# ori-drs/gpmp2

Hardware: AMD Instinct MI355X
Metric: trajectories/sec (higher is better)
Workload: dtype f64; 1 GPU; WAMFactorGraphExample: 7-DOF WAM, 100 steps x 5 GP-interp, 200^3 SDF (Synth200), 64 random-init restarts per GPU, GN to tolerance; restarts_per_gpu=64, total_restarts=64, total_step=100, obs_check_inter=5, optimizer=GN, parallelism=trajectory-sharded x1

## Files before the change

### gpmp2_amd/csrc/assembler.h

```cpp
#pragma once
#include "device_math.h"
#include "plan.h"
#include "tiles.h"

namespace g2 {

#ifdef G2_STAMPS
#define G2_BSTAMP(k) do { if (i == 4 && lane == 0 && row0 == 0 && col0 == 0 && pb.iters[b] == G2_STAMP_ITER) pb.stamps[(size_t)b * 64 + 24 + (k)] = __builtin_amdgcn_s_memtime(); } while (0)
#else
#define G2_BSTAMP(k) do {} while (0)
#endif

constexpr int GP_EXTRA_LIE = 18;

template <int D, bool LIE>
struct Assembler {
  static constexpr int n = 2 * D, NG = D * (D + 1) / 2, RECP = NG + D + 1;
  static constexpr int GPN = n + 1 + GP_EXTRA_LIE;
  static constexpr int CQ = 24;
  static constexpr int PT_EXTRA_LIE = 36;
  static constexpr int RECMAX = RECP + PT_EXTRA_LIE;

  struct Slot {
    double* base;
    int rec;
    int npts;
    int gps;
    __device__ __forceinline__ double* pt(int jj) const { return base + jj * rec; }
    __device__ __forceinline__ const double* gpr() const { return base + npts * rec; }
    __device__ __forceinline__ double* gpw() const { return base + npts * rec; }
    __device__ __forceinline__ const double* coef(int jj) const { return base + npts * rec + gps + CQ * jj; }
  };
  __host__ __device__ static int slot_doubles(int I, int RECS, int GPS) { return (I + 1) * RECS + GPS + CQ * I; }
  __device__ __forceinline__ Slot make_slot(double* smem, int which) const {
    return Slot{smem + which * slot_doubles(P.I, P.RECS, P.GPS), P.RECS, P.I + 1, P.GPS};
  }

  const PlanParams& P;
  const PlanBuffers& pb;
  const double* rec;
  const double* gpu;
  int b, lane, c, g;
  int rhscol;
  int row0, col0;
  int tri[4];
  bool valid[4];
  int a_row[4], k_row[4], a_col, k_col;

  __device__ Assembler(const PlanParams& P_, const PlanBuffers& pb_, const double* rec_, const double* gpu_,
                       int b_, int lane_, int row0_ = 0, int col0_ = 0, int rhscol_ = RHSCOL)
      : P(P_), pb(pb_), rec(rec_), gpu(gpu_), b(b_), lane(lane_), c(col0_ + (lane_ & 15)), g(row0_ + (lane_ >> 4)),
        rhscol(rhscol_), row0(row0_), col0(col0_) {
    a_col = c >= D;
    k_col = c - a_col * D;
#pragma unroll
    for (int k = 0; k < 4; k++) {
      const int rho = g + 4 * k;
      valid[k] = rho < n && c < n;
      a_row[k] = rho >= D;
      k_row[k] = rho - a_row[k] * D;
      const int lo = min(k_row[k], k_col), hi = max(k_row[k], k_col);
      tri[k] = valid[k] ? lo * D - (lo * (lo - 1)) / 2 + (hi - lo) : 0;
    }
  }

  static constexpr int NLD2 = (D <= 7) ? 6 : (D <= 11) ? 9 : 14;
  __device__ __forceinline__ void stage2(int iv, const Slot& s0, const Slot& s1, int count = 2) const {
    const int I = P.I, RECS = P.RECS, GPS = P.GPS;
    double2 val[2][NLD2];
#pragma unroll
    for (int w = 0; w < 2; w++) {
      if (w >= count) break;
      const int ivw = iv + w;
      const int npt = (ivw == 0) ? 1 : I + 1;
      const int nd2 = (npt * RECS) >> 1, ng2 = GPS >> 1, nc2 = (CQ / 2) * I;
      const int p0 = (ivw == 0) ? 0 : 1 + (ivw - 1) * (I + 1);
      const bool in_range = ivw <= P.N;
      const double2* src = reinterpret_cast<const double2*>(rec + ((size_t)b * P.Ppad + p0) * RECS);
      const double2* gsrc = reinterpret_cast<const double2*>(gpu + ((size_t)b * P.Npad + ivw) * GPS);
      const double2* csrc = reinterpret_cast<const double2*>(P.coefq);
#pragma unroll
      for (int m = 0; m < NLD2; m++) {
        const int v = lane + 64 * m;
        double2 x = {0.0, 0.0};
        if (v < nd2) {
          if (in_range) x = src[v];
        } else if (v < nd2 + ng2) {
          if (in_range && ivw > 0) x = gsrc[v - nd2];
        } else if (v < nd2 + ng2 + nc2) {
          x = csrc[v - nd2 - ng2];
        }
        val[w][m] = x;
      }
    }
#pragma unroll
    for (int w = 0; w < 2; w++) {
      if (w >= count) break;
      const Slot& s = w ? s1 : s0;
      const int ivw = iv + w;
      const int npt = (ivw == 0) ? 1 : I + 1;
      const int nd2 = (npt * RECS) >> 1, ng2 = GPS >> 1, nc2 = (CQ / 2) * I;
      double2* dpt = reinterpret_cast<double2*>(s.pt((ivw == 0) ? I : 0));
      double2* dgp = reinterpret_cast<double2*>(s.gpw());
#pragma unroll
      for (int m = 0; m < NLD2; m++) {
        const int v = lane + 64 * m;
        if (v < nd2) dpt[v] = val[w][m];
        else if (v < nd2 + ng2 + nc2) dgp[v - nd2] = val[w][m];
      }
    }
  }

  __device__ __forceinline__ static double hint_vec(const double* pt, const double* M, double s, int kr) {
    const double* gp_ = pt + NG;
    if (kr >= 3) return s * gp_[kr];
    return M[0 * 3 + kr] * gp_[0] + M[1 * 3 + kr] * gp_[1] + M[2 * 3 + kr] * gp_[2];
  }

  static constexpr int KT = (D + 15) / 16;
  __device__ __forceinline__ Tile hint_tile(const double* M, const double* cf, int role, int rt, int cbase) const {
    const int j = cbase + (lane & 15), av = j >= D, kk = j - av * D;
    const double* Mk = M + (role * 2 + av) * 9;
    const double sk = cf[role * 2 + av];
    Tile T;
#pragma unroll
    for (int k = 0; k < 4; k++) {
      const int a = 16 * rt + (lane >> 4) + 4 * k;
      const bool pose = a < 3 && kk < 3;
      const double m = Mk[pose ? a * 3 + kk : 0];
      const double v = pose ? m : ((a == kk && a >= 3) ? sk : 0.0);
      T.r[k] = (a < D && j < n) ? v : 0.0;
    }
    return T;
  }
  __device__ __forceinline__ Tile g_tile(const double* pt, int rt, int ct) const {
    const int a2 = 16 * ct + (lane & 15);
    Tile T;
#pragma unroll
    for (int k = 0; k < 4; k++) {
      const int a = 16 * rt + (lane >> 4) + 4 * k;
      const bool in = a < D && a2 < D;
      const int lo = in ? min(a, a2) : 0, hi = in ? max(a, a2) : 0;
      const double v = pt[lo * D - (lo * (lo - 1)) / 2 + (hi - lo)];
      T.r[k] = in ? v : 0.0;
    }
    return T;
  }
  __device__ __forceinline__ static void mfma_atb_acc(const Tile& A, const Tile& B, int rt, v4d& acc) {
#pragma unroll
    for (int k = 0; k < 4; k++) {
      if (16 * rt + 4 * k >= D) continue;
      acc = __builtin_amdgcn_mfma_f64_16x16x4f64(A.r[k], B.r[k], acc, 0, 0, 0);
    }
  }
  __device__ __forceinline__ Tile gp_tile(const double* J, double s, int rt, int cbase) const {
    const int j = cbase + (lane & 15), av = j >= D, kk = j - av * D;
    Tile T;
#pragma unroll
    for (int k = 0; k < 4; k++) {
      const int a = 16 * rt + (lane >> 4) + 4 * k;
      const bool pose = !av && a < 3 && kk < 3;
      const double m = J[pose ? a * 3 + kk : 0];
      const double v = pose ? m : ((a == kk && (av || a >= 3)) ? (av ? 1.0 : s) : 0.0);
      T.r[k] = (a < D && j < n) ? v : 0.0;
    }
    return T;
  }
  __device__ __forceinline__ Tile qc_tile(int rt, int ct) const {
    const int a2 = 16 * ct + (lane & 15);
    Tile T;
#pragma unroll
    for (int k = 0; k < 4; k++) {
      const int a = 16 * rt + (lane >> 4) + 4 * k;
      const bool in = a < D && a2 < D;
      const double v = P.Qc_inv[in ? a * D + a2 : 0];
      T.r[k] = in ? v : 0.0;
    }
    return T;
  }
  __device__ __forceinline__ static void congruence(const Tile (&G)[KT][KT], const Tile (&EL)[KT], const Tile (&ER)[KT],
                                                    v4d& acc) {
#pragma unroll
    for (int ra = 0; ra < KT; ra++) {
      v4d ge = {0.0, 0.0, 0.0, 0.0};
#pragma unroll
      for (int rb = 0; rb < KT; rb++) mfma_atb_acc(G[rb][ra], ER[rb], rb, ge);
      Tile GE;
#pragma unroll
      for (int k = 0; k < 4; k++) GE.r[k] = ge[k];
      mfma_atb_acc(EL[ra], GE, ra, acc);
    }
  }
  bool skip_interp = false;
  __device__ __forceinline__ void lie_interp(const Slot& si, const Slot& sn, bool has_prev, bool has_next, bool want_c,
                                             double (&dk)[4], double (&hrk)[4], double (&hlk)[4]) const {
    if (skip_interp) return;
    v4d ad = {dk[0], dk[1], dk[2], dk[3]}, ar_ = {hrk[0], hrk[1], hrk[2], hrk[3]}, al = {hlk[0], hlk[1], hlk[2], hlk[3]};
    auto point = [&](const double* pt, const double* cf, int role, v4d& acc_d, v4d& acc_c) {
      const double* M = pt + RECP;
      Tile G[KT][KT], EL[KT], ER[KT];
#pragma unroll
      for (int ra = 0; ra < KT; ra++) {
#pragma unroll
        for (int rb = 0; rb < KT; rb++) G[rb][ra] = g_tile(pt, rb, ra);
        EL[ra] = hint_tile(M, cf, role, ra, row0);
        ER[ra] = hint_tile(M, cf, role, ra, col0);
      }
      congruence(G, EL, ER, acc_d);
      if (want_c) {
#pragma unroll
        for (int ra = 0; ra < KT; ra++) ER[ra] = hint_tile(M, cf, 1 - role, ra, col0);
        congruence(G, EL, ER, acc_c);
      }
    };
#pragma unroll 1
    for (int jj = 0; jj < P.I; jj++) {
      const double* cf = si.coef(jj) + 16;
      if (has_prev) point(si.pt(jj), cf, 1, ad, al);
      if (has_next) point(sn.pt(jj), cf, 0, ad, ar_);
    }
#pragma unroll
    for (int k = 0; k < 4; k++) {
      dk[k] = ad[k];
      hrk[k] = ar_[k];
      hlk[k] = al[k];
    }
  }

  __device__ __forceinline__ double build_tiles(int i, const Slot& si, const Slot& sn, const double* z, Tile& S,
                                                Tile& Cl, Tile& Cr, bool want_c) const {
    const int I = P.I, N = P.N;
    const bool has_prev = i > 0, has_next = i < N;
    constexpr bool lie = LIE;
    const double dt = P.delta_t, w0 = P.Winv[0], w1 = P.Winv[1], w3 = P.Winv[3];
    const double* J3i = si.gpr() + n + 1 + 9;
    const double* J1n = sn.gpr() + n + 1;
    const double* J1i = si.gpr() + n + 1;
    const double* J3n = sn.gpr() + n + 1 + 9;

    G2_BSTAMP(0);
    const bool need_diag = (row0 == col0), need_rhs = (rhscol >= col0 && rhscol < col0 + 16);
    const int orow = row0 + lane;
    const bool owner = lane < 16 && orow < n && (need_diag || need_rhs);
    const int nxp = pb.xp_n[b];
    double o_dd = 0.0, o_gg = 0.0, o_ee = 0.0;
    if (owner) {
      const int rho = orow, ar = rho >= D, kr = rho - ar * D;
      const bool prior_here = (i == 0 || (i == N && pb.goal_on[b] && (ar || !P.end_conf_prior_off)));
      const double zz = z[rho];
      double z0 = 0.0, z1 = 0.0, z2 = 0.0;
      if (lie) { z0 = z[0]; z1 = z[1]; z2 = z[2]; }
      double dd = 0.0, gg = 0.0, ee = 0.0;
      if (prior_here) {
        const double* tg = (i == 0) ? (ar ? pb.start_vel : pb.start_conf) : (ar ? pb.end_vel : pb.end_conf);
        tg += (size_t)b * D;
        const double w = ar ? P.vel_prior_w : P.conf_prior_w;
        double dz = zz - tg[kr];
        if (lie && !ar && kr < 3) {
          const P2 bt = pose2_between(P2{z0, z1, z2}, P2{tg[0], tg[1], tg[2]});
          dz = -(kr == 0 ? bt.x : kr == 1 ? bt.y : bt.th);
        }
        dd += w;
        gg += w * dz;
        ee += w * dz * dz;
      }
      double Hh;
      if (!ar && P.flag_pos_limit && !(lie && kr < 3)) {
        const double e = hinge_limit(zz, P.pos_lo[kr], P.pos_hi[kr], P.pos_th[kr], Hh);
        dd += P.pos_w[kr] * Hh * Hh;
        gg += P.pos_w[kr] * Hh * e;
        ee += P.pos_w[kr] * e * e;
      }
      if (ar && P.flag_vel_limit) {
        const double e = hinge_limit(zz, -P.vel_lim[kr], P.vel_lim[kr], P.vel_th[kr], Hh);
        dd += P.vel_w[kr] * Hh * Hh;
        gg += P.vel_w[kr] * Hh * e;
        ee += P.vel_w[kr] * e * e;
      }
      if (ar && kr == 1 && P.vdyn_w > 0.0) {
        dd += P.vdyn_w;
        gg += P.vdyn_w * zz;
        ee += P.vdyn_w * zz * zz;
      }
      for (int e = 0; e < nxp; e++) {
        const size_t xe = (size_t)b * XP_MAX + e;
        if (pb.xp_state[xe] != i || (ar && !pb.xp_has_vel[xe])) continue;
        const double* Wm = pb.xp_info + (xe * 2 + ar) * D * D + (size_t)kr * D;
        const double* tg = pb.xp_target + xe * n + ar * D;
        double wr = 0.0, rk = 0.0;
        for (int cc = 0; cc < D; cc++) {
          double rc = z[ar * D + cc] - tg[cc];
          if (lie && !ar && cc < 3) {
            const P2 bt = pose2_between(P2{z0, z1, z2}, P2{tg[0], tg[1], tg[2]});
            rc = -(cc == 0 ? bt.x : cc == 1 ? bt.y : bt.th);
          }
          wr = fma(Wm[cc], rc, wr);
          if (cc == kr) rk = rc;
        }
        dd += Wm[kr];
        gg += wr;
        ee += wr * rk;
      }
      if (need_rhs) {
        if (!ar) gg += si.pt(I)[NG + kr];
        for (int jj = 0; jj < I; jj++) {
          const double* cf = si.coef(jj) + 16;
          const double cp = ar ? cf[3] : cf[2], cl = ar ? cf[1] : cf[0];
          if (lie) {
            if (has_prev) gg += hint_vec(si.pt(jj), si.pt(jj) + RECP + (ar ? 27 : 18), cp, kr);
            if (has_next) gg += hint_vec(sn.pt(jj), sn.pt(jj) + RECP + (ar ? 9 : 0), cl, kr);
            continue;
          }
          if (has_prev) gg = fma(cp, si.pt(jj)[NG + kr], gg);
          if (has_next) gg = fma(cl, sn.pt(jj)[NG + kr], gg);
        }
        if (!lie) {
          if (has_next) gg += ar ? (dt * sn.gpr()[kr] + sn.gpr()[D + kr]) : sn.gpr()[kr];
          if (has_prev) gg -= si.gpr()[rho];
        } else {
          if (has_next) {
            if (ar) gg += -dt * sn.gpr()[kr] - sn.gpr()[D + kr];
            else if (kr < 3) gg += J1n[0 * 3 + kr] * sn.gpr()[0] + J1n[1 * 3 + kr] * sn.gpr()[1] + J1n[2 * 3 + kr] * sn.gpr()[2];
            else gg -= sn.gpr()[kr];
          }
          if (has_prev) {
            if (ar) gg += si.gpr()[D + kr];
            else if (kr < 3) gg += J3i[0 * 3 + kr] * si.gpr()[0] + J3i[1 * 3 + kr] * si.gpr()[1] + J3i[2 * 3 + kr] * si.gpr()[2];
            else gg += si.gpr()[kr];
          }
        }
      }
      o_dd = dd;
      o_gg = gg;
      o_ee = need_diag ? ee : 0.0;
    }

    G2_BSTAMP(1);
    double dk[4] = {0, 0, 0, 0}, hrk[4] = {0, 0, 0, 0}, hlk[4] = {0, 0, 0, 0};
    const int ac = a_col, kc = k_col;
    if constexpr (!lie) {
      const int cc_ = min(c, n - 1);
      const double fp = has_prev ? 1.0 : 0.0, fn = has_next ? 1.0 : 0.0;
      int wq[4];
      const double* un = si.pt(I);
#pragma unroll
      for (int k = 0; k < 4; k++) {
        const int rr_ = min(g + 4 * k, n - 1);
        wq[k] = a_row[k] * 2 + ac;
        double d = fp * P.KB[rr_ * n + cc_] + fn * P.KA[rr_ * n + cc_];
        const double u = un[tri[k]];
        d += (wq[k] == 0) ? u : 0.0;
        dk[k] = d;
        if (want_c) {
          hrk[k] = fn * P.KO[rr_ * n + cc_];
          hlk[k] = fp * P.KO[cc_ * n + rr_];
        }
      }
      G2_BSTAMP(2);
      if (has_prev && has_next) {
#pragma unroll 1
        for (int jj = 0; jj < I; jj++) {
          const double* cq = si.coef(jj);
          const double* pp_ = si.pt(jj);
          const double* pn_ = sn.pt(jj);
#pragma unroll
          for (int k = 0; k < 4; k++) {
            const double Gp = pp_[tri[k]], Gn = pn_[tri[k]];
            dk[k] = fma(cq[wq[k]], Gp, dk[k]);
            dk[k] = fma(cq[4 + wq[k]], Gn, dk[k]);
            if (want_c) {
              hrk[k] = fma(cq[8 + wq[k]], Gn, hrk[k]);
              hlk[k] = fma(cq[12 + wq[k]], Gp, hlk[k]);
            }
          }
        }
      } else {
        for (int jj = 0; jj < I; jj++) {
          const double* cq = si.coef(jj);
          const double* pp_ = si.pt(jj);
          const double* pn_ = sn.pt(jj);
#pragma unroll
          for (int k = 0; k < 4; k++) {
            if (has_prev) {
              const double Gp = pp_[tri[k]];
              dk[k] = fma(cq[wq[k]], Gp, dk[k]);
              if (want_c) hlk[k] = fma(cq[12 + wq[k]], Gp, hlk[k]);
            }
            if (has_next) {
              const double Gn = pn_[tri[k]];
              dk[k] = fma(cq[4 + wq[k]], Gn, dk[k]);
              if (want_c) hrk[k] = fma(cq[8 + wq[k]], Gn, hrk[k]);
            }
          }
        }
      }
#pragma unroll
      for (int k = 0; k < 4; k++) {
        dk[k] = valid[k] ? dk[k] : 0.0;
        hrk[k] = valid[k] ? hrk[k] : 0.0;
        hlk[k] = valid[k] ? hlk[k] : 0.0;
      }
    } else {
    v4d xdp = {0.0, 0.0, 0.0, 0.0}, xl = xdp, xdn = xdp, xr = xdp;
    {
      Tile Qt[KT][KT], EL[KT], ER[KT];
#pragma unroll
      for (int ra = 0; ra < KT; ra++)
#pragma unroll
        for (int rb = 0; rb < KT; rb++) Qt[rb][ra] = qc_tile(rb, ra);
      if (has_prev) {
#pragma unroll
        for (int ra = 0; ra < KT; ra++) { EL[ra] = gp_tile(J3i, 1.0, ra, row0); ER[ra] = gp_tile(J3i, 1.0, ra, col0); }
        congruence(Qt, EL, ER, xdp);
// ... 63 lines not shown
```

### gpmp2_amd/csrc/cr_kernels.hip

```cpp
#include "assembler.h"
#include "cr_schedule.h"
#include "dispatch.h"
#include "plan_device.h"

namespace g2 {

#ifdef G2_STAMPS
#define G2_STAMP(k)                                                          \
  do {                                                                       \
    if (tid == 0 && (k) < 64 && g2_son) pb.stamps[(size_t)b * 64 + (k)] = __builtin_amdgcn_s_memtime(); \
  } while (0)
#define G2_STAMP_DECL const bool g2_son = pb.iters[b] == G2_STAMP_ITER
#else
#define G2_STAMP(k) do {} while (0)
#define G2_STAMP_DECL do {} while (0)
#endif
#ifdef G2_TSTAMPS
#define G2_TSTAMP(q)                                                                                     \
  do {                                                                                                   \
    if (w == 0 && lane == 0 && idx == 0 && g2_son && (h == 4 || h == 8 || h == 16)) \
      pb.stamps[((size_t)gridDim.x + b) * 64 + (h == 4 ? 0 : h == 8 ? 8 : 16) + (q)] = __builtin_amdgcn_s_memtime(); \
  } while (0)
#else
#define G2_TSTAMP(q) do {} while (0)
#endif
#ifdef G2_STAMPS
#define G2_ASTAMP(k) do { if (v == 5 && lane == 0 && pb.iters[b] == G2_STAMP_ITER) pb.stamps[(size_t)b * 64 + 32 + (k)] = __builtin_amdgcn_s_memtime(); \
                          if (v == 6 && lane == 0 && pb.iters[b] == G2_STAMP_ITER) pb.stamps[(size_t)b * 64 + 40 + (k)] = __builtin_amdgcn_s_memtime(); } while (0)
#else
#define G2_ASTAMP(k) do {} while (0)
#endif

template <int n>
__device__ __forceinline__ void schur_sub(Tile& S, const Tile& A, int lane) {
  const int c = lane & 15, g = lane >> 4;
  const Tile T = tile_atb(A, A);
#pragma unroll
  for (int k = 0; k < 4; k++)
    if ((g + 4 * k) < n && (c < n || c == RHSCOL)) S.r[k] -= T.r[k];
}
constexpr unsigned long long schur_mask(int n, int k) {
  unsigned long long m = 0;
  for (int g = 0; g < 4; g++)
    for (int c = 0; c < 16; c++)
      if (g + 4 * k < n && (c < n || c == RHSCOL)) m |= 1ull << (16 * g + c);
  return m;
}
template <unsigned long long M>
__device__ __forceinline__ double keep_lanes(double x) {
  int lo = __double2loint(x), hi = __double2hiint(x);
  const unsigned long long m = M;
  asm("v_cndmask_b32_e64 %0, 0, %0, %2\n\tv_cndmask_b32_e64 %1, 0, %1, %2" : "+v"(lo), "+v"(hi) : "s"(m));
  return __hiloint2double(hi, lo);
}
template <int n>
__device__ __forceinline__ void schur_keep(Tile& T) {
  T.r[0] = keep_lanes<schur_mask(n, 0)>(T.r[0]);
  T.r[1] = keep_lanes<schur_mask(n, 1)>(T.r[1]);
  T.r[2] = keep_lanes<schur_mask(n, 2)>(T.r[2]);
  T.r[3] = keep_lanes<schur_mask(n, 3)>(T.r[3]);
}
template <int n>
__device__ __forceinline__ Tile schur_prod(const Tile& A, int lane) {
  Tile T = tile_atb(A, A);
  schur_keep<n>(T);
  return T;
}
template <int n>
__device__ __forceinline__ Tile coupling(const Tile& A, const Tile& B, int lane) {
  const int c = lane & 15, g = lane >> 4;
  Tile T = tile_atb(A, B);
#pragma unroll
  for (int k = 0; k < 4; k++) T.r[k] = ((g + 4 * k) < n && c < n) ? -T.r[k] : 0.0;
  return T;
}

constexpr int ASM_WAVES = 4;
constexpr int ASM_WT_MAX_B = 256;
#ifndef G2_ASM_MINW
#define G2_ASM_MINW 5
#endif
template <int D, bool LIE, StorePolicy ASM_OUT>
__global__ __launch_bounds__(64 * ASM_WAVES, LIE ? 2 : G2_ASM_MINW) void k_assemble(const PlanParams* __restrict__ pp, PlanBuffers pb,
                                                              const double* __restrict__ traj, int bufsel,
                                                              double* __restrict__ tiles,
                                                              const int* __restrict__ active, int early_stop) {
  constexpr int n = 2 * D;
  using Asm = Assembler<D, LIE>;
  const PlanParams& P = *pp;
  const int N = P.N;
  const int groups = crr_groups(N, ASM_WAVES);
  const int b = blockIdx.x / groups, q = blockIdx.x - b * groups;
  if (active && !active[b]) return;
  if (early_stop) {
    int status;
    if (gn_decide(P.rules, pb.iters[b], pb.prev_err[b], error_from_shares(P, pb, b), status) != 0) return;
  }
  if (active && dogleg_retry(P, pb, b)) return;
  const int wv = threadIdx.x >> 6, lane = threadIdx.x & 63, c = lane & 15, g = lane >> 4;
  const int v = ASM_WAVES * q + wv, i = v - 1;
  const bool live = v >= 1 && i <= N;
  const int ic = min(max(i, 0), N);
  extern __shared__ __attribute__((aligned(16))) double asm_smem[];
  const int slotd = Asm::slot_doubles(P.I, P.RECS, P.GPS);
  double* xch = asm_smem + (size_t)(ASM_WAVES + 1) * slotd;
  double* xs0 = (slotd >= TILE_DBL) ? asm_smem : xch + 4 * TILE_DBL;
  const double* rec = rec_of(pb, pb.which[b], bufsel);
  const double* gpu = gpu_of(pb, pb.which[b], bufsel);
  Asm as(P, pb, rec, gpu, b, lane);
  G2_ASTAMP(0);
  const typename Asm::Slot slot0 = as.make_slot(asm_smem, wv), slot1 = as.make_slot(asm_smem, wv + 1);
  as.stage2(max(i, 0), slot0, slot1, wv == ASM_WAVES - 1 ? 2 : 1);
  __syncthreads();
  G2_ASTAMP(1);
  const bool odd = (v & 1) != 0;
  const bool fuse2 = N >= 3;
  const bool lvl2 = fuse2 && wv == 2 && live;
  Tile S, Cl, Cr;
  double err_acc = as.build_tiles(ic, slot0, slot1, traj + ((size_t)b * (N + 1) + ic) * n, S, Cl, Cr,
                                  odd || P.rules.opt_type == GPMP2MI_OPT_DOGLEG);
  G2_ASTAMP(2);
  if (live) {
    if (!early_stop) {
      err_acc = wave_sum(err_acc);
      if (lane == 0) pb.epart[(size_t)b * P.Npad + i] = 0.5 * err_acc;
      if (c == RHSCOL) {
#pragma unroll
        for (int k = 0; k < 4; k++) pb.gvec[((size_t)b * (N + 1) + i) * 16 + g + 4 * k] = -S.r[k];
      }
    }
    if (P.rules.opt_type == GPMP2MI_OPT_DOGLEG) {
      double* ht = pb.htiles + ((size_t)b * (N + 1) + i) * 2 * TILE_DBL;
      tile_store(ht, S, lane);
      tile_store(ht + TILE_DBL, Cr, lane);
    }
    if (P.rules.opt_type == GPMP2MI_OPT_LM) {
      const double lam = pb.lambda[b];
#pragma unroll
      for (int k = 0; k < 4; k++)
        if (g + 4 * k == c && c < n) S.r[k] += lam;
    }
    if (!odd) {
      if (!fuse2) tile_store_rows<n, ASM_OUT>(tiles + ((size_t)b * (N + 1) + i) * TILE_DBL, S, lane);
      else if (wv == 0) tile_store(xs0, S, lane);
    } else {
      Tile V;
      G2_ASTAMP(3);
      const bool ok = tile_eliminate_cv<n>(S, Cl, Cr, V, lane);
      G2_ASTAMP(4);
      double* f = pb.fac + ((size_t)b * (N + 1) + i) * 3 * TILE_DBL;
      tile_store_rows<n, ASM_OUT>(f, Cl, lane);
      tile_store_rows<n, ASM_OUT>(f + TILE_DBL, Cr, lane);
      tile_store_transposed<n, ASM_OUT>(f + 2 * TILE_DBL, V, lane);
      if (fuse2) {
        double* x = xch + (size_t)(wv >> 1) * 2 * TILE_DBL;
        tile_store(x, Cl, lane);
        tile_store(x + TILE_DBL, Cr, lane);
      }
      if (!ok && lane == 0) pb.notspd[b] = 1;
      G2_ASTAMP(5);
    }
  }
  if (!fuse2) return;
  __syncthreads();
  G2_ASTAMP(6);
  if (wv != 2) return;
  const int v0 = ASM_WAVES * q, M = N + 1;
  const bool has0 = q >= 1;
  const bool next = v0 + 4 <= M;
  Tile Sp = tile_zero();
  if (has0) Sp = tile_load(xs0, lane);
  Tile A1 = tile_zero(), R = tile_zero();
  if (has0 && v0 + 1 <= M) {
    const Tile Wl1 = tile_load(xch, lane);
    A1 = tile_atb(Wl1, Wl1);
  }
  if (next) {
    const Tile Wr3 = tile_load(xch + 3 * TILE_DBL, lane);
    R = tile_atb(Wr3, Wr3);
  }
  if (live) {
    const Tile Wr_m = tile_load(xch + TILE_DBL, lane);
    schur_sub<n>(S, Wr_m, lane);
    Tile C2l = tile_zero(), C2r = tile_zero();
    if (has0) {
      const Tile Wl_m = tile_load(xch, lane);
      C2l = coupling<n>(Wr_m, Wl_m, lane);
    }
    if (v + 1 <= M) {
      const Tile Wl_p = tile_load(xch + 2 * TILE_DBL, lane);
      schur_sub<n>(S, Wl_p, lane);
      if (v + 2 <= M) {
        const Tile Wr_p = tile_load(xch + 3 * TILE_DBL, lane);
        C2r = coupling<n>(Wl_p, Wr_p, lane);
      }
    }
    Tile V;
    const bool ok = tile_eliminate_cv<n>(S, C2l, C2r, V, lane);
    double* f = pb.fac + ((size_t)b * (N + 1) + i) * 3 * TILE_DBL;
    tile_store_rows<n, ASM_OUT>(f, C2l, lane);
    tile_store_rows<n, ASM_OUT>(f + TILE_DBL, C2r, lane);
    tile_store_transposed<n, ASM_OUT>(f + 2 * TILE_DBL, V, lane);
    if (!ok && lane == 0) pb.notspd[b] = 1;
    const Tile A2 = tile_atb(C2l, C2l);
#pragma unroll
    for (int k = 0; k < 4; k++) A1.r[k] += A2.r[k];
    if (next) {
      const Tile B2 = tile_atb(C2r, C2r);
#pragma unroll
      for (int k = 0; k < 4; k++) R.r[k] += B2.r[k];
      if (has0) {
        const Tile K = (q & 1) ? coupling<n>(C2l, C2r, lane) : coupling<n>(C2r, C2l, lane);
        tile_store_rows<n, ASM_OUT>(pb.coup + ((size_t)b * groups + q) * TILE_DBL, K, lane);
      }
    }
    G2_ASTAMP(7);
  }
  schur_keep<n>(A1);
  schur_keep<n>(R);
  if (has0) {
#pragma unroll
    for (int k = 0; k < 4; k++) Sp.r[k] -= A1.r[k];
    tile_store_rows<n, ASM_OUT>(tiles + ((size_t)b * (N + 1) + v0 - 1) * TILE_DBL, Sp, lane);
  }
  if (next) tile_store_rows<n, ASM_OUT>(pb.pend + ((size_t)b * groups + q) * TILE_DBL, R, lane);
}

int launch_assemble(const PlanParams& hp, const PlanBuffers& pb, const double* traj, int bufsel,
                    const int* active, hipStream_t st, bool early_stop) {
  const int es = early_stop ? 1 : 0;
  const dim3 grid(hp.B * crr_groups(hp.N, ASM_WAVES)), block(64 * ASM_WAVES);
  const size_t slotd = (size_t)(hp.I + 1) * hp.RECS + hp.GPS + 24 * hp.I;
  const size_t shmem = ((ASM_WAVES + 1) * slotd + (slotd >= TILE_DBL ? 4 : 5) * TILE_DBL) * sizeof(double);
  return launch_for_dof(TILE_DOFS, hp.D, [&](auto d) {
    constexpr int D = decltype(d)::value;
    constexpr StorePolicy WT = StorePolicy::WriteThrough, PL = StorePolicy::Plain;
    const bool wt = hp.B <= ASM_WT_MAX_B;
    if (hp.lie && wt) k_assemble<D, true, WT><<<grid, block, shmem, st>>>(pb.params, pb, traj, bufsel, pb.tiles, active, es);
    else if (hp.lie) k_assemble<D, true, PL><<<grid, block, shmem, st>>>(pb.params, pb, traj, bufsel, pb.tiles, active, es);
    else if (wt) k_assemble<D, false, WT><<<grid, block, shmem, st>>>(pb.params, pb, traj, bufsel, pb.tiles, active, es);
    else k_assemble<D, false, PL><<<grid, block, shmem, st>>>(pb.params, pb, traj, bufsel, pb.tiles, active, es);
  });
}

constexpr int FIN_BLOCKS = 8;
#ifndef G2_CR_WAVES
#define G2_CR_WAVES 16
#endif
constexpr int CR_WAVES = G2_CR_WAVES;



template <int n>
__device__ __forceinline__ bool cr_forward(const PlanBuffers& pb, int b, int N, int tid) {
  const int w = __builtin_amdgcn_readfirstlane(tid >> 6), lane = tid & 63, c = lane & 15, g = lane >> 4;
  double* tiles = pb.tiles + (size_t)b * (N + 1) * TILE_DBL;
  double* fac = pb.fac + (size_t)b * (N + 1) * 3 * TILE_DBL;
  bool ok = true;
  G2_STAMP_DECL;
  const int htop = crr_top(N), M = N + 1;
  const int h0 = (N >= 3) ? 4 : 2;
  const bool defer4 = (h0 == 4) && (htop >= 8);
  for (int h = h0; h <= htop; h <<= 1) {
    const CrrLevel level = crr_level(N, h, !(defer4 && h == 4));
    const int hh = h >> 1;
    for (int idx = w; idx < level.tasks(); idx += CR_WAVES) {
      const bool elim = level.elim(idx);
      const int v = level.block(idx), j = v - 1;
      const bool first = h0 == 4 && (h == 4 || (defer4 && h == 8));
      const bool ready = h0 == 4 && h == 4;
      const int jm = j - hh, jp = j + hh, qj = v >> 2;
      const bool ep = v + hh <= M;
      const bool cm = elim && v - h >= 1, cp = elim && v + h <= M;
      auto facp = [&](int blk, int which) { return fac + ((size_t)blk * 3 + which) * TILE_DBL; };
      const int groups = crr_groups(N, 4);
      const double* pend = pb.pend + (size_t)b * groups * TILE_DBL;
      const double* coup = pb.coup + (size_t)b * groups * TILE_DBL;
      G2_TSTAMP(0);
      Tile S = tile_load_rows<n>(tiles + (size_t)j * TILE_DBL, lane);
      Tile Pd = tile_zero();
      Tile Wr_m = tile_zero(), Wl_m = tile_zero(), Wl_p = tile_zero(), Wr_p = tile_zero();
      Tile Cl = tile_zero(), Cr = tile_zero();
      if (first) Pd = tile_load_rows<n>(pend + (size_t)(qj - 1) * TILE_DBL, lane);
      if (ready) {
        if (cm) Cl = tile_load_rows<n>(coup + (size_t)(qj - 1) * TILE_DBL, lane);
        if (cp) Cr = tile_load_rows<n>(coup + (size_t)qj * TILE_DBL, lane);
      } else {
        Wr_m = tile_load_rows<n>(facp(jm, 1), lane);
        if (cm) Wl_m = tile_load_rows<n>(facp(jm, 0), lane);
        if (ep) Wl_p = tile_load_rows<n>(facp(jp, 0), lane);
        if (cp) Wr_p = tile_load_rows<n>(facp(jp, 1), lane);
      }
#ifdef G2_TSTAMPS
      asm volatile("s_waitcnt vmcnt(0)" ::: "memory");
#endif
      G2_TSTAMP(1);
#pragma unroll
      for (int k = 0; k < 4; k++) S.r[k] -= Pd.r[k];
      if (!ready) {
        schur_sub<n>(S, Wr_m, lane);
        if (cm) Cl = coupling<n>(Wr_m, Wl_m, lane);
        if (ep) schur_sub<n>(S, Wl_p, lane);
        if (cp) Cr = coupling<n>(Wl_p, Wr_p, lane);
      }
      if (!elim) {
        tile_store_rows<n>(tiles + (size_t)j * TILE_DBL, S, lane);
        continue;
      }
#ifdef G2_TSTAMPS
      asm volatile("" : "+v"(S.r[0]), "+v"(Cl.r[0]), "+v"(Cr.r[0]));
#endif
      G2_TSTAMP(2);
      Tile V;
      ok = tile_eliminate_cv<n>(S, Cl, Cr, V, lane) && ok;
#ifdef G2_TSTAMPS
      asm volatile("" : "+v"(V.r[0]), "+v"(Cl.r[0]), "+v"(Cr.r[0]));
#endif
      G2_TSTAMP(3);
      double* f = fac + (size_t)j * 3 * TILE_DBL;
      tile_store_rows<n>(f, Cl, lane);
      tile_store_rows<n>(f + TILE_DBL, Cr, lane);
      tile_store_rows<n>(f + 2 * TILE_DBL, V, lane);
      G2_TSTAMP(4);
    }
    __syncthreads();
    { const int idx = 0; G2_TSTAMP(5); }
    G2_STAMP(5 + __builtin_ctz(h));
  }
  return ok;
}

template <int n>
__device__ __forceinline__ void cr_backward(const PlanBuffers& pb, int b, int N, int tid, double* xs, int hmin = 1) {
  const int w = __builtin_amdgcn_readfirstlane(tid >> 6), lane = tid & 63, c = lane & 15, g = lane >> 4;
  const double* fac = pb.fac + (size_t)b * (N + 1) * 3 * TILE_DBL;
  G2_STAMP_DECL;
  const int htop = crr_top(N), M = N + 1;
  Tile pWl = tile_zero(), pWr = tile_zero(), pV = tile_zero();
  auto prefetch = [&](int h) {
    if (h >= hmin && w < crr_back_count(N, h)) {
      const double* f = fac + (size_t)(crr_back_block(N, h, w) - 1) * 3 * TILE_DBL;
      pWl = tile_load_rows<n>(f, lane);
      pWr = tile_load_rows<n>(f + TILE_DBL, lane);
      pV = load_v<n>(f + 2 * TILE_DBL, h, N, lane);
    }
  };
  prefetch(htop);
  for (int h = htop; h >= hmin; h >>= 1) {
    const int count = crr_back_count(N, h);
    for (int idx = w; idx < count; idx += CR_WAVES) {
      const int v = crr_back_block(N, h, idx), j = v - 1;
      Tile Wl = pWl, Wr = pWr, V = pV;
      if (idx != w) {
        const double* f = fac + (size_t)j * 3 * TILE_DBL;
        Wl = tile_load_rows<n>(f, lane);
        Wr = tile_load_rows<n>(f + TILE_DBL, lane);
        V = load_v<n>(f + 2 * TILE_DBL, h, N, lane);
      }
      const int jl = j - h, jr = j + h;
      const double xl = (v - h >= 1) ? xs[jl * 16 + c] : 0.0;
      const double xr = (v + h <= M) ? xs[jr * 16 + c] : 0.0;
      const double x = cr_backsolve<n>(Wl, Wr, V, xl, xr, lane);
      if (g == 0) xs[j * 16 + c] = (c < n) ? x : 0.0;
    }
    prefetch(h >> 1);
    __syncthreads();
    G2_STAMP(16 + __builtin_ctz(h));
  }

}

template <int D>
__device__ __forceinline__ void gn_step_body(const PlanParams& P, const PlanBuffers& pb, int pass, int early_stop) {
  constexpr int n = 2 * D;
  const int b = blockIdx.x, tid = threadIdx.x, w = tid >> 6, lane = tid & 63, c = lane & 15, g = lane >> 4;
  if (!pb.active[b]) return;
  const int N = P.N;
  const size_t tsz = (size_t)(N + 1) * n;
  const bool odd = P.fuse_finish && (pass & 1);
  double* cur = (odd ? pb.last : pb.cur) + b * tsz;
  double* last = (odd ? pb.cur : pb.last) + b * tsz;
  double* result = pb.result + b * tsz;
  extern __shared__ __attribute__((aligned(16))) double smem[];
  double* xs = smem;
  double* red = smem + (size_t)(N + 1) * 16;
  int* flags = reinterpret_cast<int*>(red + CR_WAVES);
  G2_STAMP_DECL;

  G2_STAMP(0);
  const int it = pb.iters[b];
  const double prev = pb.prev_err[b];
  double new_err;
  if (early_stop) {
    new_err = error_from_shares(P, pb, b);
    if (tid == 0) flags[1] = 0;
  } else {
    if (w == 0) {
      double acc = 0.0;
      for (int i = lane; i <= N; i += 64) acc += pb.epart[(size_t)b * P.Npad + i];
      acc = wave_sum(acc);
      if (lane == 0) {
        red[0] = acc;
        flags[1] = 0;
      }
    }
    __syncthreads();
    new_err = red[0];
  }
  int status;
  const int decision = gn_decide(P.rules, it, prev, new_err, status);
  if (tid == 0) {
    if (it <= P.rules.max_iter) pb.trace[(size_t)b * (P.rules.max_iter + 1) + it] = new_err;
    pb.cur_err[b] = new_err;
    if (decision != 0) {
      pb.status[b] = status;
      pb.final_err[b] = (decision == 2) ? prev : new_err;
    }
  }
  const bool keep_err = it == 0 || (decision == 0 && P.rules.fixed_iters == 0);
  if (decision != 0) {
    const double* src = (decision == 2) ? last : cur;
    for (size_t k = tid; k < tsz; k += blockDim.x) result[k] = src[k];
    __syncthreads();
    if (tid == 0) {
      if (keep_err) pb.prev_err[b] = new_err;
      pb.active[b] = 0;
    }
    return;
  }

  G2_STAMP(1);
  const bool ok = cr_forward<n>(pb, b, N, tid);
  G2_STAMP(2);
  if ((!ok && lane == 0) || (tid == 0 && pb.notspd[b])) flags[1] = 1;
  __syncthreads();
  if (tid == 0 && keep_err) pb.prev_err[b] = new_err;
  if (flags[1]) {
    if (tid == 0) pb.notspd[b] = 0;
    for (size_t k = tid; k < tsz; k += blockDim.x) result[k] = cur[k];
    if (tid == 0) {
      pb.status[b] = GPMP2MI_TRAJ_NOT_SPD;
      pb.final_err[b] = pb.cur_err[b];
      pb.active[b] = 0;
    }
    return;
  }

  if (P.split_back) {
    cr_backward<n>(pb, b, N, tid, xs, FIN_BLOCKS);
    G2_STAMP(3);
    double* xg = pb.xg + (size_t)b * (N + 1) * 16;
    for (int k = tid; k < ((N + 1) / FIN_BLOCKS) * 16; k += blockDim.x) {
      const size_t o = ((size_t)((k >> 4) + 1) * FIN_BLOCKS - 1) * 16 + (k & 15);
      xg[o] = xs[o];
    }
    G2_STAMP(4);
    if (tid == 0) {
      pb.stepped[b] = pass + 1;
      pb.last_err[b] = pb.cur_err[b];
      pb.iters[b] += 1;
      atomicAdd(pb.n_active + pass, 1);
    }
    return;
  }
  cr_backward<n>(pb, b, N, tid, xs);
  G2_STAMP(3);
  for (size_t k = tid; k < tsz; k += blockDim.x) last[k] = cur[k];
  __syncthreads();
  for (size_t k = tid; k < tsz; k += blockDim.x) {
    const int i = (int)(k / n), rho = (int)(k - (size_t)i * n);
    const double* zs = last + (size_t)i * n;
    const double* dz = xs + i * 16;
    cur[k] = (rho < D) ? retract_coord(P.lie != 0, rho, zs, dz) : zs[rho] + dz[rho];
  }
  G2_STAMP(4);
  if (tid == 0) {
    pb.last_err[b] = pb.cur_err[b];
    pb.iters[b] += 1;
    atomicAdd(pb.n_active + pass, 1);
  }
}
template <int D>
__global__ __launch_bounds__(64 * CR_WAVES) void k_gn_step_cr(const PlanParams* __restrict__ pp,
                                                               PlanBuffers pb, int pass, int early_stop) {
  gn_step_body<D>(*pp, pb, pass, early_stop);
  if (threadIdx.x == 0) publish_pass_count(pb, pass);
}

template <int D>
struct FinishGroup {
  static constexpr int n = 2 * D;
  Tile Wl, Wr, V;
  int b, q, wv, lane, c, g, v, i, N;
  bool live;
  __device__ __forceinline__ FinishGroup(const PlanBuffers& pb, int N_, int b_, int q_, double (*xl_)[16])
      : b(b_), q(q_), N(N_) {
    wv = __builtin_amdgcn_readfirstlane(threadIdx.x >> 6);
    lane = threadIdx.x & 63;
    c = lane & 15;
    g = lane >> 4;
    v = FIN_BLOCKS * q + wv;
    i = v - 1;
    live = v >= 1 && i <= N;
    const double* xg = pb.xg + (size_t)b * (N + 1) * 16;
    const double* fac = pb.fac + (size_t)b * (N + 1) * 3 * TILE_DBL;
    Wl = Wr = V = tile_zero();
    if (live && wv != 0) {
      const double* f = fac + (size_t)i * 3 * TILE_DBL;
      Wl = tile_load_rows<n>(f, lane);
      Wr = tile_load_rows<n>(f + TILE_DBL, lane);
      V = load_v<n>(f + 2 * TILE_DBL, (v & 3) ? 1 : 4, N, lane);
    }
    if (wv == 0 && lane < 16) xl_[0][lane] = live ? xg[(size_t)i * 16 + lane] : 0.0;
    if (wv == 1 && lane < 16)
      xl_[FIN_BLOCKS][lane] = (FIN_BLOCKS * q + FIN_BLOCKS <= N + 1) ? xg[(size_t)(FIN_BLOCKS * q + FIN_BLOCKS - 1) * 16 + lane] : 0.0;
  }
  __device__ __forceinline__ void solve(int h, double (*xl_)[16]) const {
    const int vl = v - h, vr = v + h;
    const double xl = (vl >= 1) ? xl_[vl - FIN_BLOCKS * q][c] : 0.0;
    const double xr = (vr <= N + 1) ? xl_[vr - FIN_BLOCKS * q][c] : 0.0;
    const double x = cr_backsolve<n>(Wl, Wr, V, xl, xr, lane);
    if (g == 0) xl_[wv][c] = (c < n) ? x : 0.0;
  }
  __device__ __forceinline__ void solve_all(double (*xl_)[16]) const {
    __syncthreads();
    if (wv == 4 && live) solve(4, xl_);
    __syncthreads();
    if ((wv == 2 || wv == 6) && live) solve(2, xl_);
    __syncthreads();
    if ((wv & 1) && live) solve(1, xl_);
    __syncthreads();
  }
};

template <int D>
__global__ __launch_bounds__(64 * FIN_BLOCKS) void k_finish_step(const PlanParams* __restrict__ pp, PlanBuffers pb, int pass) {
  constexpr int n = 2 * D;
  const PlanParams& P = *pp;
  const int N = P.N;
  const int groups = crr_groups(N, FIN_BLOCKS);
  const int b = blockIdx.x / groups, q = blockIdx.x - b * groups;
  if (pb.stepped[b] != pass + 1) return;
  __shared__ double xl_[FIN_BLOCKS + 1][16];
  const FinishGroup<D> fg(pb, N, b, q, xl_);
  fg.solve_all(xl_);
  const int lane = fg.lane, i = fg.i;
  if (!fg.live || lane >= n) return;
  const size_t k = ((size_t)b * (N + 1) + i) * n + lane;
  const double* zs = pb.cur + ((size_t)b * (N + 1) + i) * n;
  const double zold = zs[lane];
  const double znew = (lane < D) ? retract_coord(P.lie != 0, lane, zs, xl_[fg.wv]) : zold + xl_[fg.wv][lane];
  pb.last[k] = zold;
  __builtin_amdgcn_wave_barrier();
  pb.cur[k] = znew;
}

int launch_finish_step(const PlanParams& hp, const PlanBuffers& pb, int pass, hipStream_t st) {
  const dim3 grid(hp.B * crr_groups(hp.N, FIN_BLOCKS)), block(64 * FIN_BLOCKS);
  return launch_for_dof(TILE_DOFS, hp.D, [&](auto d) {
    k_finish_step<decltype(d)::value><<<grid, block, 0, st>>>(pb.params, pb, pass);
  });
}

template <int D, int X>
__device__ __forceinline__ void finish_trial_group(const PlanParams& P, const PlanBuffers& pb, int b, int q, int i0,
                                                   const double* x) {
  constexpr int n = 2 * D;
  __shared__ double psum[FIN_BLOCKS][3];
  const int N = P.N, groups = P.spart_groups;
  const int wv = __builtin_amdgcn_readfirstlane(threadIdx.x >> 6), lane = threadIdx.x & 63;
  const int i = i0 + wv;
  double gd = 0.0, dd = 0.0, gg = 0.0;
  if (i >= 0 && i <= N && lane < n) {
    const size_t k = ((size_t)b * (N + 1) + i) * n + lane;
    const double* zs = pb.cur + ((size_t)b * (N + 1) + i) * n;
    const double xk = x[lane], gk = pb.gvec[((size_t)b * (N + 1) + i) * X + lane];
    pb.delta[k] = xk;
    pb.trial[k] = (lane < D) ? retract_coord(P.lie != 0, lane, zs, x) : zs[lane] + xk;
    gd = gk * xk;
    dd = xk * xk;
    gg = gk * gk;
  }
  gd = wave_sum(gd);
  dd = wave_sum(dd);
  gg = wave_sum(gg);
  if (lane == 0) {
    psum[wv][0] = gd;
    psum[wv][1] = dd;
    psum[wv][2] = gg;
  }
  __syncthreads();
  if (threadIdx.x < 3) {
    const int t = threadIdx.x;
    double a = 0.0;
    for (int w = 0; w < FIN_BLOCKS; w++) a += psum[w][t];
    pb.spart[((size_t)b * groups + q) * 3 + t] = a;
  }
}

template <int D>
__global__ __launch_bounds__(64 * FIN_BLOCKS) void k_finish_trial(const PlanParams* __restrict__ pp, PlanBuffers pb) {
  const PlanParams& P = *pp;
  const int N = P.N;
  const int groups = crr_groups(N, FIN_BLOCKS);
  const int b = blockIdx.x / groups, q = blockIdx.x - b * groups;
  if (!pb.active[b] || pb.stepped[b] != 1) return;
  __shared__ double xl_[FIN_BLOCKS + 1][16];
  const FinishGroup<D> fg(pb, N, b, q, xl_);
  fg.solve_all(xl_);
  finish_trial_group<D, 16>(P, pb, b, q, FIN_BLOCKS * q - 1, xl_[fg.wv]);
}

int launch_finish_trial(const PlanParams& hp, const PlanBuffers& pb, hipStream_t st) {
  const dim3 grid(hp.B * crr_groups(hp.N, FIN_BLOCKS)), block(64 * FIN_BLOCKS);
  return launch_for_dof(TILE_DOFS, hp.D, [&](auto d) {
    k_finish_trial<decltype(d)::value><<<grid, block, 0, st>>>(pb.params, pb);
  });
}

int launch_gn_step_cr(const PlanParams& hp, const PlanBuffers& pb, int pass, hipStream_t st, bool early_stop) {
  const dim3 grid(hp.B), block(64 * CR_WAVES);
  const size_t shmem = ((size_t)(hp.N + 1) * 16 + CR_WAVES + 2) * sizeof(double);
  if (shmem > 150 * 1024) {
    set_error("total_step too large for the LDS-resident solution buffer");
    return GPMP2MI_ERR_UNSUPPORTED;
  }
  return launch_for_dof(TILE_DOFS, hp.D, [&](auto d) {
    k_gn_step_cr<decltype(d)::value><<<grid, block, shmem, st>>>(pb.params, pb, pass, early_stop ? 1 : 0);
  });
}

#include "wide_cr.h"

template <int D_>
struct CrForm {
  static constexpr int D = D_, n = 2 * D, WAVES = CR_WAVES, X = 16;
  static __device__ __forceinline__ int handed(int N) { return (N + 1) / FIN_BLOCKS; }
  static __device__ __forceinline__ int handed_state(int k) { return (k + 1) * FIN_BLOCKS - 1; }
  static __device__ __forceinline__ bool forward(const PlanParams& P, const PlanBuffers& pb, int b, int tid) {
    return cr_forward<n>(pb, b, P.N, tid);
  }
  static __device__ __forceinline__ void backward(const PlanBuffers& pb, int b, int N, int tid, double* xs, int hmin = 1) {
    cr_backward<n>(pb, b, N, tid, xs, hmin);
  }
};
template <int D_>
struct WcrForm {
  static constexpr int D = D_, n = 2 * D, WAVES = WCR_WAVES, X = WX;
  static __device__ __forceinline__ int handed(int N) { return N / FIN_BLOCKS + 1; }
  static __device__ __forceinline__ int handed_state(int k) { return k * FIN_BLOCKS; }
  static __device__ __forceinline__ bool forward(const PlanParams& P, const PlanBuffers& pb, int b, int tid) {
    return wcr_forward<n>(pb, b, P.N, tid, P.wide_h0);
  }
  static __device__ __forceinline__ void backward(const PlanBuffers& pb, int b, int N, int tid, double* xs, int hmin = 1) {
    wcr_backward<n>(pb, b, N, tid, xs, hmin);
  }
};

template <class F>
__global__ __launch_bounds__(64 * F::WAVES) void k_solve_step(const PlanParams* __restrict__ pp, PlanBuffers pb) {
  constexpr int X = F::X;
  const PlanParams& P = *pp;
  const int b = blockIdx.x, tid = threadIdx.x;
  if (!pb.active[b]) return;
  const int N = P.N;
  double* sc = pb.scal + (size_t)b * SC_COUNT;
  extern __shared__ __attribute__((aligned(16))) double smem[];
  double* xs = smem;
  double* red = smem + (size_t)(N + 1) * X;
  int* flags = reinterpret_cast<int*>(red + F::WAVES);
  const bool dogleg = P.rules.opt_type == GPMP2MI_OPT_DOGLEG;
  const bool resolve = !dogleg_retry(P, pb, b);
  if (tid == 0) {
    flags[1] = 0;
    pb.stepped[b] = 0;
  }
  __syncthreads();
  if (resolve) {
    const bool ok = F::forward(P, pb, b, tid);
    if ((!ok && (tid & 63) == 0) || (tid == 0 && pb.notspd[b])) flags[1] = 1;
    __syncthreads();
    if (flags[1]) {
      if (tid == 0) pb.notspd[b] = 1;
      return;
    }
    if (P.split_back && !dogleg) {
      F::backward(pb, b, N, tid, xs, FIN_BLOCKS);
      double* xg = pb.xg + (size_t)b * (N + 1) * X;
      for (int k = tid; k < F::handed(N) * X; k += blockDim.x) {
        const size_t o = (size_t)F::handed_state(k / X) * X + (k % X);
        xg[o] = xs[o];
      }
      if (tid == 0) pb.stepped[b] = 1;
      return;
    }
    F::backward(pb, b, N, tid, xs);
    if (dogleg) {
      double acc = 0.0;
      for (int i = tid; i <= N; i += blockDim.x) acc += pb.hgpart[(size_t)b * P.Npad + i];
      acc = block_sum<F::WAVES>(acc, red, tid);
      if (tid == 0) sc[SC_GHG] = acc;
    }
  }
  trial_step_tail<F::WAVES, X>(P, pb, b, F::n, F::D, resolve, xs, xs, pb.gvec + (size_t)b * (N + 1) * X, red, tid,
                               blockDim.x);
}

int launch_solve_step(const PlanParams& hp, const PlanBuffers& pb, hipStream_t st) {
  const dim3 grid(hp.B), block(64 * CR_WAVES);
  const size_t shmem = ((size_t)(hp.N + 1) * 16 + CR_WAVES + 2) * sizeof(double);
  return launch_for_dof(TILE_DOFS, hp.D, [&](auto d) {
    k_solve_step<CrForm<decltype(d)::value>><<<grid, block, shmem, st>>>(pb.params, pb);
  });
}

int launch_solve_step_wide(const PlanParams& hp, const PlanBuffers& pb, hipStream_t st) {
  const dim3 grid(hp.B), block(64 * WCR_WAVES);
  const size_t shmem = ((size_t)(hp.N + 1) * WX + WCR_WAVES + 2) * sizeof(double);
  if (shmem > 150 * 1024) {
    set_error("total_step too large for the LDS-resident solution buffer");
    return GPMP2MI_ERR_UNSUPPORTED;
  }
  return launch_for_dof(WIDE_DOFS, hp.D, [&](auto d) {
    k_solve_step<WcrForm<decltype(d)::value>><<<grid, block, shmem, st>>>(pb.params, pb);
  });
}

template <int D>
__global__ __launch_bounds__(64) void k_ghg(const PlanParams* __restrict__ pp, PlanBuffers pb) {
  constexpr int n = 2 * D;
  const PlanParams& P = *pp;
  const int N = P.N;
  const int b = blockIdx.x / (N + 1), i = blockIdx.x - b * (N + 1);
  if (!pb.active[b] || dogleg_retry(P, pb, b)) return;
  const int lane = threadIdx.x, c = lane & 15, g = lane >> 4;
  const double* ht = pb.htiles + ((size_t)b * (N + 1) + i) * 2 * TILE_DBL;
  const Tile Dt = tile_load(ht, lane), Ht = tile_load(ht + TILE_DBL, lane);
  const double* gv = pb.gvec + ((size_t)b * (N + 1) + i) * 16;
  const double gi_c = (c < n) ? gv[c] : 0.0;
  const double gn_c = (c < n && i < N) ? gv[16 + c] : 0.0;
  double acc = 0.0;
#pragma unroll
  for (int k = 0; k < 4; k++) {
    const int rho = g + 4 * k;
    const double gi_r = (rho < n) ? gv[rho] : 0.0;
    if (c < n) acc += gi_r * (Dt.r[k] * gi_c + 2.0 * Ht.r[k] * gn_c);
  }
  acc = wave_sum(acc);
  if (lane == 0) pb.hgpart[(size_t)b * P.Npad + i] = acc;
}

int launch_ghg(const PlanParams& hp, const PlanBuffers& pb, hipStream_t st) {
  const dim3 grid(hp.B * (hp.N + 1)), block(64);
  return launch_for_dof(TILE_DOFS, hp.D, [&](auto d) { k_ghg<decltype(d)::value><<<grid, block, 0, st>>>(pb.params, pb); });
}

__global__ void k_debug_crosslane(const double* __restrict__ in, double* __restrict__ out) {
  const int l = threadIdx.x;
  const double v = in[l];
  out[0 * 64 + l] = bcast_row<0>(v);
  out[1 * 64 + l] = bcast_row<1>(v);
  out[2 * 64 + l] = bcast_row<2>(v);
  out[3 * 64 + l] = bcast_row<3>(v);
  out[4 * 64 + l] = bcast_in_row<5>(v);
  out[5 * 64 + l] = row_sum16_dpp(v);
  out[6 * 64 + l] = sum_rows(v);
  out[7 * 64 + l] = bcast_in_row<13>(v);
}
int launch_debug_crosslane(const double* in, double* out, hipStream_t st) {
  k_debug_crosslane<<<dim3(1), dim3(64), 0, st>>>(in, out);
  G2_HIP(hipGetLastError());
  return GPMP2MI_OK;
}

}
```

### gpmp2_amd/csrc/host/plan_create.hip

```cpp
#include <cmath>
#include <cstring>
#include <mutex>

#include "host.h"
#include "../cr_schedule.h"
#include "../dispatch.h"

namespace g2 {
static std::mutex g_flag_mu;
static std::vector<FlagBuf> g_flag_pool;
static std::atomic<long> g_live_chunks{0}, g_live_flagbufs{0}, g_leaked_plans{0};
int flags_acquire(int need, FlagBuf* out) {
  {
    std::lock_guard<std::mutex> lk(g_flag_mu);
    int cur = 0;
    (void)hipGetDevice(&cur);
    for (size_t k = 0; k < g_flag_pool.size(); k++)
      if (g_flag_pool[k].cap >= need && g_flag_pool[k].device == cur) {
        *out = g_flag_pool[k];
        g_flag_pool.erase(g_flag_pool.begin() + k);
        g_live_flagbufs.fetch_add(1);
        return GPMP2MI_OK;
      }
  }
// ... 85 lines not shown
  p->arena_left -= bytes;
  return GPMP2MI_OK;
}

static int choose_forms(const RobotDev& h, const gpmp2mi_settings& s, int B, const gpmp2mi_debug_forms* force,
                        PlanForms* out) {
  const gpmp2mi_debug_forms f = force ? *force : gpmp2mi_debug_forms{};
  const int D = h.dof, N = s.total_step, I = s.obs_check_inter;
  const bool fixed_arm = h.kind == GPMP2MI_ROBOT_ARM;
  G2_CHECK(f.lin_split == 0 || f.lin_split == 1 || (fixed_arm && (f.lin_split == 2 || f.lin_split == 4)), GPMP2MI_ERR_UNSUPPORTED,
           "forced lin_split: 1, or 2 / 4 on a fixed-base arm");
  static_assert(chunk_states(2) <= ZNS && chunk_states(1) > ZNS, "the I >= 2 below and at the default choice");
  G2_CHECK(f.lin_split != 4 || I >= 2, GPMP2MI_ERR_UNSUPPORTED, "forced lin_split 4: needs obs_check_inter >= 2");
  PlanForms F;
  F.wide = 2 * D > 15;
  G2_CHECK(!f.wide_dense || F.wide, GPMP2MI_ERR_UNSUPPORTED, "forced wide_dense: the plan has no wide blocks (dof < 8)");
  F.dense = D > 11 || f.wide_dense;
  F.split_back = !F.dense && N >= 16;
  while (F.wide && F.wide_h0 < 8 && 4 * F.wide_h0 <= N) F.wide_h0 *= 2;
  const bool four = B <= 256 || s.opt_type != GPMP2MI_OPT_DOGLEG;
  F.lin_split = (fixed_arm && h.nr_spheres >= 2) ? (four ? 4 : 2) : 1;
  if (F.lin_split == 4 && I < 2) F.lin_split = 2;
  if (f.lin_split) F.lin_split = f.lin_split;
  F.fuse_finish = F.lin_split == 4 && F.split_back && !F.wide && !f.no_fused_finish;
  F.spart_groups = F.fuse_finish ? (1 + N * (I + 1) + 63) / 64 : F.wide ? (N + 8) / 8 : crr_groups(N, 8);
  F.generic_gn = f.generic_gn != 0;
  F.no_early_stop = f.no_early_stop != 0;
  *out = F;
  return GPMP2MI_OK;
}

static int fill_params(const RobotDev& h, const gpmp2mi_settings* s, const gpmp2mi_graph_opts& o, const PlanForms& F,
                       int B, PlanParams& P) {
  const int D = h.dof;
  std::memset(&P, 0, sizeof(P));
  P.B = B;
  P.N = s->total_step;
  P.I = s->obs_check_inter;
  P.P = 1 + P.N * (P.I + 1);
  P.Ppad = (P.P + 63) / 64 * 64;
  P.D = D;
  P.n = 2 * D;
  P.NG = D * (D + 1) / 2;
  P.REC = P.NG + D + 1 + ((h.base_dof == 3 && P.I > 0) ? 36 : 0);
  P.Npad = (P.N + 1 + 63) / 64 * 64;
  P.lie = h.base_dof == 3 ? 1 : 0;
  P.wide = F.wide; P.split_back = F.split_back; P.spart_groups = F.spart_groups;
  P.wide_h0 = F.wide_h0; P.lin_split = F.lin_split; P.fuse_finish = F.fuse_finish;
  P.GPREC = P.n + 1 + (P.lie ? 18 : 0);
  P.RECS = (P.REC + 1) & ~1;
  P.GPS = (P.GPREC + 1) & ~1;
  P.obs_skip_first = o.obs_skip_first_state;
  P.flag_pos_limit = s->flag_pos_limit;
  P.flag_vel_limit = s->flag_vel_limit;
  P.rules.opt_type = s->opt_type;
  P.rules.max_iter = s->max_iter;
  P.rules.no_increase = s->final_iter_no_increase;
  P.rules.fixed_iters = o.fixed_iterations;
  P.end_conf_prior_off = o.end_conf_prior_off ? 1 : 0;
  P.eps = s->epsilon;
  P.obs_w = 1.0 / (s->cost_sigma * s->cost_sigma);
  P.delta_t = s->total_time / static_cast<double>(s->total_step);
  const double inter_dt = P.delta_t / static_cast<double>(s->obs_check_inter + 1);
  P.conf_prior_w = 1.0 / (s->conf_prior_sigma * s->conf_prior_sigma);
  P.vel_prior_w = 1.0 / (s->vel_prior_sigma * s->vel_prior_sigma);
  P.vdyn_w = o.vehicle_dynamics_sigma > 0 ? 1.0 / (o.vehicle_dynamics_sigma * o.vehicle_dynamics_sigma) : 0.0;
  P.rules.rel_thresh = s->rel_thresh;
  P.rules.abs_tol = o.abs_error_tol;
  P.rules.err_tol = o.error_tol;
  P.rules.lm_lambda0 = o.lm_lambda_initial;
  P.rules.lm_factor = o.lm_lambda_factor;
  P.rules.lm_upper = o.lm_lambda_upper;
  P.rules.lm_lower = o.lm_lambda_lower;
  P.rules.lm_min_fidelity = o.lm_min_model_fidelity;
  P.rules.dl_delta0 = o.dogleg_delta_initial;
  for (int j = 0; j < P.I; j++) {
    P.coef[j] = gp_coef(P.delta_t, inter_dt * static_cast<double>(j + 1));
    const double lam[2] = {P.coef[j].l11, P.coef[j].l12}, psi[2] = {P.coef[j].p11, P.coef[j].p12};
    double* q = P.coefq[j];
    for (int ar = 0; ar < 2; ar++)
      for (int ac = 0; ac < 2; ac++) {
        q[0 + ar * 2 + ac] = psi[ar] * psi[ac];
        q[4 + ar * 2 + ac] = lam[ar] * lam[ac];
        q[8 + ar * 2 + ac] = lam[ar] * psi[ac];
        q[12 + ar * 2 + ac] = psi[ar] * lam[ac];
      }
    q[16] = lam[0]; q[17] = lam[1]; q[18] = psi[0]; q[19] = psi[1];
  }
  gp_winv(P.delta_t, P.Winv);
  std::vector<double> Qc(D * D, 0.0), Qi(D * D, 0.0);
  for (int i = 0; i < D; i++) Qc[i * D + i] = 1.0;
  if (s->Qc) std::copy(s->Qc, s->Qc + D * D, Qc.begin());
  G2_CHECK(invert_small(D, Qc.data(), Qi.data()), GPMP2MI_ERR_INVALID, "Qc is singular");
  std::copy(Qi.begin(), Qi.end(), P.Qc_inv);
  for (int k = 0; k < D; k++) {
    P.pos_lo[k] = s->joint_pos_limits_down ? s->joint_pos_limits_down[k] : -1e6;
    P.pos_hi[k] = s->joint_pos_limits_up ? s->joint_pos_limits_up[k] : 1e6;
    P.pos_th[k] = s->pos_limit_thresh ? s->pos_limit_thresh[k] : 1e-3;
    const double ps = s->pos_limit_sigmas ? s->pos_limit_sigmas[k] : 1e-3;
    P.pos_w[k] = 1.0 / (ps * ps);
    P.vel_lim[k] = s->vel_limits ? s->vel_limits[k] : 1e6;
    P.vel_th[k] = s->vel_limit_thresh ? s->vel_limit_thresh[k] : 1e-3;
    const double vs = s->vel_limit_sigmas ? s->vel_limit_sigmas[k] : 1e-3;
    P.vel_w[k] = 1.0 / (vs * vs);
  }
  {
    const int n = P.n;
    const double dt = P.delta_t;
    auto W = [&](int r, int c) { return P.Winv[(r / D) * 2 + (c / D)] * Qi[(r % D) * D + (c % D)]; };
    auto PtW = [&](int r, int c) { return r < D ? W(r, c) : dt * W(r - D, c) + W(r, c); };
    for (int r = 0; r < n; r++)
      for (int c = 0; c < n; c++) {
        P.KB[r * n + c] = W(r, c);
        P.KO[r * n + c] = -PtW(r, c);
        P.KA[r * n + c] = c < D ? PtW(r, c) : dt * PtW(r, c - D) + PtW(r, c);
      }
  }
  const int cap = std::max(P.rules.fixed_iters, P.rules.max_iter);
  P.max_pass = cap * (P.rules.opt_type == GPMP2MI_OPT_LM ? 6 : P.rules.opt_type == GPMP2MI_OPT_DOGLEG ? 18 : 1) + 3;
  return GPMP2MI_OK;
}

struct ExtrasHost {
  std::vector<double> des, scd, radius;
};
static int check_extras(const RobotDev& h, const gpmp2mi_graph_opts& o, int N, PlanExtras& ex, ExtrasHost& hx) {
  std::memset(&ex, 0, sizeof(ex));
  G2_CHECK(o.n_workspace >= 0 && o.n_workspace <= GPMP2MI_MAX_WORKSPACE_FACTORS, GPMP2MI_ERR_INVALID, "too many workspace factors");
  G2_CHECK(o.n_self_collision >= 0 && o.n_self_collision <= GPMP2MI_MAX_SELF_COLLISION_PAIRS, GPMP2MI_ERR_INVALID,
           "too many self-collision pairs");
  ex.n_ws = o.n_workspace;
  ex.n_sc = o.n_self_collision;
  hx.des.assign(16 * std::max(ex.n_ws, 1), 0.0);
  hx.scd.assign(4 * std::max(ex.n_sc, 1), 0.0);
  hx.radius.assign(std::max(h.nr_spheres, 1), 0.0);
  for (int f = 0; f < ex.n_ws; f++) {
    const gpmp2mi_workspace_factor& w = o.workspace[f];
    G2_CHECK(w.mode >= GPMP2MI_WORKSPACE_POSITION && w.mode <= GPMP2MI_WORKSPACE_POSE, GPMP2MI_ERR_INVALID, "unknown workspace factor mode");
    G2_CHECK(w.link >= 0 && w.link < h.nr_links, GPMP2MI_ERR_INVALID, "workspace factor: link out of range");
    G2_CHECK(w.sigma > 0, GPMP2MI_ERR_INVALID, "workspace factor: sigma must be positive");
    G2_CHECK(w.first_state >= 0 && w.first_state <= w.last_state && w.last_state <= N, GPMP2MI_ERR_INVALID,
             "workspace factor: bad state range");
    ex.ws_mode[f] = w.mode;
    ex.ws_link[f] = w.link;
    ex.ws_first[f] = w.first_state;
    ex.ws_last[f] = w.last_state;
    ex.ws_w[f] = 1.0 / (w.sigma * w.sigma);
    std::copy(w.des_pose, w.des_pose + 16, hx.des.begin() + 16 * f);
  }
  if (ex.n_sc > 0) {
    G2_CHECK(o.self_collision_first >= 0 && o.self_collision_first <= o.self_collision_last && o.self_collision_last <= N,
             GPMP2MI_ERR_INVALID, "self collision: bad state range");
    ex.sc_first = o.self_collision_first;
    ex.sc_last = o.self_collision_last;
    for (int k = 0; k < ex.n_sc; k++) {
      const double a = o.self_collision[k][0], bb = o.self_collision[k][1], sg = o.self_collision[k][3];
      G2_CHECK(a >= 0 && a < h.nr_spheres && bb >= 0 && bb < h.nr_spheres, GPMP2MI_ERR_INVALID, "self collision: sphere id out of range");
      G2_CHECK(sg > 0, GPMP2MI_ERR_INVALID, "self collision: sigma must be positive");
      for (int t = 0; t < 4; t++) hx.scd[4 * k + t] = o.self_collision[k][t];
      ex.sc_w[k] = 1.0 / (sg * sg);
    }
  }
  G2_CHECK(o.max_moving_spheres >= 0 && o.max_moving_spheres <= GPMP2MI_MAX_MOVING_SPHERES, GPMP2MI_ERR_INVALID,
           "max_moving_spheres outside 0..GPMP2MI_MAX_MOVING_SPHERES");
  if (o.max_moving_spheres > 0) {
    G2_CHECK(o.moving_sigma > 0 && std::isfinite(o.moving_sigma), GPMP2MI_ERR_INVALID, "moving spheres: sigma must be positive");
    G2_CHECK(std::isfinite(o.moving_epsilon), GPMP2MI_ERR_INVALID, "moving spheres: epsilon must be finite");
    G2_CHECK(o.moving_first >= 0 && o.moving_first <= o.moving_last && o.moving_last <= N, GPMP2MI_ERR_INVALID,
             "moving spheres: bad state range");
    ex.mv_cap = o.max_moving_spheres;
    ex.mv_first = o.moving_first;
    ex.mv_last = o.moving_last;
    ex.mv_eps = o.moving_epsilon;
    ex.mv_w = 1.0 / (o.moving_sigma * o.moving_sigma);
  }
  G2_CHECK(o.max_self_pairs >= 0, GPMP2MI_ERR_INVALID, "max_self_pairs is negative");
  G2_CHECK(o.max_self_pairs <= GPMP2MI_MAX_PLAN_SELF_PAIRS, GPMP2MI_ERR_INVALID,
           "max_self_pairs above GPMP2MI_MAX_PLAN_SELF_PAIRS");
  if (o.max_self_pairs > 0) {
    G2_CHECK(o.self_pairs_first >= 0 && o.self_pairs_first <= o.self_pairs_last && o.self_pairs_last <= N,
             GPMP2MI_ERR_INVALID, "self-collision table: bad state range");
    ex.sp_cap = o.max_self_pairs;
    ex.sp_first = o.self_pairs_first;
    ex.sp_last = o.self_pairs_last;
  }
  G2_CHECK(o.max_carried_spheres >= 0 && o.max_carried_spheres <= GPMP2MI_MAX_CARRIED_SPHERES, GPMP2MI_ERR_INVALID,
           "max_carried_spheres outside 0..GPMP2MI_MAX_CARRIED_SPHERES");
  if (o.max_carried_spheres > 0) {
    G2_CHECK(o.carried_sigma > 0 && std::isfinite(o.carried_sigma), GPMP2MI_ERR_INVALID, "carried object: sigma must be positive");
    G2_CHECK(std::isfinite(o.carried_epsilon), GPMP2MI_ERR_INVALID, "carried object: epsilon must be finite");
    G2_CHECK(o.carried_first >= 0 && o.carried_first <= o.carried_last && o.carried_last <= N, GPMP2MI_ERR_INVALID,
             "carried object: bad state range");
    G2_DISPATCH_ROBOT_H(h, (void)0);
    ex.cr_cap = o.max_carried_spheres;
    ex.cr_first = o.carried_first;
    ex.cr_last = o.carried_last;
    ex.cr_eps = o.carried_epsilon;
    ex.cr_w = 1.0 / (o.carried_sigma * o.carried_sigma);
  }
  if (ex.n_sc > 0 || ex.mv_cap > 0)
    for (int sidx = 0; sidx < h.nr_spheres; sidx++) hx.radius[h.sph_orig[sidx]] = h.sph_r[sidx];
  G2_CHECK(o.workspace_path == 0 || o.workspace_path == 1, GPMP2MI_ERR_INVALID, "workspace_path must be 0 or 1");
  if (o.workspace_path) {
    G2_CHECK(o.workspace_path_mode >= GPMP2MI_WORKSPACE_POSITION && o.workspace_path_mode <= GPMP2MI_WORKSPACE_POSE,
             GPMP2MI_ERR_INVALID, "workspace path: unknown mode");
    G2_CHECK(o.workspace_path_link >= 0 && o.workspace_path_link < h.nr_links, GPMP2MI_ERR_INVALID,
             "workspace path: link out of range");
    G2_DISPATCH_ROBOT_H(h, (void)0);
    ex.wp_cap = 1;
    ex.wp_mode = o.workspace_path_mode;
    ex.wp_link = o.workspace_path_link;
  }
  return GPMP2MI_OK;
}

static int alloc_buffers(gpmp2mi_plan* p, const ExtrasHost& hx) {
  const PlanParams& P = p->hp;
  const PlanForms& F = p->forms;
  const RobotDev& h = p->robot->h;
  PlanBuffers& pb = p->pb;
  PlanExtras& ex = p->ex;
  const int B = P.B, D = P.D;
  const size_t tsz = p->tsz(), M = (size_t)B * (P.N + 1);
  std::memset(&pb, 0, sizeof(pb));
  G2_TRY(plan_alloc(p, &pb.params, 1));
  for (double** q : {&pb.start_conf, &pb.start_vel, &pb.end_conf, &pb.end_vel}) G2_TRY(plan_alloc(p, q, (size_t)B * D));
  for (double** q : {&pb.cur, &pb.last, &pb.trial, &pb.init, &pb.result, &pb.delta}) G2_TRY(plan_alloc(p, q, tsz));
  const size_t tq = F.wide ? 4 : 1;
  G2_TRY(plan_alloc(p, &pb.gvec, (size_t)B * (P.N + 1) * (F.wide ? 32 : 16)));
  G2_TRY(plan_alloc(p, &pb.htiles, P.rules.opt_type == GPMP2MI_OPT_DOGLEG ? (size_t)B * (P.N + 1) * 512 * tq : 1));
  G2_TRY(plan_alloc(p, &pb.hgpart, (size_t)B * P.Npad));
  G2_TRY(plan_alloc(p, &pb.scal, (size_t)B * SC_COUNT));
  for (int** q : {&pb.which, &pb.stepped}) G2_TRY(plan_alloc(p, q, B));
  G2_TRY(plan_alloc(p, &pb.spart, (size_t)B * std::max((P.N + 4) / 4, P.Ppad / 64) * 3));
  G2_TRY(plan_alloc(p, &pb.xg, (size_t)B * (P.N + 1) * (F.wide ? 32 : 16)));
  if (F.dense) {
    G2_TRY(plan_alloc(p, &pb.wHd, (size_t)B * (P.N + 1) * P.n * P.n));
    G2_TRY(plan_alloc(p, &pb.wHo, (size_t)B * P.N * P.n * P.n));
    G2_TRY(plan_alloc(p, &pb.wg, (size_t)B * (P.N + 1) * P.n));
    for (double** q : {&pb.wWl, &pb.wWr}) G2_TRY(plan_alloc(p, q, (size_t)B * (P.N + 1) * P.n * P.n));
    for (double** q : {&pb.wy, &pb.wrb, &pb.wx}) G2_TRY(plan_alloc(p, q, (size_t)B * (P.N + 1) * P.n));
  }
  G2_TRY(plan_alloc(p, &pb.xp_n, B));
  for (int** q : {&pb.xp_state, &pb.xp_has_vel}) G2_TRY(plan_alloc(p, q, (size_t)B * XP_MAX));
  G2_TRY(plan_alloc(p, &pb.xp_target, (size_t)B * XP_MAX * P.n));
  G2_TRY(plan_alloc(p, &pb.xp_info, (size_t)B * XP_MAX * 2 * D * D));
  G2_TRY(plan_alloc(p, &pb.goal_on, B));
  for (double** q : {&pb.rec, &pb.rec2}) G2_TRY(plan_alloc(p, q, (size_t)B * P.RECS * P.Ppad));
  for (double** q : {&pb.gpu, &pb.gpu2}) G2_TRY(plan_alloc(p, q, (size_t)B * P.GPS * P.Npad));
  G2_TRY(plan_alloc(p, &pb.tiles, (size_t)B * (P.N + 1) * 256 * tq));
  G2_TRY(plan_alloc(p, &pb.fac, (size_t)B * (P.N + 1) * 768 * tq));
  for (double** q : {&pb.pend, &pb.coup}) G2_TRY(plan_alloc(p, q, (size_t)B * crr_groups(P.N, 4) * 256));
  for (double** q : {&pb.cur_err, &pb.prev_err, &pb.last_err, &pb.final_err, &pb.lambda}) G2_TRY(plan_alloc(p, q, B));
  G2_TRY(plan_alloc(p, &pb.trace, (size_t)B * (P.rules.max_iter + 1)));
  for (int** q : {&pb.iters, &pb.status, &pb.active, &pb.phase, &pb.notspd}) G2_TRY(plan_alloc(p, q, B));
  G2_TRY(plan_alloc(p, &pb.epart, (size_t)B * P.Npad));
  G2_TRY(plan_alloc(p, &pb.cshare, (size_t)B * (P.Ppad / 64) * 3));
  if (ex.n_ws > 0) {
    G2_TRY(plan_alloc(p, &ex.des, hx.des.size()));
    G2_TRY(plan_alloc(p, &ex.poses, M * h.nr_links * 16));
    G2_TRY(plan_alloc(p, &ex.Jp, M * h.nr_links * 6 * D));
    G2_TRY(plan_alloc(p, &ex.ws_err, (size_t)ex.n_ws * M * 6));
    G2_TRY(plan_alloc(p, &ex.ws_H, (size_t)ex.n_ws * M * 6 * D));
  }
  if (ex.n_sc > 0) {
    G2_TRY(plan_alloc(p, &ex.sc_data, hx.scd.size()));
    G2_TRY(plan_alloc(p, &ex.radius, hx.radius.size()));
    G2_TRY(plan_alloc(p, &ex.cen, M * h.nr_spheres * 3));
    G2_TRY(plan_alloc(p, &ex.Jc, M * h.nr_spheres * 3 * D));
    G2_TRY(plan_alloc(p, &ex.sc_err, M * ex.n_sc));
    G2_TRY(plan_alloc(p, &ex.sc_H, M * ex.n_sc * D));
  }
  if (ex.mv_cap > 0) {
    if (ex.n_sc == 0) {
      G2_TRY(plan_alloc(p, &ex.radius, hx.radius.size()));
      G2_TRY(plan_alloc(p, &ex.cen, M * h.nr_spheres * 3));
      G2_TRY(plan_alloc(p, &ex.Jc, M * h.nr_spheres * 3 * D));
    }
    G2_TRY(plan_alloc(p, &ex.mv_radius, (size_t)ex.mv_cap));
    G2_TRY(plan_alloc(p, &ex.mv_centers, (size_t)ex.mv_cap * (P.N + 1) * 3));
  }
  if (ex.sp_cap > 0) {
    if (ex.n_sc == 0 && ex.mv_cap == 0) {
      G2_TRY(plan_alloc(p, &ex.cen, M * h.nr_spheres * 3));
      G2_TRY(plan_alloc(p, &ex.Jc, M * h.nr_spheres * 3 * D));
    }
    G2_TRY(plan_alloc(p, &ex.sp_rec, (size_t)ex.sp_cap));
  }
  if (ex.wp_cap > 0) {
    G2_TRY(plan_alloc(p, &ex.wp_des, (size_t)(P.N + 1) * 16));
    G2_TRY(plan_alloc(p, &ex.wp_sigma, (size_t)P.N + 1));
    G2_TRY(plan_alloc(p, &ex.wp_list, (size_t)P.N + 1));
    G2_TRY(plan_alloc(p, &ex.wp_count, 1));
  }
  if (ex.cr_cap > 0) {
    G2_TRY(plan_alloc(p, &ex.cr_radius, (size_t)ex.cr_cap));
    G2_TRY(plan_alloc(p, &ex.cr_centers, (size_t)ex.cr_cap * 3));
  }
  G2_TRY(plan_alloc(p, &pb.n_active, p->n_active_len));
  G2_TRY(plan_alloc(p, &pb.stamps, (size_t)B * 128));
  G2_TRY(flags_acquire(p->n_active_len, &p->flagbuf));
  p->h_flags = p->flagbuf.host;
  pb.host_flags = p->flagbuf.dev;
  G2_TRY(plan_alloc(p, &pb.done, p->n_active_len));
  return GPMP2MI_OK;
}

static int upload_constants(gpmp2mi_plan* p, const ExtrasHost& hx) {
  const std::vector<int> ones(p->hp.B, 1);
  G2_HIP(hipMemcpy(p->pb.goal_on, ones.data(), ones.size() * sizeof(int), hipMemcpyHostToDevice));
  const PlanExtras& ex = p->ex;
  if (ex.n_ws > 0) G2_HIP(hipMemcpy(ex.des, hx.des.data(), hx.des.size() * sizeof(double), hipMemcpyHostToDevice));
  if (ex.n_sc > 0) {
    G2_HIP(hipMemcpy(ex.sc_data, hx.scd.data(), hx.scd.size() * sizeof(double), hipMemcpyHostToDevice));
  }
  if (ex.n_sc > 0 || ex.mv_cap > 0)
    G2_HIP(hipMemcpy(ex.radius, hx.radius.data(), hx.radius.size() * sizeof(double), hipMemcpyHostToDevice));
  G2_HIP(hipMemcpy(p->pb.params, &p->hp, sizeof(p->hp), hipMemcpyHostToDevice));
  G2_HIP(hipStreamSynchronize(nullptr));
  p->null_stream_dirty = false;
  return GPMP2MI_OK;
}

extern "C" {

int gpmp2mi_plan_create(const gpmp2mi_robot* robot, const gpmp2mi_sdf* sdf, const gpmp2mi_settings* s,
                        const gpmp2mi_graph_opts* o, int B, gpmp2mi_plan** out) {
  return gpmp2mi_debug_plan_create(robot, sdf, s, o, B, nullptr, out);
}

int gpmp2mi_debug_plan_create(const gpmp2mi_robot* robot, const gpmp2mi_sdf* sdf, const gpmp2mi_settings* s,
                              const gpmp2mi_graph_opts* o_in, int B, const gpmp2mi_debug_forms* forms,
                              gpmp2mi_plan** out) {
  G2_CHECK(robot && sdf && s && out, GPMP2MI_ERR_INVALID, "null argument");
  *out = nullptr;
  gpmp2mi_graph_opts o;
  if (o_in) o = *o_in;
  else gpmp2mi_graph_opts_default(&o);
  const int D = robot->h.dof;
  G2_CHECK(B > 0, GPMP2MI_ERR_INVALID, "batch size must be positive");
  G2_CHECK(s->dof == D, GPMP2MI_ERR_INVALID, "[TrajOptimizerSetting] dof does not match the robot");
  G2_CHECK(s->total_step >= 1 && s->total_time > 0, GPMP2MI_ERR_INVALID, "bad total_step / total_time");
  G2_CHECK(s->obs_check_inter >= 0 && s->obs_check_inter <= MAXI, GPMP2MI_ERR_UNSUPPORTED, "obs_check_inter > 16");
  G2_CHECK(D <= MAXD, GPMP2MI_ERR_UNSUPPORTED, "plans are instantiated for dof <= 18");
  G2_CHECK(D <= 11 || D == 17 || D == 18, GPMP2MI_ERR_UNSUPPORTED,
           "plans are instantiated for dof <= 11 and for dof 17 / 18 (SE(2) base [+ lift] + two 7-joint arms)");
  PlanForms F;
  G2_TRY(choose_forms(robot->h, *s, B, forms, &F));
  {
    const int nd = D * (D + 1) / 2 + D + 1 + ((robot->h.base_dof == 3 && s->obs_check_inter > 0) ? 36 : 0);
    const int gpr = 2 * D + 1 + (robot->h.base_dof == 3 ? 18 : 0);
    const int nds = (nd + 1) & ~1, gps = (gpr + 1) & ~1;
    G2_CHECK((s->obs_check_inter + 1) * nds + gps + 24 * s->obs_check_inter <= 2 * 64 * (D > 11 ? 14 : F.wide ? 9 : 6), GPMP2MI_ERR_UNSUPPORTED,
             "obs_check_inter too large for the staged assembly");
  }
  G2_CHECK(s->opt_type >= GPMP2MI_OPT_GAUSS_NEWTON && s->opt_type <= GPMP2MI_OPT_DOGLEG, GPMP2MI_ERR_INVALID,
           "unknown opt_type");
  G2_CHECK(s->cost_sigma > 0 && s->conf_prior_sigma > 0 && s->vel_prior_sigma > 0, GPMP2MI_ERR_INVALID,
           "sigmas must be positive");
  if (s->flag_vel_limit && s->vel_limits)
    for (int k = 0; k < D; k++)
      G2_CHECK(s->vel_limits[k] > 0, GPMP2MI_ERR_INVALID, "[VelocityLimitFactorVector] velocity limit <= 0");
  G2_TRY(ensure_device());

  auto p = std::make_unique<gpmp2mi_plan>();
  p->robot = robot;
  p->sdf = sdf;
  p->forms = F;
  p->fail_alloc_at = forms ? forms->fail_alloc_at : 0;
  G2_HIP(hipGetDevice(&p->device));
  G2_TRY(fill_params(robot->h, s, o, F, B, p->hp));
  p->n_active_len = p->hp.max_pass;
  p->Qc.assign((size_t)D * D, 0.0);
  for (int i = 0; i < D; i++) p->Qc[(size_t)i * D + i] = 1.0;
  if (s->Qc) std::copy(s->Qc, s->Qc + (size_t)D * D, p->Qc.begin());
  ExtrasHost hx;
  G2_TRY(check_extras(robot->h, o, p->hp.N, p->ex, hx));
  p->has_extras = p->ex.n_ws > 0 || p->ex.n_sc > 0 || p->ex.mv_cap > 0 || p->ex.wp_cap > 0 || p->ex.sp_cap > 0 ||
                  p->ex.cr_cap > 0;
  p->h_xp_n.assign(B, 0);
  p->goal_removed.assign(B, 0);
  G2_TRY(alloc_buffers(p.get(), hx));
  G2_TRY(upload_constants(p.get(), hx));
  *out = p.release();
  return GPMP2MI_OK;
}

void gpmp2mi_plan_destroy(gpmp2mi_plan* p) { delete p; }

int gpmp2mi_debug_resource_counts(long* live_chunks, long* pooled_chunks, long* live_flagbufs, long* pooled_flagbufs,
                                  long* leaked_plans) {
  std::lock_guard<std::mutex> lk(g_flag_mu);
  if (live_chunks) *live_chunks = g_live_chunks.load();
  if (pooled_chunks) *pooled_chunks = (long)g_chunk_pool.size();
  if (live_flagbufs) *live_flagbufs = g_live_flagbufs.load();
  if (pooled_flagbufs) *pooled_flagbufs = (long)g_flag_pool.size();
  if (leaked_plans) *leaked_plans = g_leaked_plans.load();
  return GPMP2MI_OK;
}

}
```

### gpmp2_amd/csrc/host/plan_run.hip

```cpp
#include <chrono>
#include <cstdlib>

#include "host.h"

using namespace g2;

int g2::plan_linearize(gpmp2mi_plan* p, const double* traj, int bufsel, const int* active, hipStream_t st, double* dst,
                       int pass, bool trial) {
  const PlanParams& P = p->hp;
  G2_TRY(launch_linearize(p->robot->h, p->robot->d, p->sdf->h, P, p->pb, traj, bufsel, active, st, dst, pass, trial));
  if (!p->has_extras) return GPMP2MI_OK;
  if (dst) traj = dst;
  const PlanExtras& ex = p->ex;
  const RobotDev& h = p->robot->h;
  const int M = P.B * (P.N + 1), D = P.D, L = h.nr_links, S = h.nr_spheres;
  if (ex.n_ws > 0) {
    G2_TRY(launch_fk(h, p->robot->d, M, traj, ex.poses, ex.Jp, st, 2 * D));
    for (int f = 0; f < ex.n_ws; f++)
      G2_TRY(launch_workspace_prior(ex.ws_mode[f], ex.ws_link[f], L, D, M, ex.des + 16 * f, ex.poses, ex.Jp,
                                    ex.ws_err + (size_t)f * M * 6, ex.ws_H + (size_t)f * M * 6 * D, st));
  }
  if (ex.n_sc > 0 || ex.mv_K > 0 || ex.sp_P > 0)
    G2_TRY(launch_sphere_centers(h, p->robot->d, M, traj, ex.cen, ex.Jc, st, 2 * D));
  if (ex.n_sc > 0)
    G2_TRY(launch_self_collision(ex.n_sc, S, D, M, ex.sc_data, ex.radius, ex.cen, ex.Jc, ex.sc_err, ex.sc_H, st));
  if (ex.n_ws > 0 || ex.n_sc > 0) G2_TRY(launch_extra_accumulate(P, p->pb, ex, L, S, bufsel, active, st));
  G2_TRY(launch_moving_accumulate(P, p->pb, ex, S, bufsel, active, st));
  G2_TRY(launch_selfpair_accumulate(P, p->pb, ex, S, bufsel, active, st));
  G2_TRY(launch_path_accumulate(h, p->robot->d, P, p->pb, ex, traj, bufsel, active, st));
  return launch_carried_accumulate(h, p->robot->d, p->sdf->h, P, p->pb, ex, traj, bufsel, active, st);
}

static double wait_timeout_seconds() {
  const char* e = getenv("GPMP2MI_WAIT_TIMEOUT_MS");
  const double ms = e ? atof(e) : 5000.0;
  return (ms > 0 ? ms : 5000.0) * 1e-3;
}
int g2::spin_wait_flag(const volatile int* flag, bool st_valid, hipStream_t st, double timeout_s, int* count) {
  const auto t0 = std::chrono::steady_clock::now();
  double next_query = 2e-3;
  for (long spin = 0;; spin++) {
    const int v = __atomic_load_n(flag, __ATOMIC_ACQUIRE);
    if (v >= 0) {
      *count = v;
      return GPMP2MI_OK;
    }
    if ((spin & 0xfff) == 0xfff) {
      const double el0 = std::chrono::duration<double>(std::chrono::steady_clock::now() - t0).count();
      if (st_valid && el0 >= next_query) {
        next_query = el0 + 2e-3;
        const hipError_t e = hipStreamQuery(st);
        if (e == hipSuccess) {
          const int w = __atomic_load_n(flag, __ATOMIC_ACQUIRE);
          G2_CHECK(w >= 0, GPMP2MI_ERR_HIP, "pass count was never published");
          *count = w;
          return GPMP2MI_OK;
        }
        if (e != hipErrorNotReady) G2_HIP(e);
      }
      const double el = std::chrono::duration<double>(std::chrono::steady_clock::now() - t0).count();
      if (el > timeout_s) {
        set_error("timed out after " + std::to_string((int)(el * 1e3)) +
                  " ms waiting for a pass to finish (kernel hung?); GPMP2MI_WAIT_TIMEOUT_MS raises the limit");
        return GPMP2MI_ERR_TIMEOUT;
      }
    }
  }
}
static int wait_pass_count(const int* flags, int pass, hipStream_t st, int* count) {
  return spin_wait_flag(flags + pass, true, st, wait_timeout_seconds(), count);
}

static int enqueue_gn_pass(gpmp2mi_plan* p, const PlanBuffers& pb, int pass, double* states, hipStream_t st) {
  const PlanParams& P = p->hp;
  const PlanForms& F = p->forms;
  const bool early = F.early_stop(p->has_extras);
  if (P.rules.fixed_iters > 0 && pass % (P.rules.fixed_iters + 1) == P.rules.fixed_iters) {
    if (!early) {
      p->timer.begin("final_error", st);
      G2_TRY(launch_error_parts(P, pb, states, 0, pb.active, st));
    }
  } else {
    p->timer.begin("assemble", st);
    G2_TRY(launch_assemble(P, pb, states, 0, pb.active, st, early));
  }
  p->timer.begin("gn_step_cr", st);
  G2_TRY(launch_gn_step_cr(P, pb, pass, st, early));
  if (F.split_back && !F.fuse_finish) {
    p->timer.begin("finish_step", st);
    G2_TRY(launch_finish_step(P, pb, pass, st));
  }
  return GPMP2MI_OK;
}

static int enqueue_trial_pass(gpmp2mi_plan* p, const PlanBuffers& pb, hipStream_t st) {
  const PlanParams& P = p->hp;
  const PlanForms& F = p->forms;
  if (F.dense) {
    p->timer.begin("export_dense", st);
    G2_TRY(launch_export_normal_eq(P, pb, pb.cur, 0, pb.wHd, pb.wHo, pb.wg, st, pb.active));
    p->timer.begin("solve_dense", st);
    G2_TRY(launch_solve_dense(P, pb, st));
  } else if (F.wide) {
    p->timer.begin("assemble_wide", st);
    G2_TRY(launch_assemble_wide(P, pb, pb.cur, 0, pb.active, st));
    if (P.rules.opt_type == GPMP2MI_OPT_DOGLEG) {
      p->timer.begin("ghg_wide", st);
      G2_TRY(launch_ghg_wide(P, pb, st));
    }
    for (int h = 2; h < P.wide_h0; h *= 2) {
      p->timer.begin(h == 2 ? "cr_level2_wide" : "cr_level4_wide", st);
      G2_TRY(launch_cr_level_wide(P, pb, h, st));
    }
    p->timer.begin("solve_step_wide", st);
    G2_TRY(launch_solve_step_wide(P, pb, st));
    if (F.finish_trial(P.rules.opt_type)) {
      p->timer.begin("finish_trial_wide", st);
      G2_TRY(launch_finish_trial_wide(P, pb, st));
    }
  } else {
    p->timer.begin("assemble", st);
    G2_TRY(launch_assemble(P, pb, pb.cur, 0, pb.active, st));
    if (P.rules.opt_type == GPMP2MI_OPT_DOGLEG) {
      p->timer.begin("ghg", st);
      G2_TRY(launch_ghg(P, pb, st));
    }
    p->timer.begin("solve_step", st);
    G2_TRY(launch_solve_step(P, pb, st));
    if (F.finish_trial(P.rules.opt_type)) {
      p->timer.begin("finish_trial", st);
      G2_TRY(launch_finish_trial(P, pb, st));
    }
  }
  p->timer.begin("linearize", st);
  if (F.trial_lin_steps(P.rules.opt_type)) {
    return plan_linearize(p, pb.cur, 1, pb.active, st, pb.trial, 1, true);
  }
  return plan_linearize(p, pb.trial, 1, pb.active, st);
}

static double* states_of(const gpmp2mi_plan* p, int pass) {
  return (p->forms.fuse_finish && (pass & 1)) ? p->pb.last : p->pb.cur;
}
static int enqueue_gn_lin(gpmp2mi_plan* p, int pass, hipStream_t st) {
  p->timer.begin("linearize", st);
  if (p->forms.fuse_finish && pass > 0)
    return plan_linearize(p, states_of(p, pass - 1), 0, p->pb.active, st, states_of(p, pass), pass);
  return plan_linearize(p, p->pb.cur, 0, p->pb.active, st);
}

static int plan_run_impl(gpmp2mi_plan* p, hipStream_t st, const double* start, bool update) {
  const PlanParams& P = p->hp;
  const PlanForms& F = p->forms;
  PlanBuffers& pb = p->pb;
  p->timer.reset();
  for (int k = 0; k < p->n_active_len; k++) p->h_flags[k] = -1;
  G2_TRY(launch_plan_reset(P, pb, start, st));
  const int iter_cap = (P.rules.fixed_iters > 0 ? P.rules.fixed_iters : P.rules.max_iter);
  if (P.rules.opt_type == GPMP2MI_OPT_GAUSS_NEWTON && F.gn_fast(update)) {
    const int max_pass = iter_cap + 1;
    G2_TRY(enqueue_gn_lin(p, 0, st));
    for (int pass = 0; pass < max_pass; pass++) {
      G2_TRY(enqueue_gn_pass(p, pb, pass, states_of(p, pass), st));
      if (pass + 1 == max_pass) break;
      G2_TRY(enqueue_gn_lin(p, pass + 1, st));
      p->timer.close(st);
      int cnt = 0;
      G2_TRY(wait_pass_count(p->h_flags, pass, st, &cnt));
      if (cnt == 0) break;
    }
    p->timer.close(st);
  } else {
    const int max_pass = p->n_active_len - 1;
    p->timer.begin("linearize", st);
    G2_TRY(plan_linearize(p, pb.cur, 0, pb.active, st));
    p->timer.begin("decide", st);
    G2_TRY(launch_decide(P, pb, 0, true, st));
    p->timer.close(st);
    for (int pass = 1; pass < max_pass; pass++) {
      G2_TRY(enqueue_trial_pass(p, pb, st));
      p->timer.begin("decide", st);
      G2_TRY(launch_decide(P, pb, pass, false, st));
      p->timer.close(st);
      if (pass >= 2) {
        int cnt = 0;
        G2_TRY(wait_pass_count(p->h_flags, pass - 1, st, &cnt));
        if (cnt == 0) break;
      }
    }
    G2_TRY(launch_finalize_unfinished(P, pb, st));
  }
  G2_HIP(hipStreamSynchronize(st));
  if (p->timer.enabled) p->timer.collect();
  p->optimized = true;
  return GPMP2MI_OK;
}
template <class Driver>
static int guarded_run(gpmp2mi_plan* p, hipStream_t st, QueueStage* stage, Driver driver) {
  p->mark_dirty(st);
  const int rc = driver();
  if (rc == GPMP2MI_ERR_TIMEOUT) {
    p->poisoned = true;
    if (stage) stage->leak();
    return rc;
  }
  if (rc != GPMP2MI_OK) (void)hipStreamSynchronize(st);
  p->mark_clean(st);
  return rc;
}
static int plan_run(gpmp2mi_plan* p, hipStream_t st, const double* start, bool update) {
  G2_PLAN_LIVE(p);
  return guarded_run(p, st, nullptr, [&] { return plan_run_impl(p, st, start, update); });
}

static int plan_queue_impl(gpmp2mi_plan* p, hipStream_t st, QueueRun q, int* passes_out) {
  const PlanParams& P = p->hp;
  const PlanForms& F = p->forms;
  const int B = P.B;
  const bool gn = P.rules.opt_type == GPMP2MI_OPT_GAUSS_NEWTON && F.gn_fast(false);
  const int iter_cap = (P.rules.fixed_iters > 0 ? P.rules.fixed_iters : P.rules.max_iter);
  q.budget = gn ? 0 : p->n_active_len - 2;
  const long per = gn ? iter_cap + 1 : q.budget;
  const long cap_l = ((long)q.M * per + B - 1) / B + per + 2;
  G2_CHECK(cap_l <= (1L << 26), GPMP2MI_ERR_UNSUPPORTED, "too many problems for one queue run");
  const int cap = (int)cap_l;

  const size_t ints = 5 * (size_t)B + 1 + 3 * (size_t)cap;
  const size_t bytes = sizeof(long long) + ints * sizeof(int);
  G2_TRY(p->ws[p->WS_QUEUE].reserve(bytes));
  if (p->qflags.cap < cap) {
    flags_release(p->qflags);
    p->qflags = FlagBuf{};
    G2_TRY(flags_acquire(cap, &p->qflags));
  }
  q.busy = (long long*)p->ws[p->WS_QUEUE].p;
  int* w = (int*)(q.busy + 1);
  q.job = w;
  q.next = w + B;
  q.act = w + 2 * B;
  q.fresh = w + 3 * B;
  q.qpass = w + 4 * B;
  q.head = w + 5 * B;
  PlanBuffers qb = p->pb;
  qb.n_active = q.head + 1;
  qb.done = qb.n_active + cap;
  qb.host_flags = qb.done + cap;
  q.flags = p->qflags.dev;
  for (int k = 0; k < cap; k++) p->qflags.host[k] = -1;
  G2_HIP(hipMemsetAsync(qb.n_active, 0, 3 * (size_t)cap * sizeof(int), st));

  const PlanBuffers& pb = p->pb;
  p->timer.reset();
  G2_TRY(launch_queue_reset(P, qb, q, st));
  G2_TRY(launch_queue_refill(P, qb, q, pb.cur, st));
  auto refill = [&](int pass, bool load, double* states) -> int {
    p->timer.begin("queue_scan", st);
    G2_TRY(launch_queue_scan(P, qb, q, pass, load, st));
    p->timer.begin("queue_refill", st);
    return launch_queue_refill(P, qb, q, states, st);
  };
  int passes = 0;
  if (gn) {
    G2_TRY(enqueue_gn_lin(p, 0, st));
    for (int pass = 0;; pass++) {
      G2_CHECK(pass < cap, GPMP2MI_ERR_HIP, "queue run exceeded its pass bound");
      G2_TRY(enqueue_gn_pass(p, qb, pass, states_of(p, pass), st));
      const bool load = P.rules.fixed_iters == 0 || pass % (P.rules.fixed_iters + 1) == P.rules.fixed_iters;
      G2_TRY(refill(pass, load, states_of(p, pass)));
      G2_TRY(enqueue_gn_lin(p, pass + 1, st));
      p->timer.close(st);
      passes = pass + 1;
      int cnt = 0;
      G2_TRY(wait_pass_count(p->qflags.host, pass, st, &cnt));
      if (cnt == 0) break;
    }
  } else {
    for (int pass = 0;; pass++) {
      G2_CHECK(pass < cap, GPMP2MI_ERR_HIP, "queue run exceeded its pass bound");
      p->timer.begin("linearize_fresh", st);
      G2_TRY(plan_linearize(p, pb.cur, 0, q.fresh, st));
      p->timer.begin("decide_fresh", st);
      G2_TRY(launch_queue_first(P, qb, q, pass, st));
      G2_TRY(enqueue_trial_pass(p, qb, st));
      p->timer.begin("decide", st);
      G2_TRY(launch_decide(P, qb, pass, false, st));
      G2_TRY(refill(pass, true, pb.cur));
      p->timer.close(st);
      passes = pass + 1;
      if (pass >= 1) {
        int cnt = 0;
        G2_TRY(wait_pass_count(p->qflags.host, pass - 1, st, &cnt));
        if (cnt == 0) {
          passes = pass;
          break;
        }
      }
    }
  }
  G2_HIP(hipStreamSynchronize(st));
  if (p->timer.enabled) p->timer.collect();
  *passes_out = passes;
  return GPMP2MI_OK;
}

void KernelTimer::collect() {
  names.clear();
  ms.clear();
  launches.clear();
  for (size_t i = 0; i + 1 < recs.size(); i++) {
    if (!recs[i].name) continue;
    float t = 0;
    if (hipEventElapsedTime(&t, recs[i].ev, recs[i + 1].ev) != hipSuccess) continue;
    size_t k = 0;
    for (; k < names.size(); k++)
      if (names[k] == recs[i].name) break;
    if (k == names.size()) {
      names.push_back(recs[i].name);
      ms.push_back(0.0);
      launches.push_back(0);
    }
    ms[k] += t;
    launches[k] += 1;
  }
  cnames.clear();
  for (auto& s : names) cnames.push_back(s.c_str());
}

int QueueStage::alloc(int M, const QueueRun& io, int D_, size_t trow, int T_) {
  D = D_, tr = trow, T = T_;
  const size_t m = M, md = m * D, mt = m * tr;
  const size_t nd = 4 * md + mt + (io.traj ? mt : 0) + (io.final_err ? m : 0) + (io.trace ? m * T : 0);
  const size_t ni = (io.iters ? m : 0) + (io.status ? m : 0);
  G2_TRY(dev_malloc(&base, nd * sizeof(double) + ni * sizeof(int)));
  double* d = (double*)base;
  auto take = [&](size_t cnt) { double* r = d; d += cnt; return r; };
  q.M = M;
  q.start_conf = take(md); q.start_vel = take(md); q.end_conf = take(md); q.end_vel = take(md); q.init = take(mt);
  if (io.traj) q.traj = take(mt);
  if (io.final_err) q.final_err = take(m);
  if (io.trace) q.trace = take(m * T);
  int* i = (int*)d;
  if (io.iters) q.iters = i, i += m;
  if (io.status) q.status = i;
  return GPMP2MI_OK;
}
int QueueStage::upload(const QueueRun& io, size_t j, hipStream_t st, bool with_init) const {
  const size_t md = (size_t)q.M * D * sizeof(double);
  G2_HIP(hipMemcpyAsync((void*)q.start_conf, io.start_conf + j * D, md, hipMemcpyHostToDevice, st));
  G2_HIP(hipMemcpyAsync((void*)q.start_vel, io.start_vel + j * D, md, hipMemcpyHostToDevice, st));
  G2_HIP(hipMemcpyAsync((void*)q.end_conf, io.end_conf + j * D, md, hipMemcpyHostToDevice, st));
  G2_HIP(hipMemcpyAsync((void*)q.end_vel, io.end_vel + j * D, md, hipMemcpyHostToDevice, st));
  if (with_init) G2_HIP(hipMemcpyAsync((void*)q.init, io.init + j * tr, q.M * tr * sizeof(double), hipMemcpyHostToDevice, st));
  return GPMP2MI_OK;
}
int QueueStage::download(const QueueRun& io, size_t j, hipStream_t st) const {
  const size_t m = q.M;
  if (q.traj) G2_HIP(hipMemcpyAsync(io.traj + j * tr, q.traj, m * tr * sizeof(double), hipMemcpyDeviceToHost, st));
  if (q.iters) G2_HIP(hipMemcpyAsync(io.iters + j, q.iters, m * sizeof(int), hipMemcpyDeviceToHost, st));
  if (q.final_err) G2_HIP(hipMemcpyAsync(io.final_err + j, q.final_err, m * sizeof(double), hipMemcpyDeviceToHost, st));
  if (q.status) G2_HIP(hipMemcpyAsync(io.status + j, q.status, m * sizeof(int), hipMemcpyDeviceToHost, st));
  if (q.trace) G2_HIP(hipMemcpyAsync(io.trace + j * T, q.trace, m * T * sizeof(double), hipMemcpyDeviceToHost, st));
  return GPMP2MI_OK;
}

int g2::plan_set_problem(gpmp2mi_plan* p, const double* sc, const double* sv, const double* ec, const double* ev,
                         const double* init, hipMemcpyKind kind, hipStream_t st) {
  G2_CHECK(p && sc && sv && ec && ev && init, GPMP2MI_ERR_INVALID, "null argument");
  G2_PLAN_LIVE(p);
  const size_t bd = (size_t)p->hp.B * p->hp.D * sizeof(double);
  G2_HIP(hipMemcpyAsync(p->pb.start_conf, sc, bd, kind, st));
  G2_HIP(hipMemcpyAsync(p->pb.start_vel, sv, bd, kind, st));
  G2_HIP(hipMemcpyAsync(p->pb.end_conf, ec, bd, kind, st));
  G2_HIP(hipMemcpyAsync(p->pb.end_vel, ev, bd, kind, st));
  G2_HIP(hipMemcpyAsync(p->pb.init, init, p->tsz() * sizeof(double), kind, st));
  G2_TRY(p->close_copies(kind, st));
  p->problem_set = true;
  p->optimized = false;
  return GPMP2MI_OK;
}

int g2::plan_optimize_queue(gpmp2mi_plan* p, QueueRun io, bool host, hipStream_t st) {
  G2_CHECK(p, GPMP2MI_ERR_INVALID, "null plan");
  G2_CHECK(io.M >= 1, GPMP2MI_ERR_INVALID, "queue: M must be >= 1");
  G2_CHECK(io.start_conf && io.start_vel && io.end_conf && io.end_vel && io.init, GPMP2MI_ERR_INVALID, "queue: null input");
  G2_PLAN_LIVE(p);
  const PlanParams& P = p->hp;
  for (int b = 0; b < P.B; b++) {
    G2_CHECK(p->h_xp_n[b] == 0, GPMP2MI_ERR_INVALID,
             "queue: slot " + std::to_string(b) + " carries state priors (fix_state / add_state_estimate): clear them with "
             "gpmp2mi_plan_clear_state_priors first");
    G2_CHECK(!p->goal_removed[b], GPMP2MI_ERR_INVALID,
             "queue: the goal of slot " + std::to_string(b) + " was removed (remove_goal): restore it with "
             "gpmp2mi_plan_change_goal first");
  }
  QueueStage stage;
  if (host) {
    G2_TRY(stage.alloc(io.M, io, P.D, (size_t)(P.N + 1) * P.n, P.rules.max_iter + 1));
    G2_TRY(stage.upload(io, 0, st));
  }
  const QueueRun q = host ? stage.q : io;
  p->problem_set = false;
  p->optimized = false;
  p->queue_ran = false;
  int passes = 0;
  G2_TRY(guarded_run(p, st, host ? &stage : nullptr, [&] { return plan_queue_impl(p, st, q, &passes); }));
  p->qstats.passes = passes;
  p->qstats.slot_passes = (long)P.B * passes;
  G2_HIP(hipMemcpy(&p->qstats.busy_slot_passes, p->ws[p->WS_QUEUE].p, sizeof(long long), hipMemcpyDeviceToHost));
  p->queue_ran = true;
  if (host) {
    G2_TRY(stage.download(io, 0, st));
    G2_HIP(hipStreamSynchronize(st));
  }
  return GPMP2MI_OK;
}

int g2::plan_get_result(gpmp2mi_plan* p, double* traj, int* iters, double* ferr, int* status, double* trace,
                        hipMemcpyKind kind, hipStream_t st) {
  G2_CHECK(p, GPMP2MI_ERR_INVALID, "null plan");
  G2_PLAN_LIVE(p);
  G2_CHECK(p->optimized, GPMP2MI_ERR_INVALID, "plan has not been optimized");
  const int B = p->hp.B;
  if (traj) G2_HIP(hipMemcpyAsync(traj, p->pb.result, p->tsz() * sizeof(double), kind, st));
  if (iters) G2_HIP(hipMemcpyAsync(iters, p->pb.iters, B * sizeof(int), kind, st));
  if (ferr) G2_HIP(hipMemcpyAsync(ferr, p->pb.final_err, B * sizeof(double), kind, st));
  if (status) G2_HIP(hipMemcpyAsync(status, p->pb.status, B * sizeof(int), kind, st));
  if (trace)
    G2_HIP(hipMemcpyAsync(trace, p->pb.trace, (size_t)B * (p->hp.rules.max_iter + 1) * sizeof(double), kind, st));
  return p->close_copies(kind, st);
}

static int plan_add_prior(gpmp2mi_plan* p, int b, int state, const double* conf, const double* Wc, const double* vel,
                          const double* Wv) {
  G2_CHECK(p && conf && Wc, GPMP2MI_ERR_INVALID, "null argument");
  G2_CHECK(b >= 0 && b < p->hp.B && state >= 0 && state <= p->hp.N, GPMP2MI_ERR_INVALID, "index out of range");
  G2_CHECK(p->h_xp_n[b] < XP_MAX, GPMP2MI_ERR_UNSUPPORTED, "too many state priors on this trajectory");
  const int D = p->hp.D, n = p->hp.n, e = p->h_xp_n[b];
  const size_t xe = (size_t)b * XP_MAX + e;
  std::vector<double> tg(n, 0.0), info(2 * D * D, 0.0);
  std::copy(conf, conf + D, tg.begin());
  std::copy(Wc, Wc + D * D, info.begin());
  const int has_vel = (vel && Wv) ? 1 : 0;
  if (has_vel) {
    std::copy(vel, vel + D, tg.begin() + D);
    std::copy(Wv, Wv + D * D, info.begin() + D * D);
  }
  G2_HIP(hipMemcpy(p->pb.xp_target + xe * n, tg.data(), n * sizeof(double), hipMemcpyHostToDevice));
  G2_HIP(hipMemcpy(p->pb.xp_info + xe * 2 * D * D, info.data(), info.size() * sizeof(double), hipMemcpyHostToDevice));
  G2_HIP(hipMemcpy(p->pb.xp_state + xe, &state, sizeof(int), hipMemcpyHostToDevice));
  G2_HIP(hipMemcpy(p->pb.xp_has_vel + xe, &has_vel, sizeof(int), hipMemcpyHostToDevice));
  p->h_xp_n[b] = e + 1;
  G2_HIP(hipMemcpy(p->pb.xp_n + b, &p->h_xp_n[b], sizeof(int), hipMemcpyHostToDevice));
  return GPMP2MI_OK;
}

extern "C" {

int gpmp2mi_plan_set_problem(gpmp2mi_plan* p, const double* sc, const double* sv, const double* ec,
                             const double* ev, const double* init) {
  return plan_set_problem(p, sc, sv, ec, ev, init, hipMemcpyHostToDevice, nullptr);
}
int gpmp2mi_plan_set_problem_dev(gpmp2mi_plan* p, const double* sc, const double* sv, const double* ec,
                                 const double* ev, const double* init, void* stream) {
  return plan_set_problem(p, sc, sv, ec, ev, init, hipMemcpyDeviceToDevice, (hipStream_t)stream);
}

int gpmp2mi_plan_optimize(gpmp2mi_plan* p, void* stream) {
  G2_CHECK(p, GPMP2MI_ERR_INVALID, "null plan");
  G2_CHECK(p->problem_set, GPMP2MI_ERR_INVALID, "call gpmp2mi_plan_set_problem first");
  return plan_run(p, (hipStream_t)stream, p->pb.init, false);
}
int gpmp2mi_plan_get_result(gpmp2mi_plan* p, double* traj, int* iters, double* ferr, int* status, double* trace) {
  return plan_get_result(p, traj, iters, ferr, status, trace, hipMemcpyDeviceToHost, nullptr);
}
int gpmp2mi_plan_get_result_dev(gpmp2mi_plan* p, double* traj, int* iters, double* ferr, int* status, void* stream) {
  return plan_get_result(p, traj, iters, ferr, status, nullptr, hipMemcpyDeviceToDevice, (hipStream_t)stream);
}
const double* gpmp2mi_plan_traj_dev(const gpmp2mi_plan* p) { return p ? p->pb.result : nullptr; }

int gpmp2mi_plan_optimize_queue(gpmp2mi_plan* p, int M, const double* start_conf, const double* start_vel,
                                const double* end_conf, const double* end_vel, const double* init, double* traj,
                                int* iters, double* final_error, int* status, double* error_trace) {
  const QueueRun io{M, 0, start_conf, start_vel, end_conf, end_vel, init, traj, iters, final_error, status, error_trace};
  return plan_optimize_queue(p, io, true, nullptr);
}
int gpmp2mi_plan_optimize_queue_dev(gpmp2mi_plan* p, int M, const double* start_conf, const double* start_vel,
                                    const double* end_conf, const double* end_vel, const double* init, double* traj,
                                    int* iters, double* final_error, int* status, double* error_trace, void* stream) {
  const QueueRun io{M, 0, start_conf, start_vel, end_conf, end_vel, init, traj, iters, final_error, status, error_trace};
  return plan_optimize_queue(p, io, false, (hipStream_t)stream);
}
int gpmp2mi_plan_queue_stats(const gpmp2mi_plan* p, gpmp2mi_queue_stats* out) {
  G2_CHECK(p && out, GPMP2MI_ERR_INVALID, "null argument");
  G2_CHECK(p->queue_ran, GPMP2MI_ERR_INVALID, "no queue run on this plan yet");
  *out = p->qstats;
  return GPMP2MI_OK;
}

int gpmp2mi_plan_graph_error(gpmp2mi_plan* p, const double* traj, double* err) {
  G2_CHECK(p && traj && err, GPMP2MI_ERR_INVALID, "null argument");
  G2_CHECK(p->problem_set, GPMP2MI_ERR_INVALID, "call gpmp2mi_plan_set_problem first");
  DevBuf<double> dt, de;
  G2_TRY(dt.upload(traj, p->tsz()));
  G2_TRY(de.out(err, p->hp.B));
  G2_TRY(plan_linearize(p, dt.p, 1, nullptr, nullptr));
  G2_TRY(launch_error_reduce(p->hp, p->pb, dt.p, 1, de.p, nullptr));
  return fetch_all(de);
}

int gpmp2mi_plan_linearize(gpmp2mi_plan* p, const double* traj, double* Hdiag, double* Hoff, double* g, double* err) {
  G2_CHECK(p && traj, GPMP2MI_ERR_INVALID, "null argument");
  G2_CHECK(p->problem_set, GPMP2MI_ERR_INVALID, "call gpmp2mi_plan_set_problem first");
  const PlanParams& P = p->hp;
  const size_t nb = (size_t)P.B * (P.N + 1), n = P.n;
  DevBuf<double> dt, dd, dob, dg, de;
  G2_TRY(dt.upload(traj, p->tsz()));
  if (Hdiag) G2_TRY(dd.out(Hdiag, nb * n * n));
  if (Hoff) G2_TRY(dob.out(Hoff, (size_t)P.B * P.N * n * n));
  if (g) G2_TRY(dg.out(g, nb * n));
  if (err) G2_TRY(de.out(err, P.B));
  const PlanBuffers& pb = p->pb;
  G2_TRY(plan_linearize(p, dt.p, 1, nullptr, nullptr));
  G2_TRY(launch_export_normal_eq(P, pb, dt.p, 1, dd.p, dob.p, dg.p, nullptr));
  if (err) G2_TRY(launch_error_reduce(P, pb, dt.p, 1, de.p, nullptr));
  return fetch_all(dd, dob, dg, de);
}

int gpmp2mi_plan_fix_state(gpmp2mi_plan* p, int b, int state_idx, const double* conf, const double* vel) {
  G2_CHECK(p && conf && vel, GPMP2MI_ERR_INVALID, "null argument");
  const int D = p->hp.D;
  std::vector<double> Wc(D * D, 0.0), Wv(D * D, 0.0);
  for (int k = 0; k < D; k++) {
    Wc[k * D + k] = p->hp.conf_prior_w;
    Wv[k * D + k] = p->hp.vel_prior_w;
  }
  return plan_add_prior(p, b, state_idx, conf, Wc.data(), vel, Wv.data());
}

int gpmp2mi_plan_add_state_estimate(gpmp2mi_plan* p, int b, int state_idx, const double* conf, const double* conf_cov,
                                    const double* vel, const double* vel_cov) {
  G2_CHECK(p && conf && conf_cov, GPMP2MI_ERR_INVALID, "null argument");
  G2_CHECK((vel == nullptr) == (vel_cov == nullptr), GPMP2MI_ERR_INVALID, "pass vel and vel_cov together");
  const int D = p->hp.D;
  std::vector<double> Wc(D * D), Wv(D * D);
  G2_CHECK(invert_small(D, conf_cov, Wc.data()), GPMP2MI_ERR_INVALID, "pose covariance is singular");
  if (vel) G2_CHECK(invert_small(D, vel_cov, Wv.data()), GPMP2MI_ERR_INVALID, "velocity covariance is singular");
  return plan_add_prior(p, b, state_idx, conf, Wc.data(), vel, vel ? Wv.data() : nullptr);
}

int gpmp2mi_plan_change_goal(gpmp2mi_plan* p, int b, const double* goal_conf, const double* goal_vel) {
  G2_CHECK(p && goal_conf && goal_vel && b >= 0 && b < p->hp.B, GPMP2MI_ERR_INVALID, "bad argument");
  const int D = p->hp.D, one = 1;
// ... 77 lines not shown
```

### gpmp2_amd/csrc/linearize_kernels.hip

```cpp
#include "dispatch.h"
#include "device_math.h"
#include "plan.h"
#include "tiles.h"
#include "cr_schedule.h"
#include "rec_pieces.h"
#include "plan_device.h"

namespace g2 {

#ifdef G2_STAMPS
#define G2_LSTAMP(k) do { if (chunk == 1 && threadIdx.x == 0 && pb.iters[b] == G2_STAMP_ITER) pb.stamps[(size_t)b * 64 + 48 + (k)] = __builtin_amdgcn_s_memtime(); } while (0)
#else
#define G2_LSTAMP(k) do {} while (0)
#endif
template <int KIND, int AD, int AD2, int SDIM, int NSPLIT>
__global__ __launch_bounds__(64 * NSPLIT, KIND == GPMP2MI_ROBOT_ARM ? 2 : 1) void k_linearize(const RobotDev* __restrict__ Rg, SdfDev sdf,
                                                            const PlanParams* __restrict__ pp,
                                                            PlanBuffers pb, const double* __restrict__ traj,
                                                            int bufsel, const int* __restrict__ active) {
  using K = Kin<KIND, AD, AD2>;
  constexpr int D = K::DOF, n = 2 * D, NG = D * (D + 1) / 2;
  const PlanParams& P = *pp;
  const int nchunk = P.Ppad / 64;
  const int b = blockIdx.x / nchunk, chunk = blockIdx.x - b * nchunk;
  if (active && !active[b]) return;
  const int wv = __builtin_amdgcn_readfirstlane(threadIdx.x >> 6), lane = threadIdx.x & 63;
#ifdef G2_WGTIMES
  if (threadIdx.x == 0) pb.stamps[(size_t)blockIdx.x * 2] = wall_clock64();
#endif
  double* __restrict__ rec = rec_of(pb, pb.which[b], bufsel);
  double* __restrict__ gpu = gpu_of(pb, pb.which[b], bufsel);
  G2_LSTAMP(0);
  __shared__ RobotDev R;
  constexpr int NT = 64 * NSPLIT, RN = sizeof(RobotDev) / 4, RPT = (RN + NT - 1) / NT;
  int rtmp[RPT];
#pragma unroll
  for (int u = 0; u < RPT; u++) {
    const int idx = threadIdx.x + NT * u;
    rtmp[u] = idx < RN ? reinterpret_cast<const int*>(Rg)[idx] : 0;
  }
  const int p_raw = chunk * 64 + lane;
  const int p = min(p_raw, P.P - 1);
  const int N = P.N, I = P.I;
  int i = 0, j = I;
  if (p > 0) {
    const int t = p - 1;
    i = 1 + t / (I + 1);
    j = t - (i - 1) * (I + 1);
  }
  const bool unary = (j == I);
  const double* z1 = traj + ((size_t)b * (N + 1) + i) * n;
  const double* z0 = (i > 0) ? z1 - n : z1;
  double x0[D], v0[D], x1[D], v1[D], q[D];
#pragma unroll
  for (int k = 0; k < D; k++) {
    x1[k] = z1[k];
    v1[k] = z1[D + k];
    x0[k] = (i > 0) ? z0[k] : 0.0;
    v0[k] = (i > 0) ? z0[D + k] : 0.0;
  }
  if (unary) {
#pragma unroll
    for (int k = 0; k < D; k++) q[k] = x1[k];
  } else {
    const GpCoef c = P.coef[j];
    if constexpr (K::BASE == 3) {
      lie_interpolate<D>(c, x0, v0, x1, v1, q, nullptr);
    } else {
#pragma unroll
      for (int k = 0; k < D; k++) q[k] = c.l11 * x0[k] + c.l12 * v0[k] + c.p11 * x1[k] + c.p12 * v1[k];
    }
  }

#pragma unroll
  for (int u = 0; u < RPT; u++) {
    const int idx = threadIdx.x + NT * u;
    if (idx < RN) reinterpret_cast<int*>(&R)[idx] = rtmp[u];
  }
  __syncthreads();
  if (NSPLIT == 1 && p_raw >= P.P) return;
  G2_LSTAMP(1);
  double G[NG], gv[D], e = 0.0;
#pragma unroll
  for (int k = 0; k < NG; k++) G[k] = 0.0;
#pragma unroll
  for (int k = 0; k < D; k++) gv[k] = 0.0;

  if (!(P.obs_skip_first && p == 0)) {
    const double eps = P.eps;
    double hx, hy, hz, r;
    auto accumulate = [&](const double (&Jc)[D][3], auto nc) {
      constexpr int NC = decltype(nc)::value, FIRST = decltype(nc)::first, NB = K::NB;
      auto live = [](int k) { return !(k >= NB && k < FIRST); };
      double Jr[NC];
#pragma unroll
      for (int k = 0; k < NC; k++)
        Jr[k] = hx * Jc[k][0] + hy * Jc[k][1] + (SDIM == 3 ? hz * Jc[k][2] : 0.0);
      e += r * r;
#pragma unroll
      for (int k = 0; k < NC; k++) {
        if (!live(k)) continue;
        gv[k] += Jr[k] * r;
#pragma unroll
        for (int k2 = k; k2 < NC; k2++)
          if (live(k2)) G[k * D - (k * (k - 1)) / 2 + (k2 - k)] += Jr[k] * Jr[k2];
      }
    };
    K::visit_spheres(
        R, q,
        [&](int s, const double (&pt)[3]) {
          if (s < 11) G2_LSTAMP(2 + s);
          r = hinge_obstacle<SDIM>(sdf, pt[0], pt[1], pt[2], R.sph_r[s] + eps, hx, hy, hz);
          return !(hx == 0.0 && hy == 0.0 && hz == 0.0 && r == 0.0);
        },
        [&](int, const double (&)[3], const double (&Jc)[D][3], auto nc) { accumulate(Jc, nc); }, wv, NSPLIT);
  }
  if constexpr (NSPLIT > 1) {
    static_assert(NSPLIT == 2, "two wavefronts per point set");
    constexpr int RV = NG + D + 1;
    __shared__ double part[RV][64];
    if (wv == 1) {
#pragma unroll
      for (int k = 0; k < NG; k++) part[k][lane] = G[k];
#pragma unroll
      for (int k = 0; k < D; k++) part[NG + k][lane] = gv[k];
      part[NG + D][lane] = e;
    }
    __syncthreads();
    if (wv == 0) {
#pragma unroll
      for (int k = 0; k < NG; k++) G[k] += part[k][lane];
#pragma unroll
      for (int k = 0; k < D; k++) gv[k] += part[NG + k][lane];
      e += part[NG + D][lane];
    }
  }
  const bool store_ok = (NSPLIT == 1) || (p_raw < P.P);
  G2_LSTAMP(13);
  const double w = P.obs_w;
  if (NSPLIT == 1 || wv == 0) {
    constexpr int RECL = NG + D + 1 + (K::BASE == 3 ? 36 : 0);
    double rv[RECL + 1];
#pragma unroll
    for (int k = 0; k < NG; k++) rv[k] = G[k] * w;
#pragma unroll
    for (int k = 0; k < D; k++) rv[NG + k] = gv[k] * w;
    rv[NG + D] = e * w;
    if constexpr (K::BASE == 3) {
      double Mlie[4][9];
#pragma unroll
      for (int m = 0; m < 4; m++)
#pragma unroll
        for (int t = 0; t < 9; t++) Mlie[m][t] = 0.0;
      if (!unary) {
        double a0[D], b0[D], a1[D], b1[D], qq[D];
#pragma unroll
        for (int k = 0; k < D; k++) {
          a1[k] = z1[k];
          b1[k] = z1[D + k];
          a0[k] = z0[k];
          b0[k] = z0[D + k];
        }
        lie_interpolate<D>(P.coef[j], a0, b0, a1, b1, qq, Mlie);
      }
#pragma unroll
      for (int m = 0; m < 4; m++)
#pragma unroll
        for (int t = 0; t < 9; t++) rv[NG + D + 1 + m * 9 + t] = Mlie[m][t];
    }
    rv[RECL] = 0.0;
    double2* rb = reinterpret_cast<double2*>(rec + ((size_t)b * P.Ppad + p) * P.RECS);
    const int nst = P.RECS >> 1;
#pragma unroll
    for (int k = 0; k < (RECL + 1) / 2; k++)
      if (k < nst && store_ok) rb[k] = double2{rv[2 * k], rv[2 * k + 1]};
  }

  G2_LSTAMP(14);
  if (unary && i > 0 && store_ok && (NSPLIT == 1 || wv == NSPLIT - 1)) {
    double rx[D], rv[D], sx[D], sv[D];
    double* gb = gpu + ((size_t)b * P.Npad + i) * P.GPS;
    if constexpr (NSPLIT > 1) {
#pragma unroll
      for (int k = 0; k < D; k++) {
        x1[k] = z1[k];
        v1[k] = z1[D + k];
        x0[k] = z0[k];
        v0[k] = z0[D + k];
      }
    }
    if constexpr (K::BASE == 3) {
      const P2 p1{x0[0], x0[1], x0[2]}, p2{x1[0], x1[1], x1[2]};
      const P2 bt = pose2_between(p1, p2);
      double lg[3], Hinv[9], Hc1[9], Hlog[9], T[9], J1[9];
      pose2_logmap(bt, lg);
      pose2_adjoint(p1, Hinv);
      pose2_adjoint(pose2_inverse(p2), Hc1);
      pose2_logmap_derivative(bt, Hlog);
      mat3_mul(Hlog, Hc1, T);
      mat3_mul(T, Hinv, J1);
#pragma unroll
      for (int k = 0; k < 9; k++) {
        gb[n + 1 + k] = -J1[k];
        gb[n + 1 + 9 + k] = Hlog[k];
      }
#pragma unroll
      for (int k = 0; k < D; k++) {
        const double r = (k < 3) ? lg[k] : (x1[k] - x0[k]);
        rx[k] = r - v0[k] * P.delta_t;
        rv[k] = v1[k] - v0[k];
      }
    } else {
#pragma unroll
      for (int k = 0; k < D; k++) {
        rx[k] = x0[k] + P.delta_t * v0[k] - x1[k];
        rv[k] = v0[k] - v1[k];
      }
    }
#pragma unroll
    for (int k = 0; k < D; k++) {
      double ax = 0, av = 0;
#pragma unroll
      for (int m = 0; m < D; m++) {
        ax += P.Qc_inv[k * D + m] * rx[m];
        av += P.Qc_inv[k * D + m] * rv[m];
      }
      sx[k] = ax;
      sv[k] = av;
    }
    double en = 0.0;
#pragma unroll
    for (int k = 0; k < D; k++) {
      const double ux = P.Winv[0] * sx[k] + P.Winv[1] * sv[k];
      const double uv = P.Winv[2] * sx[k] + P.Winv[3] * sv[k];
      gb[k] = ux;
      gb[D + k] = uv;
      en += rx[k] * ux + rv[k] * uv;
    }
    gb[n] = en;
  }
  G2_LSTAMP(15);
#ifdef G2_WGTIMES
  if (threadIdx.x == 0) pb.stamps[(size_t)blockIdx.x * 2 + 1] = wall_clock64();
#endif
}

template <int AD, int SDIM, int NW>
__global__ __launch_bounds__(64 * NW, 3) void k_linearize_arm(const RobotDev* __restrict__ Rg, SdfDev sdf,
                                                               const PlanParams* __restrict__ pp, PlanBuffers pb,
                                                               const double* __restrict__ traj, int bufsel,
                                                               const int* __restrict__ active, double* __restrict__ dst,
                                                               int pass, int trial) {
  static_assert(NW == 4, "tree reduction below");
  constexpr int D = AD, n = 2 * D, NG = D * (D + 1) / 2, RV = NG + D + 1;
  constexpr int FR = 9;
  constexpr int ROWS_F = FR * AD, ROWS_SC = 2 * AD;
  constexpr int ROWS_P = (NW / 2) * rec_lds_stride(RV);
  constexpr int ROWS = (ROWS_F + ROWS_SC > ROWS_P) ? ROWS_F + ROWS_SC : ROWS_P;
  const PlanParams& P = *pp;
  const int nchunk = P.Ppad / 64;
  const int b = blockIdx.x / nchunk, chunk = blockIdx.x - b * nchunk;
  if (active && !active[b]) return;
  const int wv = __builtin_amdgcn_readfirstlane(threadIdx.x >> 6), lane = threadIdx.x & 63;
  double* __restrict__ rec = rec_of(pb, pb.which[b], bufsel);
  double* __restrict__ gpu = gpu_of(pb, pb.which[b], bufsel);
  G2_LSTAMP(0);
  __shared__ RobotDev R;
  __shared__ double buf[ROWS][64];
  constexpr int NT = 64 * NW, RN = sizeof(RobotDev) / 4, RPT = (RN + NT - 1) / NT;
  int rtmp[RPT];
#pragma unroll
  for (int u = 0; u < RPT; u++) {
    const int idx = threadIdx.x + NT * u;
    rtmp[u] = idx < RN ? reinterpret_cast<const int*>(Rg)[idx] : 0;
  }
  const int p_raw = chunk * 64 + lane;
  const int p = min(p_raw, P.P - 1);
  const int N = P.N, I = P.I;
  int i = 0, j = I;
  if (p > 0) {
    const int t = p - 1;
    i = 1 + t / (I + 1);
    j = t - (i - 1) * (I + 1);
  }
  const bool unary = (j == I);
  const bool store_ok = p_raw < P.P;
  double (*fx)[16] = reinterpret_cast<double (*)[16]>(&buf[0][0]);
  static_assert(FXS * 16 <= ROWS * 64, "the step window lives in the frame buffer");
  __shared__ double zn[ZNS][n];
  const int p_lo = chunk * 64, p_hi = min(p_lo + 63, P.P - 1);
  auto state_of = [&](int pt) { return pt == 0 ? 0 : 1 + (pt - 1) / (I + 1); };
  const int s1 = state_of(p_hi), s0 = max(0, state_of(p_lo) - 1), ns = s1 - s0 + 1;
  const bool apply = dst != nullptr && pb.stepped[b] == pass;
  const bool shares = bufsel == 0 && !trial;
  double* __restrict__ cshare = pb.cshare + ((size_t)b * nchunk + chunk) * 3;
  if (apply) {
    const double* fac = pb.fac + (size_t)b * (N + 1) * 3 * TILE_DBL;
    const double* xg = pb.xg + (size_t)b * (N + 1) * 16;
    const int w0 = (s0 + 1) & ~7, M = N + 1, c = lane & 15, g = lane >> 4;
    using u64 = unsigned long long;
    const CrrWindow win = crr_window(N, s0, s1, FXS);
    const u64 need1 = win.need1, need2 = win.need2, need4 = win.need4, need8 = win.need8;
    for (u64 m = need8; m; m &= m - 1) {
      const int k = __builtin_ctzll(m);
      if (wv == ((k >> 3) & (NW - 1)) && lane < 16) fx[k][lane] = xg[(size_t)(w0 + k - 1) * 16 + lane];
    }
    __syncthreads();
    auto level = [&](u64 need, int h) {
      int t = 0;
      for (u64 m = need; m; m &= m - 1, t++) {
        if ((t & (NW - 1)) != wv) continue;
        const int k = __builtin_ctzll(m), vb = w0 + k;
        const double* f = fac + (size_t)(vb - 1) * 3 * TILE_DBL;
        const Tile Wl = tile_load_rows<n>(f, lane), Wr = tile_load_rows<n>(f + TILE_DBL, lane);
        const Tile V = load_v<n>(f + 2 * TILE_DBL, h, N, lane);
        const double xl = (vb - h >= 1) ? fx[k - h][c] : 0.0;
        const double xr = (vb + h <= M) ? fx[k + h][c] : 0.0;
        const double x = cr_backsolve<n>(Wl, Wr, V, xl, xr, lane);
        if (g == 0) fx[k][c] = (c < n) ? x : 0.0;
      }
      __syncthreads();
    };
    level(need4, 4);
    level(need2, 2);
    level(need1, 1);
  }
  double s_gd = 0.0, s_dd = 0.0, s_gg = 0.0;
  for (int e = threadIdx.x; e < ns * n; e += 64 * NW) {
    const int t = e / n, rho = e - t * n, st = s0 + t;
    const size_t k = ((size_t)b * (N + 1) + st) * n + rho;
    double z = traj[k];
    const double x = apply ? fx[st + 1 - ((s0 + 1) & ~7)][rho] : 0.0;
    z += x;
    zn[t][rho] = z;
    const int pu = st * (I + 1);
    if (dst != nullptr && pu >= p_lo && pu <= p_lo + 63) {
      dst[k] = z;
      if (trial && apply) {
        const double gk = pb.gvec[((size_t)b * (N + 1) + st) * 16 + rho];
        pb.delta[k] = x;
        s_gd = fma(gk, x, s_gd);
        s_dd = fma(x, x, s_dd);
        s_gg = fma(gk, gk, s_gg);
      }
    }
  }
  if (trial && apply) {
    __shared__ double psum[NW][3];
    s_gd = wave_sum(s_gd);
    s_dd = wave_sum(s_dd);
    s_gg = wave_sum(s_gg);
    if (lane == 0) {
      psum[wv][0] = s_gd;
      psum[wv][1] = s_dd;
      psum[wv][2] = s_gg;
    }
    __syncthreads();
    if (threadIdx.x < 3) {
      double a = 0.0;
#pragma unroll
      for (int w = 0; w < NW; w++) a += psum[w][threadIdx.x];
      pb.spart[((size_t)b * nchunk + chunk) * 3 + threadIdx.x] = a;
    }
  }
  __syncthreads();
  const double* z1 = &zn[i - s0][0];
  const double* z0 = (i > 0) ? z1 - n : z1;
  {
    double q[D];
    if (unary) {
#pragma unroll
      for (int k = 0; k < D; k++) q[k] = z1[k];
    } else {
      const GpCoef c = P.coef[j];
#pragma unroll
      for (int k = 0; k < D; k++) q[k] = c.l11 * z0[k] + c.l12 * z0[D + k] + c.p11 * z1[k] + c.p12 * z1[D + k];
    }
#pragma unroll
    for (int k = 0; k < AD; k++) {
      if (k % NW != wv) continue;
      double sn, cs;
      sincos(q[k] + Rg->bias[k], &sn, &cs);
      buf[ROWS_F + 2 * k][lane] = sn;
      buf[ROWS_F + 2 * k + 1][lane] = cs;
    }
  }
#pragma unroll
  for (int u = 0; u < RPT; u++) {
    const int idx = threadIdx.x + NT * u;
    if (idx < RN) reinterpret_cast<int*>(&R)[idx] = rtmp[u];
  }
  __syncthreads();
  G2_LSTAMP(1);
  if (wv == 0) {
    Frame F;
    frame_from_3x4(R.base, F);
    static_for<0, AD>([&](auto jc) {
      constexpr int k = decltype(jc)::value;
      const double sn = buf[ROWS_F + 2 * k][lane], cs = buf[ROWS_F + 2 * k + 1][lane];
      dh_advance_sc(F, sn, cs, R.a[k], R.d[k], R.ca[k], R.sa[k]);
#pragma unroll
      for (int t = 0; t < 3; t++) {
        buf[FR * k + t][lane] = F.c0[t];
        buf[FR * k + 3 + t][lane] = F.c2[t];
        buf[FR * k + 6 + t][lane] = F.t[t];
      }
    });
  } else if (wv == 1 && shares) {
    const int nxp = pb.xp_n[b];
    const bool every_state = misc_every_state(P, nxp);
    double acc = 0.0;
    for (int e = lane; e < ns * n; e += 64) {
      const int t = e / n, rho = e - t * n, st = s0 + t;
      const int pu = st * (I + 1);
      if (pu < p_lo || pu > p_lo + 63 || !(every_state || st == 0 || st == N)) continue;
      acc = misc_entry_add<false>(acc, P, pb, b, nxp, st, rho, &zn[t][0]);
    }
    acc = wave_sum(acc);
    if (lane == 0) cshare[2] = acc;
  } else if (wv == 2) {
    double en = 0.0;
    if (unary && i > 0 && store_ok) {
      double rx[D], rv[D], sx[D], sv[D];
      double* gb = gpu + ((size_t)b * P.Npad + i) * P.GPS;
#pragma unroll
      for (int k = 0; k < D; k++) {
        rx[k] = z0[k] + P.delta_t * z0[D + k] - z1[k];
        rv[k] = z0[D + k] - z1[D + k];
      }
#pragma unroll
      for (int k = 0; k < D; k++) {
        double ax = 0, av = 0;
#pragma unroll
        for (int m = 0; m < D; m++) {
          ax += P.Qc_inv[k * D + m] * rx[m];
          av += P.Qc_inv[k * D + m] * rv[m];
        }
        sx[k] = ax;
        sv[k] = av;
      }
#pragma unroll
      for (int k = 0; k < D; k++) {
        const double ux = P.Winv[0] * sx[k] + P.Winv[1] * sv[k];
        const double uv = P.Winv[2] * sx[k] + P.Winv[3] * sv[k];
        gb[k] = ux;
        gb[D + k] = uv;
        en += rx[k] * ux + rv[k] * uv;
      }
      gb[n] = en;
    }
    if (shares) {
      const double gs = wave_sum(en);
      if (lane == 0) cshare[1] = gs;
    }
  }
  __syncthreads();
  G2_LSTAMP(2);
  double G[NG], gv[D], e = 0.0;
#pragma unroll
  for (int k = 0; k < NG; k++) G[k] = 0.0;
#pragma unroll
  for (int k = 0; k < D; k++) gv[k] = 0.0;
  if (!(P.obs_skip_first && p == 0)) {
    const double eps = P.eps;
    static_for<0, AD>([&](auto jc) {
      constexpr int L = decltype(jc)::value, NC = L + 1;
      for (int s = R.link_first[L]; s < R.link_first[L + 1]; s++) {
        if (s % NW != wv) continue;
        double c0[3], c2[3], o[3], pt[3];
#pragma unroll
        for (int t = 0; t < 3; t++) {
          c0[t] = buf[FR * L + t][lane];
          c2[t] = buf[FR * L + 3 + t][lane];
          o[t] = buf[FR * L + 6 + t][lane];
        }
        const double c1[3] = {c2[1] * c0[2] - c2[2] * c0[1], c2[2] * c0[0] - c2[0] * c0[2], c2[0] * c0[1] - c2[1] * c0[0]};
        const double cx = R.sph_c[3 * s], cy = R.sph_c[3 * s + 1], cz = R.sph_c[3 * s + 2];
#pragma unroll
        for (int t = 0; t < 3; t++) pt[t] = o[t] + c0[t] * cx + c1[t] * cy + c2[t] * cz;
        double hx, hy, hz;
        const double r = hinge_obstacle<SDIM>(sdf, pt[0], pt[1], pt[2], R.sph_r[s] + eps, hx, hy, hz);
        if (hx == 0.0 && hy == 0.0 && hz == 0.0 && r == 0.0) continue;
        double Jr[NC];
#pragma unroll
        for (int k = 0; k < NC; k++) {
          double zx, zy, zz, ox, oy, oz;
          if (k == 0) {
            zx = R.base[2]; zy = R.base[6]; zz = R.base[10];
            ox = R.base[3]; oy = R.base[7]; oz = R.base[11];
          } else {
            zx = buf[FR * (k - 1) + 3][lane]; zy = buf[FR * (k - 1) + 4][lane]; zz = buf[FR * (k - 1) + 5][lane];
            ox = buf[FR * (k - 1) + 6][lane]; oy = buf[FR * (k - 1) + 7][lane]; oz = buf[FR * (k - 1) + 8][lane];
          }
          const double rx = pt[0] - ox, ry = pt[1] - oy, rz = pt[2] - oz;
          const double Jx = zy * rz - zz * ry, Jy = zz * rx - zx * rz, Jz = zx * ry - zy * rx;
          Jr[k] = hx * Jx + hy * Jy + (SDIM == 3 ? hz * Jz : 0.0);
        }
        e += r * r;
#pragma unroll
        for (int k = 0; k < NC; k++) {
          gv[k] += Jr[k] * r;
#pragma unroll
          for (int k2 = k; k2 < NC; k2++) G[k * D - (k * (k - 1)) / 2 + (k2 - k)] += Jr[k] * Jr[k2];
        }
      }
    });
  }
  G2_LSTAMP(3);
  __syncthreads();
  constexpr int RECL = RV, RVP = rec_lds_stride(RECL), SLOT = 64 * RVP;
  static_assert(2 * SLOT <= ROWS * 64, "two partial records fit in the frame buffer");
  double* const part = &buf[0][0];
  auto put = [&](int slot) {
    double* q = part + slot * SLOT + lane * RVP;
#pragma unroll
    for (int k = 0; k < NG; k++) q[k] = G[k];
#pragma unroll
    for (int k = 0; k < D; k++) q[NG + k] = gv[k];
    q[NG + D] = e;
  };
  auto add = [&](int slot) {
    const double* q = part + slot * SLOT + lane * RVP;
#pragma unroll
    for (int k = 0; k < NG; k++) G[k] += q[k];
#pragma unroll
    for (int k = 0; k < D; k++) gv[k] += q[NG + k];
    e += q[NG + D];
  };
  if (wv >= 2) put(wv - 2);
  __syncthreads();
  if (wv < 2) {
    add(wv);
    put(wv);
  }
  __syncthreads();
  G2_LSTAMP(13);
  const double w = P.obs_w;
  {
    const int npc = rec_piece_count(rec_live_points(P.P, p_lo), RECL);
    double* rchunk = rec + ((size_t)b * P.Ppad + p_lo) * P.RECS;
    constexpr int NIT = (64 * rec_npieces(RECL) + 64 * NW - 1) / (64 * NW);
#pragma unroll
    for (int it = 0; it < NIT; it++) {
      const int pe = threadIdx.x + 64 * NW * it;
      if (pe < npc) {
        const RecPiece pc = rec_piece(pe, RECL, P.RECS);
        const double* a = part + pc.src;
        const double v0 = (a[0] + a[SLOT]) * w;
        const double v1 = pc.padded ? 0.0 : (a[1] + a[SLOT + 1]) * w;
        *reinterpret_cast<double2*>(rchunk + pc.dst) = double2{v0, v1};
      }
    }
  }
  if (wv == 0 && shares) {
    const double es = wave_sum(store_ok ? (e + part[SLOT + lane * RVP + NG + D]) * w : 0.0);
    if (lane == 0) cshare[0] = es;
  }
  G2_LSTAMP(14);
  G2_LSTAMP(15);
}

int launch_linearize(const RobotDev& h, const RobotDev* robot, const SdfDev& sdf, const PlanParams& hp,
                     const PlanBuffers& pb, const double* traj, int bufsel, const int* active,
                     hipStream_t st, double* dst, int pass, bool trial) {
  if (dst != nullptr && !(hp.fuse_finish && hp.lin_split == 4)) {
    set_error("fused finish asked of a plan that was not set up for it");
    return GPMP2MI_ERR_INVALID;
  }
  if (hp.lin_split == 4 && chunk_states(hp.I) > ZNS) {
    set_error("the four-wavefront linearization needs obs_check_inter >= 2");
    return GPMP2MI_ERR_INVALID;
  }
  const dim3 grid(hp.B * (hp.Ppad / 64));
  if (hp.lin_split == 4) {
    const dim3 block(256);
    if (sdf.dim == 3) {
      G2_DISPATCH_ROBOT_ARM_ONLY(h.arm_dof, (k_linearize_arm<AD_, 3, 4><<<grid, block, 0, st>>>(robot, sdf, pb.params, pb, traj, bufsel, active, dst, pass, trial ? 1 : 0)));
    } else {
      G2_DISPATCH_ROBOT_ARM_ONLY(h.arm_dof, (k_linearize_arm<AD_, 2, 4><<<grid, block, 0, st>>>(robot, sdf, pb.params, pb, traj, bufsel, active, dst, pass, trial ? 1 : 0)));
    }
  } else if (hp.lin_split == 2) {
    const dim3 block(128);
    if (sdf.dim == 3) {
      G2_DISPATCH_ROBOT_ARM_ONLY(h.arm_dof, (k_linearize<GPMP2MI_ROBOT_ARM, AD_, 0, 3, 2><<<grid, block, 0, st>>>(robot, sdf, pb.params, pb, traj, bufsel, active)));
    } else {
      G2_DISPATCH_ROBOT_ARM_ONLY(h.arm_dof, (k_linearize<GPMP2MI_ROBOT_ARM, AD_, 0, 2, 2><<<grid, block, 0, st>>>(robot, sdf, pb.params, pb, traj, bufsel, active)));
    }
  } else {
    const dim3 block(64);
    if (sdf.dim == 3) {
      G2_DISPATCH_ROBOT_H(h, (k_linearize<KIND_, AD_, AD2_, 3, 1><<<grid, block, 0, st>>>(robot, sdf, pb.params, pb, traj, bufsel, active)));
    } else {
      G2_DISPATCH_ROBOT_H(h, (k_linearize<KIND_, AD_, AD2_, 2, 1><<<grid, block, 0, st>>>(robot, sdf, pb.params, pb, traj, bufsel, active)));
    }
  }
  G2_HIP(hipGetLastError());
  return GPMP2MI_OK;
}

}
```

### gpmp2_amd/csrc/plan.h

```cpp
#pragma once
#include <cstdint>

#include "common.h"
#include "step_control.h"

namespace g2 {

constexpr int MAXI = 16;
constexpr int TILE = 16;
constexpr int XP_MAX = GPMP2MI_MAX_STATE_PRIORS;

struct PlanParams {
  int B, N, I, P, Ppad, D, n, NG, REC, Npad, GPREC;
  int RECS, GPS;
  int max_pass;
  int obs_skip_first, flag_pos_limit, flag_vel_limit, lie;
  int lin_split;
  int end_conf_prior_off;
  int wide;
  int split_back;
  int spart_groups;
  int wide_h0;
  int fuse_finish;
  double eps, obs_w, delta_t;
  double conf_prior_w, vel_prior_w;
  double vdyn_w;
  StepRules rules;
  alignas(16) GpCoef coef[MAXI];
  alignas(16) double coefq[MAXI][24];
  double Winv[4];
  double Qc_inv[MAXD * MAXD];
  double pos_lo[MAXD], pos_hi[MAXD], pos_th[MAXD], pos_w[MAXD];
  double vel_lim[MAXD], vel_th[MAXD], vel_w[MAXD];
  double KA[4 * MAXD * MAXD], KB[4 * MAXD * MAXD], KO[4 * MAXD * MAXD];
};

struct SelfPairRec {
  double total_eps, w;
  int a, b;
};

struct PlanExtras {
  int n_ws, n_sc, sc_first, sc_last;
  int ws_mode[GPMP2MI_MAX_WORKSPACE_FACTORS], ws_link[GPMP2MI_MAX_WORKSPACE_FACTORS];
  int ws_first[GPMP2MI_MAX_WORKSPACE_FACTORS], ws_last[GPMP2MI_MAX_WORKSPACE_FACTORS];
  double ws_w[GPMP2MI_MAX_WORKSPACE_FACTORS];
  double sc_w[GPMP2MI_MAX_SELF_COLLISION_PAIRS];
  double* des;
  double* sc_data;
  double* radius;
  double* poses;
  double* Jp;
  double* ws_err;
  double* ws_H;
  double* cen;
  double* Jc;
  double* sc_err;
  double* sc_H;
  int mv_cap, mv_K, mv_first, mv_last;
  double mv_eps, mv_w;
  double* mv_radius;
  double* mv_centers;
  int wp_cap, wp_mode, wp_link, wp_n;
  double* wp_des;
  double* wp_sigma;
  int* wp_list;
  int* wp_count;
  int sp_cap, sp_P, sp_first, sp_last;
  SelfPairRec* sp_rec;
  int cr_cap, cr_A, cr_link, cr_first, cr_last;
  double cr_eps, cr_w;
  double* cr_radius;
  double* cr_centers;
};

struct PlanBuffers {
  PlanParams* params;
  double* start_conf;
  double* start_vel;
  double* end_conf;
  double* end_vel;
  double* cur;
  double* last;
  double* trial;
  double* init;
  double* result;
  double* rec;
  double* rec2;
  double* gpu;
  double* gpu2;
  double* tiles;
  double* fac;
  double* pend;
  double* coup;
  double* delta;
  double* gvec;
  double* htiles;
  double* hgpart;
  double* scal;
  int* xp_n;
  int* xp_state;
  int* xp_has_vel;
  double* xp_target;
  double* xp_info;
  int* goal_on;
  double* wHd;
  double* wHo;
  double* wg;
  double* wWl;
  double* wWr;
  double* wy;
  double* wrb;
  double* wx;
  double* xg;
  int* stepped;
  double* spart;
  int* which;
  double* cur_err;
  double* prev_err;
  double* last_err;
  double* final_err;
  double* lambda;
  double* trace;
  int* iters;
  int* status;
  int* active;
  int* phase;
  int* notspd;
  double* epart;
  double* cshare;
  int* n_active;
  int* done;
  int* host_flags;
  unsigned long long* stamps;
};

struct QueueRun {
  int M;
  int budget;
  const double* start_conf;
  const double* start_vel;
  const double* end_conf;
  const double* end_vel;
  const double* init;
  double* traj;
  int* iters;
  double* final_err;
  int* status;
  double* trace;
  int* job;
  int* next;
  int* act;
  int* fresh;
  int* qpass;
  int* head;
  long long* busy;
  int* flags;
};

enum { SC_GD = 0, SC_DD, SC_GG, SC_GHG, SC_GN, SC_NN, SC_Q, SC_XNORM, SC_ZERO_STEP, SC_COUNT = 16 };

__host__ __device__ inline double* rec_of(const PlanBuffers& pb, int which_b, int sel) {
  return (which_b ^ sel) ? pb.rec2 : pb.rec;
}
__host__ __device__ inline double* gpu_of(const PlanBuffers& pb, int which_b, int sel) {
  return (which_b ^ sel) ? pb.gpu2 : pb.gpu;
}

int launch_linearize(const RobotDev& hrobot, const RobotDev* robot, const SdfDev& sdf,
                     const PlanParams& hp, const PlanBuffers& pb, const double* traj, int bufsel,
                     const int* active, hipStream_t st, double* dst = nullptr, int pass = 0, bool trial = false);
int launch_extra_accumulate(const PlanParams& hp, const PlanBuffers& pb, const PlanExtras& ex, int L, int S, int bufsel,
                            const int* active, hipStream_t st);
int launch_moving_accumulate(const PlanParams& hp, const PlanBuffers& pb, const PlanExtras& ex, int S, int bufsel,
                             const int* active, hipStream_t st);
int launch_selfpair_accumulate(const PlanParams& hp, const PlanBuffers& pb, const PlanExtras& ex, int S, int bufsel,
                               const int* active, hipStream_t st);
int launch_path_accumulate(const RobotDev& h, const RobotDev* R, const PlanParams& hp, const PlanBuffers& pb,
                           const PlanExtras& ex, const double* traj, int bufsel, const int* active, hipStream_t st);
int launch_carried_accumulate(const RobotDev& h, const RobotDev* R, const SdfDev& s, const PlanParams& hp,
                              const PlanBuffers& pb, const PlanExtras& ex, const double* traj, int bufsel,
                              const int* active, hipStream_t st);
int launch_set_mode(const PlanBuffers& pb, int opt_type, int fixed_iters, hipStream_t st);
int launch_error_parts(const PlanParams& hp, const PlanBuffers& pb, const double* traj, int bufsel, const int* active,
                       hipStream_t st);
int launch_plan_reset(const PlanParams& hp, const PlanBuffers& pb, const double* start, hipStream_t st);
int launch_assemble(const PlanParams& hp, const PlanBuffers& pb, const double* traj, int bufsel,
                    const int* active, hipStream_t st, bool early_stop = false);
int launch_solve_step(const PlanParams& hp, const PlanBuffers& pb, hipStream_t st);
int launch_ghg(const PlanParams& hp, const PlanBuffers& pb, hipStream_t st);
int launch_decide(const PlanParams& hp, const PlanBuffers& pb, int pass, bool init, hipStream_t st);
int launch_finalize_unfinished(const PlanParams& hp, const PlanBuffers& pb, hipStream_t st);
int launch_queue_reset(const PlanParams& hp, const PlanBuffers& pb, const QueueRun& q, hipStream_t st);
int launch_queue_first(const PlanParams& hp, const PlanBuffers& pb, const QueueRun& q, int pass, hipStream_t st);
int launch_queue_scan(const PlanParams& hp, const PlanBuffers& pb, const QueueRun& q, int pass, bool load, hipStream_t st);
int launch_queue_refill(const PlanParams& hp, const PlanBuffers& pb, const QueueRun& q, double* states, hipStream_t st);
int launch_debug_crosslane(const double* in, double* out, hipStream_t st);
int launch_gn_step_cr(const PlanParams& hp, const PlanBuffers& pb, int pass, hipStream_t st, bool early_stop = false);
int launch_finish_step(const PlanParams& hp, const PlanBuffers& pb, int pass, hipStream_t st);
int launch_finish_trial(const PlanParams& hp, const PlanBuffers& pb, hipStream_t st);
int launch_solve_dense(const PlanParams& hp, const PlanBuffers& pb, hipStream_t st);
int launch_assemble_wide(const PlanParams& hp, const PlanBuffers& pb, const double* traj, int bufsel,
                         const int* active, hipStream_t st);
int launch_ghg_wide(const PlanParams& hp, const PlanBuffers& pb, hipStream_t st);
int launch_solve_step_wide(const PlanParams& hp, const PlanBuffers& pb, hipStream_t st);
int launch_finish_trial_wide(const PlanParams& hp, const PlanBuffers& pb, hipStream_t st);
int launch_cr_level_wide(const PlanParams& hp, const PlanBuffers& pb, int h, hipStream_t st);
int launch_error_reduce(const PlanParams& hp, const PlanBuffers& pb, const double* traj, int bufsel,
                        double* err, hipStream_t st);
int launch_export_normal_eq(const PlanParams& hp, const PlanBuffers& pb, const double* traj, int bufsel,
                            double* Hdiag, double* Hoff, double* g, hipStream_t st, const int* active = nullptr);
int launch_block_tridiag_solve(int B, int nblk, int n, const double* Hd, const double* Ho,
                               const double* b, double* x, int* ok, double* scratch, hipStream_t st);
struct PosteriorArgs {
  int nblk, K;
  const double *Hd, *Ho;
  const double* z;
  double *Sd, *So;
  double* delta;
  int* ok;
  double* fac;
};
int launch_posterior(int B, int n, const PosteriorArgs& a, hipStream_t st);
struct NormalFillArgs {
  uint64_t seed;
  uint32_t stream;
  int a_first, a_count, b_first, b_count, nblk, n;
  double* out;
};
int launch_normal_fill(const NormalFillArgs& a, hipStream_t st);
struct SeedSampleArgs {
  uint64_t seed;
  uint32_t stream;
  int nblk, count;
  int a_first, b_first;
  const double* fac;
  double* out;
  double scale;
  int keep_first, D;
  const double* mean;
  const double *start_conf, *end_conf;
};
int launch_sample_seeded(int systems, int n, bool shared, const SeedSampleArgs& a, hipStream_t st);

}
```

### gpmp2_amd/csrc/plan_device.h

```cpp
#pragma once
#include "device_math.h"
#include "plan.h"
#include "tiles.h"

namespace g2 {

template <bool MAYBE_LIE = true>
__device__ __forceinline__ double misc_entry_add(double acc, const PlanParams& P, const PlanBuffers& pb, int b, int nxp,
                                                 int i, int rho, const double* __restrict__ zs) {
  const int D = P.D, n = P.n, N = P.N;
  const bool lie = MAYBE_LIE && P.lie;
  const int a = rho >= D, k = rho - a * D;
  const double z = zs[rho];
  if (i == 0 || (i == N && pb.goal_on[b] && (a || !P.end_conf_prior_off))) {
    const double* tg = (i == 0) ? (a ? pb.start_vel : pb.start_conf) : (a ? pb.end_vel : pb.end_conf);
    tg += (size_t)b * D;
    double d = z - tg[k];
    if (lie && !a && k < 3) {
      const P2 bt = pose2_between(P2{zs[0], zs[1], zs[2]}, P2{tg[0], tg[1], tg[2]});
      d = -(k == 0 ? bt.x : k == 1 ? bt.y : bt.th);
    }
    acc += (a ? P.vel_prior_w : P.conf_prior_w) * d * d;
  }
  for (int e = 0; e < nxp; e++) {
    const size_t xe = (size_t)b * XP_MAX + e;
    if (pb.xp_state[xe] != i || (a && !pb.xp_has_vel[xe])) continue;
    const double* Wm = pb.xp_info + (xe * 2 + a) * D * D + (size_t)k * D;
    const double* tg = pb.xp_target + xe * n + a * D;
    double wr = 0.0, rk = 0.0;
    for (int cc = 0; cc < D; cc++) {
      double rc = zs[a * D + cc] - tg[cc];
      if (lie && !a && cc < 3) {
        const P2 bt = pose2_between(P2{zs[0], zs[1], zs[2]}, P2{tg[0], tg[1], tg[2]});
        rc = -(cc == 0 ? bt.x : cc == 1 ? bt.y : bt.th);
      }
      wr = fma(Wm[cc], rc, wr);
      if (cc == k) rk = rc;
    }
    acc += wr * rk;
  }
  double H;
  if (!a && P.flag_pos_limit && !(lie && k < 3)) {
    const double e = hinge_limit(z, P.pos_lo[k], P.pos_hi[k], P.pos_th[k], H);
    acc += P.pos_w[k] * e * e;
  }
  if (a && P.flag_vel_limit) {
    const double e = hinge_limit(z, -P.vel_lim[k], P.vel_lim[k], P.vel_th[k], H);
    acc += P.vel_w[k] * e * e;
  }
  if (a && k == 1 && P.vdyn_w > 0.0) acc += P.vdyn_w * z * z;
  return acc;
}
__device__ __forceinline__ bool misc_every_state(const PlanParams& P, int nxp) {
  return P.flag_pos_limit || P.flag_vel_limit || P.vdyn_w > 0.0 || nxp > 0;
}
__device__ __forceinline__ double misc_error_partial(const PlanParams& P, const PlanBuffers& pb, int b,
                                                     const double* __restrict__ tr, int tid, int nthr) {
  const int n = P.n, N = P.N;
  double acc = 0.0;
  const int nxp = pb.xp_n[b];
  const bool every_state = misc_every_state(P, nxp);
  const int count = every_state ? (N + 1) * n : (N > 0 ? 2 * n : n);
  for (int q = tid; q < count; q += nthr) {
    const int idx = (every_state || q < n) ? q : N * n + (q - n);
    const int i = idx / n, rho = idx - i * n;
    acc = misc_entry_add(acc, P, pb, b, nxp, i, rho, tr + (size_t)i * n);
  }
  return acc;
}
__device__ __forceinline__ double misc_error(const PlanParams& P, const PlanBuffers& pb, int b,
                                             const double* __restrict__ tr, int lane) {
  return wave_sum(misc_error_partial(P, pb, b, tr, lane, 64));
}

__device__ __forceinline__ double total_error(const PlanParams& P, const PlanBuffers& pb, int b,
                                              const double* __restrict__ tr,
                                              const double* __restrict__ rec,
                                              const double* __restrict__ gpu, int lane) {
  const double* eb = rec + (size_t)b * P.Ppad * P.RECS + (P.NG + P.D);
  double acc = 0.0;
  for (int p = lane; p < P.P; p += 64) acc += eb[(size_t)p * P.RECS];
  const double* gb = gpu + (size_t)b * P.Npad * P.GPS + P.n;
  for (int i = 1 + lane; i <= P.N; i += 64) acc += gb[(size_t)i * P.GPS];
  return 0.5 * (wave_sum(acc) + misc_error(P, pb, b, tr, lane));
}

__device__ __forceinline__ double total_error_partial(const PlanParams& P, const PlanBuffers& pb, int b,
                                                      const double* __restrict__ tr, const double* __restrict__ rec,
                                                      const double* __restrict__ gpu, int tid, int nthr) {
  const double* eb = rec + (size_t)b * P.Ppad * P.RECS + (P.NG + P.D);
  double acc = 0.0;
  for (int p = tid; p < P.P; p += nthr) acc += eb[(size_t)p * P.RECS];
  const double* gb = gpu + (size_t)b * P.Npad * P.GPS + P.n;
  for (int i = 1 + tid; i <= P.N; i += nthr) acc += gb[(size_t)i * P.GPS];
  return acc + misc_error_partial(P, pb, b, tr, tid, nthr);
}

__device__ __forceinline__ bool dogleg_retry(const PlanParams& P, const PlanBuffers& pb, int b) {
  return P.rules.opt_type == GPMP2MI_OPT_DOGLEG && pb.phase[b] != 0;
}

__device__ __forceinline__ double error_from_shares(const PlanParams& P, const PlanBuffers& pb, int b) {
  const int nchunk = P.Ppad / 64;
  const double* __restrict__ cs = pb.cshare + (size_t)b * nchunk * 3;
  double acc = 0.0;
  for (int q = 0; q < nchunk; q++) acc += (cs[3 * q] + cs[3 * q + 1]) + cs[3 * q + 2];
  return 0.5 * acc;
}


template <int WAVES>
__device__ __forceinline__ double block_sum(double v, double* red, int tid) {
  v = wave_sum(v);
  __syncthreads();
  if ((tid & 63) == 0) red[tid >> 6] = v;
  __syncthreads();
  double t = 0.0;
  for (int k = 0; k < WAVES; k++) t += red[k];
  return t;
}

template <int WAVES, int X>
__device__ __forceinline__ void trial_step_tail(const PlanParams& P, const PlanBuffers& pb, int b, int n, int D,
                                                bool resolve, const double* xsrc, double* xs, const double* gv,
                                                double* red, int tid, int nthr) {
  const size_t tsz = (size_t)(P.N + 1) * n;
  const double* cur = pb.cur + b * tsz;
  double* trial = pb.trial + b * tsz;
  double* delta = pb.delta + b * tsz;
  double* sc = pb.scal + (size_t)b * SC_COUNT;
  const int xstride = X ? X : n;
  auto off = [&](size_t k) -> size_t {
    if constexpr (X == 0) {
      return k;
    } else {
      const int i = (int)(k / n), rho = (int)(k - (size_t)i * n);
      return i * X + rho;
    }
  };
  if (resolve) {
    double gd = 0.0, dd = 0.0, gg = 0.0;
    for (size_t k = tid; k < tsz; k += nthr) {
      const size_t o = off(k);
      const double x = xsrc[o], gk = gv[o];
      if constexpr (X == 0) xs[o] = x;
      delta[k] = x;
      gd = fma(gk, x, gd);
      dd = fma(x, x, dd);
      gg = fma(gk, gk, gg);
    }
    gd = block_sum<WAVES>(gd, red, tid);
    dd = block_sum<WAVES>(dd, red, tid);
    gg = block_sum<WAVES>(gg, red, tid);
    if (tid == 0) {
      sc[SC_GD] = gd;
      sc[SC_DD] = dd;
      sc[SC_GG] = gg;
      sc[SC_GN] = gd;
      sc[SC_NN] = dd;
    }
    __syncthreads();
  }
  const bool dogleg = P.rules.opt_type == GPMP2MI_OPT_DOGLEG;
  double q = 0.0, xn = 0.0;
  if (dogleg) {
    double cu, cn;
    dogleg_blend(sc[SC_GG], sc[SC_GHG], sc[SC_GN], sc[SC_NN], pb.lambda[b], cu, cn, q);
    __syncthreads();
    for (size_t k = tid; k < tsz; k += nthr) {
      const size_t o = off(k);
      const double x = cu * gv[o] + cn * delta[k];
      xs[o] = x;
      xn = fma(x, x, xn);
    }
    __syncthreads();
  }
  for (size_t k = tid; k < tsz; k += nthr) {
    const int i = (int)(k / n), rho = (int)(k - (size_t)i * n);
    const double* zs = cur + (size_t)i * n;
    const double* dz = xs + i * xstride;
    trial[k] = (rho < D) ? retract_coord(P.lie != 0, rho, zs, dz) : zs[rho] + dz[rho];
  }
  if (!dogleg) return;
  xn = block_sum<WAVES>(xn, red, tid);
  if (tid == 0) {
    sc[SC_Q] = q;
    sc[SC_XNORM] = sqrt(xn);
  }
}

__device__ __forceinline__ void publish_pass_count(const PlanBuffers& pb, int pass) {
  __threadfence();
  if (atomicAdd(pb.done + pass, 1) == (int)gridDim.x - 1) {
    const int v = atomicAdd(pb.n_active + pass, 0);
    __hip_atomic_store(pb.host_flags + pass, v, __ATOMIC_RELEASE, __HIP_MEMORY_SCOPE_SYSTEM);
  }
}

}
```

### gpmp2_amd/csrc/plan_kernels.hip

```cpp
#include "device_math.h"
#include "dispatch.h"
#include "plan.h"
#include "tiles.h"
#include "assembler.h"
#include "cr_schedule.h"
#include "plan_device.h"

namespace g2 {

__global__ __launch_bounds__(64) void k_extra_accumulate(const PlanParams* __restrict__ pp, PlanBuffers pb, PlanExtras ex,
                                                          int bufsel, const int* __restrict__ active) {
  const PlanParams& P = *pp;
  const int N = P.N, D = P.D, M = P.B * (N + 1);
  const int m = blockIdx.x * blockDim.x + threadIdx.x;
  if (m >= M) return;
  const int b = m / (N + 1), i = m - b * (N + 1);
  if (active && !active[b]) return;
  double* rec = rec_of(pb, pb.which[b], bufsel) + ((size_t)b * P.Ppad + (size_t)i * (P.I + 1)) * P.RECS;
  auto add_rows = [&](const double* err, const double* H, int rows, const double* w, double wu) {
    double e = 0.0;
    for (int r = 0; r < rows; r++) e += (w ? w[r] : wu) * err[r] * err[r];
    rec[P.NG + D] += e;
    for (int k = 0; k < D; k++) {
      double g = 0.0;
      for (int r = 0; r < rows; r++) g += (w ? w[r] : wu) * H[r * D + k] * err[r];
      rec[P.NG + k] += g;
      for (int k2 = k; k2 < D; k2++) {
        double a = 0.0;
        for (int r = 0; r < rows; r++) a += (w ? w[r] : wu) * H[r * D + k] * H[r * D + k2];
        rec[k * D - (k * (k - 1)) / 2 + (k2 - k)] += a;
      }
    }
  };
  for (int f = 0; f < ex.n_ws; f++) {
    if (i < ex.ws_first[f] || i > ex.ws_last[f]) continue;
    const int rows = ex.ws_mode[f] == GPMP2MI_WORKSPACE_POSE ? 6 : 3;
    add_rows(ex.ws_err + (size_t)f * M * 6 + (size_t)m * rows, ex.ws_H + ((size_t)f * M * 6 + (size_t)m * rows) * D, rows,
             nullptr, ex.ws_w[f]);
  }
  if (ex.n_sc > 0 && i >= ex.sc_first && i <= ex.sc_last)
    add_rows(ex.sc_err + (size_t)m * ex.n_sc, ex.sc_H + (size_t)m * ex.n_sc * D, ex.n_sc, ex.sc_w, 0.0);
}

int launch_extra_accumulate(const PlanParams& hp, const PlanBuffers& pb, const PlanExtras& ex, int L, int S, int bufsel,
                            const int* active, hipStream_t st) {
  const int M = hp.B * (hp.N + 1);
  k_extra_accumulate<<<dim3((M + 63) / 64), dim3(64), 0, st>>>(pb.params, pb, ex, bufsel, active);
  G2_HIP(hipGetLastError());
  return GPMP2MI_OK;
}

__global__ __launch_bounds__(64) void k_error_reduce(const PlanParams* __restrict__ pp, PlanBuffers pb,
                                                      const double* __restrict__ traj, int bufsel,
                                                      double* __restrict__ err) {
  const PlanParams& P = *pp;
  const int b = blockIdx.x, lane = threadIdx.x;
  const double e = total_error(P, pb, b, traj + (size_t)b * (P.N + 1) * P.n, rec_of(pb, pb.which[b], bufsel),
                               gpu_of(pb, pb.which[b], bufsel), lane);
  if (lane == 0) err[b] = e;
}

int launch_error_reduce(const PlanParams& hp, const PlanBuffers& pb, const double* traj, int bufsel,
                        double* err, hipStream_t st) {
  k_error_reduce<<<dim3(hp.B), dim3(64), 0, st>>>(pb.params, pb, traj, bufsel, err);
  G2_HIP(hipGetLastError());
  return GPMP2MI_OK;
}


__global__ __launch_bounds__(256) void k_error_parts(const PlanParams* __restrict__ pp, PlanBuffers pb,
                                                      const double* __restrict__ traj, int bufsel,
                                                      const int* __restrict__ active) {
  const PlanParams& P = *pp;
  const int b = blockIdx.x, tid = threadIdx.x;
  if (active && !active[b]) return;
  __shared__ double red[4];
  const double part = total_error_partial(P, pb, b, traj + (size_t)b * (P.N + 1) * P.n, rec_of(pb, pb.which[b], bufsel),
                                          gpu_of(pb, pb.which[b], bufsel), tid, 256);
  const double ws = wave_sum(part);
  if ((tid & 63) == 0) red[tid >> 6] = ws;
  __syncthreads();
  const double e = 0.5 * (((red[0] + red[1]) + red[2]) + red[3]);
  for (int i = tid; i <= P.N; i += 256) pb.epart[(size_t)b * P.Npad + i] = (i == 0) ? e : 0.0;
}

int launch_error_parts(const PlanParams& hp, const PlanBuffers& pb, const double* traj, int bufsel, const int* active,
                       hipStream_t st) {
  k_error_parts<<<dim3(hp.B), dim3(256), 0, st>>>(pb.params, pb, traj, bufsel, active);
  G2_HIP(hipGetLastError());
  return GPMP2MI_OK;
}

__global__ void k_set_mode(PlanParams* pp, int opt_type, int fixed_iters) {
  pp->rules.opt_type = opt_type;
  pp->rules.fixed_iters = fixed_iters;
}
int launch_set_mode(const PlanBuffers& pb, int opt_type, int fixed_iters, hipStream_t st) {
  k_set_mode<<<dim3(1), dim3(1), 0, st>>>(pb.params, opt_type, fixed_iters);
  G2_HIP(hipGetLastError());
  return GPMP2MI_OK;
}

__device__ __forceinline__ void reset_slot(const PlanParams& P, const PlanBuffers& pb, size_t b) {
  pb.iters[b] = 0;
  pb.status[b] = GPMP2MI_TRAJ_MAX_ITER;
  pb.active[b] = 1;
  pb.phase[b] = 0;
  pb.which[b] = 0;
  pb.stepped[b] = 0;
  pb.notspd[b] = 0;
  pb.cur_err[b] = pb.prev_err[b] = pb.last_err[b] = pb.final_err[b] = 0.0;
  pb.lambda[b] = (P.rules.opt_type == GPMP2MI_OPT_DOGLEG) ? P.rules.dl_delta0 : P.rules.lm_lambda0;
}

__global__ __launch_bounds__(256) void k_plan_reset(const PlanParams* __restrict__ pp, PlanBuffers pb,
                                                    const double* __restrict__ start) {
  const PlanParams& P = *pp;
  const size_t tid = (size_t)blockIdx.x * blockDim.x + threadIdx.x, nth = (size_t)gridDim.x * blockDim.x;
  const size_t B = P.B;
  if (start) {
    const size_t tot = B * (size_t)(P.N + 1) * P.n;
    for (size_t k = tid; k < tot; k += nth) pb.cur[k] = start[k];
  }
  for (size_t k = tid; k < (size_t)P.max_pass; k += nth) pb.n_active[k] = pb.done[k] = 0;
  for (size_t k = tid; k < B * SC_COUNT; k += nth) pb.scal[k] = 0.0;
  for (size_t k = tid; k < B * (size_t)(P.rules.max_iter + 1); k += nth) pb.trace[k] = __longlong_as_double(0x7ff8000000000000LL);
  for (size_t b = tid; b < B; b += nth) reset_slot(P, pb, b);
}

int launch_plan_reset(const PlanParams& hp, const PlanBuffers& pb, const double* start, hipStream_t st) {
  const size_t tot = (size_t)hp.B * (hp.N + 1) * hp.n;
  const int blocks = (int)std::min<size_t>(1024, std::max<size_t>(1, (tot + 1023) / 1024));
  k_plan_reset<<<dim3(blocks), dim3(256), 0, st>>>(pb.params, pb, start);
  G2_HIP(hipGetLastError());
  return GPMP2MI_OK;
}

__device__ __forceinline__ void decide_body(const PlanParams& P, const PlanBuffers& pb, int pass, int init) {
  const int b = blockIdx.x, tid = threadIdx.x, lane = tid & 63;
  const bool w0 = tid < 64;
  __shared__ int dec[2];
  __shared__ double red[4];
  if (!pb.active[b]) return;
  const int N = P.N, n = P.n;
  const size_t tsz = (size_t)(N + 1) * n;
  double* cur = pb.cur + b * tsz;
  double* last = pb.last + b * tsz;
  double* trial = pb.trial + b * tsz;
  double* result = pb.result + b * tsz;
  double* sc = pb.scal + (size_t)b * SC_COUNT;
  double* tr = pb.trace + (size_t)b * (P.rules.max_iter + 1);
  const int wh = pb.which[b];
  int action = 0, accept = 0;

  constexpr int PF = 10;
  double pf_cur[PF], pf_trial[PF];
#pragma unroll
  for (int m = 0; m < PF; m++) {
    const size_t k = tid + (size_t)m * 256;
    pf_cur[m] = (k < tsz) ? cur[k] : 0.0;
    pf_trial[m] = (!init && k < tsz) ? trial[k] : 0.0;
  }

  const bool failed = !init && pb.notspd[b] != 0;
  double err_sum = 0.0;
  if (!failed) {
    const double part = init ? total_error_partial(P, pb, b, cur, rec_of(pb, wh, 0), gpu_of(pb, wh, 0), tid, blockDim.x)
                             : total_error_partial(P, pb, b, trial, rec_of(pb, wh, 1), gpu_of(pb, wh, 1), tid, blockDim.x);
    const double ws = wave_sum(part);
    if (lane == 0) red[tid >> 6] = ws;
  }
  __syncthreads();
  if (!failed) err_sum = 0.5 * (((red[0] + red[1]) + red[2]) + red[3]);
  if (w0 && init) {
    const double err = err_sum;
    if (lane == 0) {
      pb.cur_err[b] = pb.prev_err[b] = err;
      tr[0] = err;
      int status;
      action = first_decide(P.rules, err, status);
      if (action) {
        pb.status[b] = status;
        pb.final_err[b] = err;
      }
    }
  } else if (w0) {
    const double new_err = err_sum;
    const int opt = P.rules.opt_type;
    double sp_gd = 0.0, sp_dd = 0.0, sp_gg = 0.0;
    if (P.split_back && opt == GPMP2MI_OPT_LM && !failed) {
      const int groups = P.spart_groups;
      const double* sp = pb.spart + (size_t)b * groups * 3;
      for (int qq = lane; qq < groups; qq += 64) {
        sp_gd += sp[3 * qq];
        sp_dd += sp[3 * qq + 1];
        sp_gg += sp[3 * qq + 2];
      }
      sp_gd = wave_sum(sp_gd);
      sp_dd = wave_sum(sp_dd);
      sp_gg = wave_sum(sp_gg);
    }
    if (lane == 0) {
      pb.notspd[b] = 0;
      const double cur_err = pb.cur_err[b];
      TrialOutcome o;
      if (opt == GPMP2MI_OPT_GAUSS_NEWTON) {
        o = gn_iterate(failed);
      } else if (opt == GPMP2MI_OPT_LM) {
        if (P.split_back && !failed) {
          sc[SC_GD] = sp_gd;
          sc[SC_DD] = sp_dd;
          sc[SC_GG] = sp_gg;
        }
        o = lm_try_lambda(P.rules, pb.lambda[b], cur_err, new_err, sc[SC_GD], sc[SC_DD], failed);
        pb.lambda[b] = o.param;
      } else {
        o = dogleg_iterate(pb.lambda[b], cur_err, new_err, sc[SC_Q], sc[SC_XNORM], failed);
        if (!failed) {
          pb.lambda[b] = o.param;
          pb.phase[b] = o.retry ? 1 : 0;
        }
      }
      if (o.not_spd) {
        action = 1;
        pb.status[b] = GPMP2MI_TRAJ_NOT_SPD;
        pb.final_err[b] = cur_err;
      }
      if (o.returned) {
        const double err_after = o.moved ? new_err : cur_err;
        const bool counted = o.moved || opt == GPMP2MI_OPT_DOGLEG;
        const int it = pb.iters[b] + (counted ? 1 : 0);
        pb.iters[b] = it;
        if (o.moved) accept = 1;
        const int call = (opt == GPMP2MI_OPT_LM) ? ++pb.phase[b] : it;
        if (call <= P.rules.max_iter) tr[call] = err_after;
        const double prev = pb.prev_err[b];
        int status;
        action = loop_decide(P.rules, it, counted, prev, err_after, status);
        if (action) {
          pb.status[b] = status;
          pb.final_err[b] = (action == 2) ? prev : err_after;
        } else if (P.rules.fixed_iters == 0) {
          pb.prev_err[b] = err_after;
        }
        pb.cur_err[b] = err_after;
      }
    }
  }
  if (tid == 0) {
    dec[0] = action;
    dec[1] = accept;
  }
  __syncthreads();
  action = dec[0];
  accept = dec[1];
  if (accept) {
    if (action == 2) {
#pragma unroll
      for (int m = 0; m < PF; m++) {
        const size_t k = tid + (size_t)m * 256;
        if (k < tsz) result[k] = pf_cur[m];
      }
      for (size_t k = tid + (size_t)PF * 256; k < tsz; k += 256) result[k] = cur[k];
    } else {
#pragma unroll
      for (int m = 0; m < PF; m++) {
        const size_t k = tid + (size_t)m * 256;
        if (k < tsz) {
          last[k] = pf_cur[m];
          cur[k] = pf_trial[m];
          if (action == 1) result[k] = pf_trial[m];
        }
      }
      for (size_t k = tid + (size_t)PF * 256; k < tsz; k += 256) {
        const double t = trial[k];
        last[k] = cur[k];
        cur[k] = t;
        if (action == 1) result[k] = t;
      }
      if (tid == 0) pb.which[b] = wh ^ 1;
    }
  } else if (action == 1) {
#pragma unroll
    for (int m = 0; m < PF; m++) {
      const size_t k = tid + (size_t)m * 256;
      if (k < tsz) result[k] = pf_cur[m];
    }
    for (size_t k = tid + (size_t)PF * 256; k < tsz; k += 256) result[k] = cur[k];
  } else if (action == 2) {
    for (size_t k = tid; k < tsz; k += blockDim.x) result[k] = last[k];
  }
  if (tid == 0) {
    if (action != 0) pb.active[b] = 0;
    else atomicAdd(pb.n_active + pass, 1);
  }
}
__global__ __launch_bounds__(256) void k_decide(const PlanParams* __restrict__ pp, PlanBuffers pb, int pass, int init) {
  decide_body(*pp, pb, pass, init);
  if (threadIdx.x == 0) publish_pass_count(pb, pass);
}

int launch_decide(const PlanParams& hp, const PlanBuffers& pb, int pass, bool init, hipStream_t st) {
  k_decide<<<dim3(hp.B), dim3(256), 0, st>>>(pb.params, pb, pass, init ? 1 : 0);
  G2_HIP(hipGetLastError());
  return GPMP2MI_OK;
}

__global__ __launch_bounds__(256) void k_finalize_unfinished(const PlanParams* __restrict__ pp, PlanBuffers pb) {
  const PlanParams& P = *pp;
  const int b = blockIdx.x;
  if (!pb.active[b]) return;
  const size_t tsz = (size_t)(P.N + 1) * P.n;
  for (size_t k = threadIdx.x; k < tsz; k += blockDim.x) pb.result[b * tsz + k] = pb.cur[b * tsz + k];
  if (threadIdx.x == 0) {
    pb.status[b] = GPMP2MI_TRAJ_MAX_ITER;
    pb.final_err[b] = pb.cur_err[b];
    pb.active[b] = 0;
  }
}
int launch_finalize_unfinished(const PlanParams& hp, const PlanBuffers& pb, hipStream_t st) {
  k_finalize_unfinished<<<dim3(hp.B), dim3(256), 0, st>>>(pb.params, pb);
  G2_HIP(hipGetLastError());
  return GPMP2MI_OK;
}

__global__ __launch_bounds__(256) void k_queue_reset(const PlanParams* __restrict__ pp, PlanBuffers pb, QueueRun q) {
  const int B = pp->B;
  for (int b = threadIdx.x; b < B; b += blockDim.x) {
    q.job[b] = -1;
    q.act[b] = 0;
    q.next[b] = b < q.M ? b : -1;
    q.fresh[b] = 0;
    q.qpass[b] = 0;
    pb.active[b] = 0;
  }
  if (threadIdx.x == 0) {
    *q.head = min(q.M, B);
    *q.busy = 0;
  }
}
int launch_queue_reset(const PlanParams& hp, const PlanBuffers& pb, const QueueRun& q, hipStream_t st) {
  k_queue_reset<<<dim3(1), dim3(256), 0, st>>>(pb.params, pb, q);
  G2_HIP(hipGetLastError());
  return GPMP2MI_OK;
}

__global__ __launch_bounds__(256) void k_queue_first(const PlanParams* __restrict__ pp, PlanBuffers pb,
                                                     const int* __restrict__ fresh, int pass) {
  if (!fresh[blockIdx.x]) return;
  decide_body(*pp, pb, pass, 1);
}
int launch_queue_first(const PlanParams& hp, const PlanBuffers& pb, const QueueRun& q, int pass, hipStream_t st) {
  k_queue_first<<<dim3(hp.B), dim3(256), 0, st>>>(pb.params, pb, q.fresh, pass);
  G2_HIP(hipGetLastError());
  return GPMP2MI_OK;
}

__global__ __launch_bounds__(256) void k_queue_scan(const PlanParams* __restrict__ pp, PlanBuffers pb, QueueRun q, int pass,
                                                    int load) {
  constexpr int NT = 256;
  const int B = pp->B, tid = threadIdx.x;
  const int per = (B + NT - 1) / NT, b0 = min(B, tid * per), b1 = min(B, b0 + per);
  const int head = *q.head;
  int elig = 0, still = 0, busy = 0;
  for (int b = b0; b < b1; b++) {
    const int j = q.job[b];
    int a = 0;
    if (j >= 0) {
      busy++;
      if (!pb.active[b]) {
        a = 1;
      } else if (q.budget > 0) {
        const int qp = q.qpass[b] + 1;
        q.qpass[b] = qp;
        if (qp >= q.budget) a = 2;
      }
      if (!a) still++;
    }
    q.act[b] = a;
    if (a || j < 0) elig++;
  }
  __shared__ int scan[NT];
  __shared__ int sums[2];
  if (tid == 0) sums[0] = sums[1] = 0;
  scan[tid] = elig;
  __syncthreads();
  if (still) atomicAdd(&sums[0], still);
  if (busy) atomicAdd(&sums[1], busy);
  for (int d = 1; d < NT; d *= 2) {
    const int v = (tid >= d) ? scan[tid - d] : 0;
    __syncthreads();
    scan[tid] += v;
    __syncthreads();
  }
  int r = scan[tid] - elig;
  for (int b = b0; b < b1; b++) {
    int nj = -1;
    if (q.act[b] || q.job[b] < 0) {
      if (load && head + r < q.M) nj = head + r;
      r++;
    }
    q.next[b] = nj;
  }
  if (tid == 0) {
    const int loaded = load ? min(scan[NT - 1], q.M - head) : 0;
    *q.head = head + loaded;
    *q.busy += sums[1];
    __hip_atomic_store(q.flags + pass, sums[0] + loaded + (q.M - head - loaded), __ATOMIC_RELEASE, __HIP_MEMORY_SCOPE_SYSTEM);
  }
}
int launch_queue_scan(const PlanParams& hp, const PlanBuffers& pb, const QueueRun& q, int pass, bool load, hipStream_t st) {
  k_queue_scan<<<dim3(1), dim3(256), 0, st>>>(pb.params, pb, q, pass, load ? 1 : 0);
  G2_HIP(hipGetLastError());
  return GPMP2MI_OK;
}

__global__ __launch_bounds__(256) void k_queue_refill(const PlanParams* __restrict__ pp, PlanBuffers pb, QueueRun q,
                                                      double* __restrict__ states) {
  const PlanParams& P = *pp;
  const int b = blockIdx.x, tid = threadIdx.x;
  const int a = q.act[b], nj = q.next[b];
  if (!a && nj < 0) {
    if (tid == 0) q.fresh[b] = 0;
    return;
  }
  const int D = P.D, T = P.rules.max_iter + 1;
  const size_t tsz = (size_t)(P.N + 1) * P.n;
  if (a) {
    const size_t j = q.job[b];
    const double* src = (a == 2 ? pb.cur : pb.result) + b * tsz;
    if (q.traj)
      for (size_t k = tid; k < tsz; k += blockDim.x) q.traj[j * tsz + k] = src[k];
    if (q.trace)
      for (int k = tid; k < T; k += blockDim.x) q.trace[j * T + k] = pb.trace[(size_t)b * T + k];
    if (tid == 0) {
      if (q.iters) q.iters[j] = pb.iters[b];
      if (q.status) q.status[j] = (a == 2) ? GPMP2MI_TRAJ_MAX_ITER : pb.status[b];
      if (q.final_err) q.final_err[j] = (a == 2) ? pb.cur_err[b] : pb.final_err[b];
      pb.active[b] = 0;
    }
    __syncthreads();
  }
  if (nj < 0) {
    if (tid == 0) {
      q.job[b] = -1;
      q.fresh[b] = 0;
    }
    return;
  }
  const size_t jn = nj;
  if (tid < D) {
    pb.start_conf[(size_t)b * D + tid] = q.start_conf[jn * D + tid];
    pb.start_vel[(size_t)b * D + tid] = q.start_vel[jn * D + tid];
    pb.end_conf[(size_t)b * D + tid] = q.end_conf[jn * D + tid];
    pb.end_vel[(size_t)b * D + tid] = q.end_vel[jn * D + tid];
  }
  for (size_t k = tid; k < tsz; k += blockDim.x) states[b * tsz + k] = q.init[jn * tsz + k];
  for (int k = tid; k < SC_COUNT; k += blockDim.x) pb.scal[(size_t)b * SC_COUNT + k] = 0.0;
  for (int k = tid; k < T; k += blockDim.x) pb.trace[(size_t)b * T + k] = __longlong_as_double(0x7ff8000000000000LL);
  if (tid == 0) {
    reset_slot(P, pb, b);
    q.job[b] = nj;
    q.fresh[b] = 1;
    q.qpass[b] = 0;
  }
}
int launch_queue_refill(const PlanParams& hp, const PlanBuffers& pb, const QueueRun& q, double* states, hipStream_t st) {
  k_queue_refill<<<dim3(hp.B), dim3(256), 0, st>>>(pb.params, pb, q, states);
  G2_HIP(hipGetLastError());
  return GPMP2MI_OK;
}

template <int D, bool LIE>
__global__ __launch_bounds__(64) void k_export_normal_eq(const PlanParams* __restrict__ pp, PlanBuffers pb,
                                                          const double* __restrict__ traj, int bufsel,
                                                          double* __restrict__ Hd, double* __restrict__ Ho,
                                                          double* __restrict__ gout, const int* __restrict__ active) {
  constexpr int n = 2 * D;
  using Asm = Assembler<D, LIE>;
  const PlanParams& P = *pp;
  const int N = P.N;
  const int b = blockIdx.x / (N + 1), i = blockIdx.x - b * (N + 1);
  if (active && (!active[b] || dogleg_retry(P, pb, b))) return;
  const int lane = threadIdx.x, c = lane & 15, g = lane >> 4;
  extern __shared__ __attribute__((aligned(16))) double asm_smem[];
  Asm as(P, pb, rec_of(pb, pb.which[b], bufsel), gpu_of(pb, pb.which[b], bufsel), b, lane);
  const typename Asm::Slot slot0 = as.make_slot(asm_smem, 0), slot1 = as.make_slot(asm_smem, 1);
  as.stage2(i, slot0, slot1);
  __syncthreads();
  constexpr int T = (n <= 15) ? 1 : (n <= 31) ? 2 : 3, RC = 16 * T - 1;
  const double* zi = traj + ((size_t)b * (N + 1) + i) * n;
  for (int ti = 0; ti < T; ti++)
    for (int tj = 0; tj < T; tj++) {
      Asm at(P, pb, rec_of(pb, pb.which[b], bufsel), gpu_of(pb, pb.which[b], bufsel), b, lane, 16 * ti, 16 * tj, RC);
      Tile S, Cl, Cr;
      at.build_tiles(i, slot0, slot1, zi, S, Cl, Cr, true);
      const int cc = 16 * tj + c;
#pragma unroll
      for (int k = 0; k < 4; k++) {
        const int rho = 16 * ti + g + 4 * k;
        if (rho < n && cc < n) {
          if (Hd) Hd[(((size_t)b * (N + 1) + i) * n + rho) * n + cc] = S.r[k];
          if (Ho && i < N) Ho[(((size_t)b * N + i) * n + cc) * n + rho] = Cr.r[k];
        }
        if (rho < n && cc == RC && gout) gout[((size_t)b * (N + 1) + i) * n + rho] = -S.r[k];
      }
    }
}

int launch_export_normal_eq(const PlanParams& hp, const PlanBuffers& pb, const double* traj, int bufsel,
                            double* Hd, double* Ho, double* g, hipStream_t st, const int* active) {
  const dim3 grid(hp.B * (hp.N + 1)), block(64);
  const size_t shmem = 2 * (size_t)((hp.I + 1) * hp.RECS + hp.GPS + 24 * hp.I) * sizeof(double);
  switch (hp.D) {
#define G2_EXP_CASE(DD) \
  case DD:                                                                                          \
    if (hp.lie) k_export_normal_eq<DD, true><<<grid, block, shmem, st>>>(pb.params, pb, traj, bufsel, Hd, Ho, g, active); \
    else k_export_normal_eq<DD, false><<<grid, block, shmem, st>>>(pb.params, pb, traj, bufsel, Hd, Ho, g, active);       \
    break;
    G2_EXP_CASE(1) G2_EXP_CASE(2) G2_EXP_CASE(3) G2_EXP_CASE(4) G2_EXP_CASE(5) G2_EXP_CASE(6) G2_EXP_CASE(7)
    G2_EXP_CASE(8) G2_EXP_CASE(9) G2_EXP_CASE(10) G2_EXP_CASE(11) G2_EXP_CASE(17) G2_EXP_CASE(18)
#undef G2_EXP_CASE
    default:
      set_error("normal equations are instantiated for dof <= 11 and 17, 18");
      return GPMP2MI_ERR_UNSUPPORTED;
  }
  G2_HIP(hipGetLastError());
  return GPMP2MI_OK;
}

template <int n>
__global__ __launch_bounds__(64) void k_block_tridiag_solve(int nblk, const double* __restrict__ Hd,
                                                             const double* __restrict__ Ho,
                                                             const double* __restrict__ rhs,
                                                             double* __restrict__ x, int* __restrict__ okf,
                                                             double* __restrict__ scratch) {
  const int b = blockIdx.x, lane = threadIdx.x, c = lane & 15, g = lane >> 4;
  const double* D_ = Hd + (size_t)b * nblk * n * n;
  const double* O_ = Ho + (size_t)b * (nblk - 1) * n * n;
  const double* r_ = rhs + (size_t)b * nblk * n;
  const bool ok = chain_solve<n>(
      nblk,
      [&](int i, Tile& Dt, Tile& Wt) {
#pragma unroll
        for (int k = 0; k < 4; k++) {
          const int rho = g + 4 * k;
          double d = 0.0, h = 0.0;
          if (rho < n && c < n) {
            d = D_[((size_t)i * n + rho) * n + c];
            if (i + 1 < nblk) h = O_[((size_t)i * n + c) * n + rho];
          }
          if (rho < n && c == RHSCOL) h = r_[(size_t)i * n + rho];
          Dt.r[k] = d;
          Wt.r[k] = h;
        }
      },
      scratch + (size_t)b * nblk * 512, x + (size_t)b * nblk * n, lane);
  if (lane == 0 && okf) okf[b] = ok ? 1 : 0;
}

int launch_block_tridiag_solve(int B, int nblk, int n, const double* Hd, const double* Ho, const double* b,
                               double* x, int* ok, double* scratch, hipStream_t st) {
  const dim3 grid(B), block(64);
  switch (n) {
#define G2_SOLVE_CASE(NN) \
  case NN: k_block_tridiag_solve<NN><<<grid, block, 0, st>>>(nblk, Hd, Ho, b, x, ok, scratch); break;
    G2_SOLVE_CASE(1) G2_SOLVE_CASE(2) G2_SOLVE_CASE(3) G2_SOLVE_CASE(4) G2_SOLVE_CASE(5) G2_SOLVE_CASE(6)
    G2_SOLVE_CASE(7) G2_SOLVE_CASE(8) G2_SOLVE_CASE(9) G2_SOLVE_CASE(10) G2_SOLVE_CASE(11) G2_SOLVE_CASE(12)
    G2_SOLVE_CASE(13) G2_SOLVE_CASE(14) G2_SOLVE_CASE(15)
#undef G2_SOLVE_CASE
    default:
      set_error("block size must be 1..15");
      return GPMP2MI_ERR_UNSUPPORTED;
  }
  G2_HIP(hipGetLastError());
  return GPMP2MI_OK;
}

}
```

Before: 104,100 trajectories/sec.

## Pass scalar constants by value, batch head loads, and fuse pass counter atomics

Kernel launches now receive a by-value PassConsts struct, so the kernels no longer dereference the PlanParams pointer for sizes and rules. Per-problem head loads (active, which, phase, iters, prev_err, share sums) are issued together up front, and the early-stop error reduction now reads the chunk shares lane-parallel and broadcasts them with readlane instead of a serial loop. The done and n_active atomics plus the threadfence are replaced by one packed 64-bit relaxed fetch-add, and the last arriving block publishes the count. The early-stop check is moved between the global loads and the LDS stores so its latency overlaps the staging loads. The risk is the relaxed ordering on the host-visible flag and the extra plumbing across kernels and queue buffers.

```diff
diff --git a/gpmp2_amd/csrc/assembler.h b/gpmp2_amd/csrc/assembler.h
--- a/gpmp2_amd/csrc/assembler.h
+++ b/gpmp2_amd/csrc/assembler.h
@@ -35,6 +35,13 @@
   __device__ __forceinline__ Slot make_slot(double* smem, int which) const {
     return Slot{smem + which * slot_doubles(P.I, P.RECS, P.GPS), P.RECS, P.I + 1, P.GPS};
   }
+  struct StageDims {
+    int I, RECS, GPS, N, Ppad, Npad;
+  };
+  __device__ __forceinline__ StageDims stage_dims() const { return StageDims{P.I, P.RECS, P.GPS, P.N, P.Ppad, P.Npad}; }
+  __device__ __forceinline__ static Slot make_slot(double* smem, int which, const StageDims& d) {
+    return Slot{smem + which * slot_doubles(d.I, d.RECS, d.GPS), d.RECS, d.I + 1, d.GPS};
+  }
 
   const PlanParams& P;
   const PlanBuffers& pb;
@@ -66,7 +73,12 @@
 
   static constexpr int NLD2 = (D <= 7) ? 6 : (D <= 11) ? 9 : 14;
   __device__ __forceinline__ void stage2(int iv, const Slot& s0, const Slot& s1, int count = 2) const {
-    const int I = P.I, RECS = P.RECS, GPS = P.GPS;
+    stage2(stage_dims(), iv, s0, s1, count, [] { return false; });
+  }
+  template <class Between>
+  __device__ __forceinline__ bool stage2(const StageDims& dm, int iv, const Slot& s0, const Slot& s1, int count,
+                                         Between between) const {
+    const int I = dm.I, RECS = dm.RECS, GPS = dm.GPS;
     double2 val[2][NLD2];
 #pragma unroll
     for (int w = 0; w < 2; w++) {
@@ -75,9 +87,9 @@
       const int npt = (ivw == 0) ? 1 : I + 1;
       const int nd2 = (npt * RECS) >> 1, ng2 = GPS >> 1, nc2 = (CQ / 2) * I;
       const int p0 = (ivw == 0) ? 0 : 1 + (ivw - 1) * (I + 1);
-      const bool in_range = ivw <= P.N;
-      const double2* src = reinterpret_cast<const double2*>(rec + ((size_t)b * P.Ppad + p0) * RECS);
-      const double2* gsrc = reinterpret_cast<const double2*>(gpu + ((size_t)b * P.Npad + ivw) * GPS);
+      const bool in_range = ivw <= dm.N;
+      const double2* src = reinterpret_cast<const double2*>(rec + ((size_t)b * dm.Ppad + p0) * RECS);
+      const double2* gsrc = reinterpret_cast<const double2*>(gpu + ((size_t)b * dm.Npad + ivw) * GPS);
       const double2* csrc = reinterpret_cast<const double2*>(P.coefq);
 #pragma unroll
       for (int m = 0; m < NLD2; m++) {
@@ -93,6 +105,7 @@
         val[w][m] = x;
       }
     }
+    if (between()) return true;
 #pragma unroll
     for (int w = 0; w < 2; w++) {
       if (w >= count) break;
@@ -109,6 +122,7 @@
         else if (v < nd2 + ng2 + nc2) dgp[v - nd2] = val[w][m];
       }
     }
+    return false;
   }
 
   __device__ __forceinline__ static double hint_vec(const double* pt, const double* M, double s, int kr) {
diff --git a/gpmp2_amd/csrc/cr_kernels.hip b/gpmp2_amd/csrc/cr_kernels.hip
--- a/gpmp2_amd/csrc/cr_kernels.hip
+++ b/gpmp2_amd/csrc/cr_kernels.hip
@@ -81,36 +81,46 @@
 #define G2_ASM_MINW 5
 #endif
 template <int D, bool LIE, StorePolicy ASM_OUT>
-__global__ __launch_bounds__(64 * ASM_WAVES, LIE ? 2 : G2_ASM_MINW) void k_assemble(const PlanParams* __restrict__ pp, PlanBuffers pb,
+__global__ __launch_bounds__(64 * ASM_WAVES, LIE ? 2 : G2_ASM_MINW) void k_assemble(PassConsts pc, const PlanParams* __restrict__ pp, PlanBuffers pb,
                                                               const double* __restrict__ traj, int bufsel,
                                                               double* __restrict__ tiles,
                                                               const int* __restrict__ active, int early_stop) {
   constexpr int n = 2 * D;
   using Asm = Assembler<D, LIE>;
   const PlanParams& P = *pp;
-  const int N = P.N;
+  const int N = pc.N;
   const int groups = crr_groups(N, ASM_WAVES);
   const int b = blockIdx.x / groups, q = blockIdx.x - b * groups;
-  if (active && !active[b]) return;
-  if (early_stop) {
-    int status;
-    if (gn_decide(P.rules, pb.iters[b], pb.prev_err[b], error_from_shares(P, pb, b), status) != 0) return;
-  }
-  if (active && dogleg_retry(P, pb, b)) return;
+  const int nchunk = pc.Ppad / 64;
+  int act = (active ? active : pb.active)[b];
+  int wh = pb.which[b];
+  int ph = pb.phase[b];
+  int it = pb.iters[b];
+  const double prev = pb.prev_err[b];
+  const ShareHead sh = shares_request(pb, b, nchunk, threadIdx.x & 63);
+  head_batch_end(act, wh, ph, it);
+  if (active && !act) return;
+  if (active && pc.rules.opt_type == GPMP2MI_OPT_DOGLEG && ph != 0) return;
   const int wv = threadIdx.x >> 6, lane = threadIdx.x & 63, c = lane & 15, g = lane >> 4;
   const int v = ASM_WAVES * q + wv, i = v - 1;
   const bool live = v >= 1 && i <= N;
   const int ic = min(max(i, 0), N);
   extern __shared__ __attribute__((aligned(16))) double asm_smem[];
-  const int slotd = Asm::slot_doubles(P.I, P.RECS, P.GPS);
+  const typename Asm::StageDims dm{pc.I, pc.RECS, pc.GPS, pc.N, pc.Ppad, pc.Npad};
+  const int slotd = Asm::slot_doubles(dm.I, dm.RECS, dm.GPS);
   double* xch = asm_smem + (size_t)(ASM_WAVES + 1) * slotd;
   double* xs0 = (slotd >= TILE_DBL) ? asm_smem : xch + 4 * TILE_DBL;
-  const double* rec = rec_of(pb, pb.which[b], bufsel);
-  const double* gpu = gpu_of(pb, pb.which[b], bufsel);
+  const double* rec = rec_of(pb, wh, bufsel);
+  const double* gpu = gpu_of(pb, wh, bufsel);
   Asm as(P, pb, rec, gpu, b, lane);
   G2_ASTAMP(0);
-  const typename Asm::Slot slot0 = as.make_slot(asm_smem, wv), slot1 = as.make_slot(asm_smem, wv + 1);
-  as.stage2(max(i, 0), slot0, slot1, wv == ASM_WAVES - 1 ? 2 : 1);
+  const typename Asm::Slot slot0 = Asm::make_slot(asm_smem, wv, dm), slot1 = Asm::make_slot(asm_smem, wv + 1, dm);
+  const bool stops = as.stage2(dm, max(i, 0), slot0, slot1, wv == ASM_WAVES - 1 ? 2 : 1, [&] {
+    if (!early_stop) return false;
+    int status;
+    return gn_decide(pc.rules, it, prev, error_from_shares(sh, pb, b, nchunk), status) != 0;
+  });
+  if (stops) return;
   __syncthreads();
   G2_ASTAMP(1);
   const bool odd = (v & 1) != 0;
@@ -236,10 +246,11 @@
     constexpr int D = decltype(d)::value;
     constexpr StorePolicy WT = StorePolicy::WriteThrough, PL = StorePolicy::Plain;
     const bool wt = hp.B <= ASM_WT_MAX_B;
-    if (hp.lie && wt) k_assemble<D, true, WT><<<grid, block, shmem, st>>>(pb.params, pb, traj, bufsel, pb.tiles, active, es);
-    else if (hp.lie) k_assemble<D, true, PL><<<grid, block, shmem, st>>>(pb.params, pb, traj, bufsel, pb.tiles, active, es);
-    else if (wt) k_assemble<D, false, WT><<<grid, block, shmem, st>>>(pb.params, pb, traj, bufsel, pb.tiles, active, es);
-    else k_assemble<D, false, PL><<<grid, block, shmem, st>>>(pb.params, pb, traj, bufsel, pb.tiles, active, es);
+    const PassConsts pc = pass_consts(hp);
+    if (hp.lie && wt) k_assemble<D, true, WT><<<grid, block, shmem, st>>>(pc, pb.params, pb, traj, bufsel, pb.tiles, active, es);
+    else if (hp.lie) k_assemble<D, true, PL><<<grid, block, shmem, st>>>(pc, pb.params, pb, traj, bufsel, pb.tiles, active, es);
+    else if (wt) k_assemble<D, false, WT><<<grid, block, shmem, st>>>(pc, pb.params, pb, traj, bufsel, pb.tiles, active, es);
+    else k_assemble<D, false, PL><<<grid, block, shmem, st>>>(pc, pb.params, pb, traj, bufsel, pb.tiles, active, es);
   });
 }
 
@@ -371,13 +382,20 @@
 }
 
 template <int D>
-__device__ __forceinline__ void gn_step_body(const PlanParams& P, const PlanBuffers& pb, int pass, int early_stop) {
+__device__ __forceinline__ int gn_step_body(const PassConsts& pc, const PlanParams& P, const PlanBuffers& pb, int pass,
+                                            int early_stop) {
   constexpr int n = 2 * D;
   const int b = blockIdx.x, tid = threadIdx.x, w = tid >> 6, lane = tid & 63, c = lane & 15, g = lane >> 4;
-  if (!pb.active[b]) return;
-  const int N = P.N;
+  const int N = pc.N, nchunk = pc.Ppad / 64;
+  int act = pb.active[b];
+  int it = pb.iters[b];
+  const double prev = pb.prev_err[b];
+  const ShareHead sh = shares_request(pb, b, nchunk, lane);
+  int prev_hi = __double2hiint(prev);
+  head_batch_end(act, it, prev_hi);
+  if (!act) return 0;
   const size_t tsz = (size_t)(N + 1) * n;
-  const bool odd = P.fuse_finish && (pass & 1);
+  const bool odd = pc.fuse_finish && (pass & 1);
   double* cur = (odd ? pb.last : pb.cur) + b * tsz;
   double* last = (odd ? pb.cur : pb.last) + b * tsz;
   double* result = pb.result + b * tsz;
@@ -388,11 +406,9 @@
   G2_STAMP_DECL;
 
   G2_STAMP(0);
-  const int it = pb.iters[b];
-  const double prev = pb.prev_err[b];
   double new_err;
   if (early_stop) {
-    new_err = error_from_shares(P, pb, b);
+    new_err = error_from_shares(sh, pb, b, nchunk);
     if (tid == 0) flags[1] = 0;
   } else {
     if (w == 0) {
@@ -408,16 +424,16 @@
     new_err = red[0];
   }
   int status;
-  const int decision = gn_decide(P.rules, it, prev, new_err, status);
+  const int decision = gn_decide(pc.rules, it, prev, new_err, status);
   if (tid == 0) {
-    if (it <= P.rules.max_iter) pb.trace[(size_t)b * (P.rules.max_iter + 1) + it] = new_err;
+    if (it <= pc.rules.max_iter) pb.trace[(size_t)b * (pc.rules.max_iter + 1) + it] = new_err;
     pb.cur_err[b] = new_err;
     if (decision != 0) {
       pb.status[b] = status;
       pb.final_err[b] = (decision == 2) ? prev : new_err;
     }
   }
-  const bool keep_err = it == 0 || (decision == 0 && P.rules.fixed_iters == 0);
+  const bool keep_err = it == 0 || (decision == 0 && pc.rules.fixed_iters == 0);
   if (decision != 0) {
     const double* src = (decision == 2) ? last : cur;
     for (size_t k = tid; k < tsz; k += blockDim.x) result[k] = src[k];
@@ -426,7 +442,7 @@
       if (keep_err) pb.prev_err[b] = new_err;
       pb.active[b] = 0;
     }
-    return;
+    return 0;
   }
 
   G2_STAMP(1);
@@ -443,10 +459,10 @@
       pb.final_err[b] = pb.cur_err[b];
       pb.active[b] = 0;
     }
-    return;
-  }
-
-  if (P.split_back) {
+    return 0;
+  }
+
+  if (pc.split_back) {
     cr_backward<n>(pb, b, N, tid, xs, FIN_BLOCKS);
     G2_STAMP(3);
     double* xg = pb.xg + (size_t)b * (N + 1) * 16;
@@ -459,9 +475,8 @@
       pb.stepped[b] = pass + 1;
       pb.last_err[b] = pb.cur_err[b];
       pb.iters[b] += 1;
-      atomicAdd(pb.n_active + pass, 1);
-    }
-    return;
+    }
+    return 1;
   }
   cr_backward<n>(pb, b, N, tid, xs);
   G2_STAMP(3);
@@ -471,20 +486,20 @@
     const int i = (int)(k / n), rho = (int)(k - (size_t)i * n);
     const double* zs = last + (size_t)i * n;
     const double* dz = xs + i * 16;
-    cur[k] = (rho < D) ? retract_coord(P.lie != 0, rho, zs, dz) : zs[rho] + dz[rho];
+    cur[k] = (rho < D) ? retract_coord(pc.lie != 0, rho, zs, dz) : zs[rho] + dz[rho];
   }
   G2_STAMP(4);
   if (tid == 0) {
     pb.last_err[b] = pb.cur_err[b];
     pb.iters[b] += 1;
-    atomicAdd(pb.n_active + pass, 1);
-  }
+  }
+  return 1;
 }
 template <int D>
-__global__ __launch_bounds__(64 * CR_WAVES) void k_gn_step_cr(const PlanParams* __restrict__ pp,
+__global__ __launch_bounds__(64 * CR_WAVES) void k_gn_step_cr(PassConsts pc, const PlanParams* __restrict__ pp,
                                                                PlanBuffers pb, int pass, int early_stop) {
-  gn_step_body<D>(*pp, pb, pass, early_stop);
-  if (threadIdx.x == 0) publish_pass_count(pb, pass);
+  const int continues = gn_step_body<D>(pc, *pp, pb, pass, early_stop);
+  if (threadIdx.x == 0) publish_pass_count(pb, pass, continues);
 }
 
 template <int D>
@@ -626,7 +641,7 @@
     return GPMP2MI_ERR_UNSUPPORTED;
   }
   return launch_for_dof(TILE_DOFS, hp.D, [&](auto d) {
-    k_gn_step_cr<decltype(d)::value><<<grid, block, shmem, st>>>(pb.params, pb, pass, early_stop ? 1 : 0);
+    k_gn_step_cr<decltype(d)::value><<<grid, block, shmem, st>>>(pass_consts(hp), pb.params, pb, pass, early_stop ? 1 : 0);
   });
 }
 
diff --git a/gpmp2_amd/csrc/host/plan_create.hip b/gpmp2_amd/csrc/host/plan_create.hip
--- a/gpmp2_amd/csrc/host/plan_create.hip
+++ b/gpmp2_amd/csrc/host/plan_create.hip
@@ -411,7 +411,7 @@
   G2_TRY(flags_acquire(p->n_active_len, &p->flagbuf));
   p->h_flags = p->flagbuf.host;
   pb.host_flags = p->flagbuf.dev;
-  G2_TRY(plan_alloc(p, &pb.done, p->n_active_len));
+  G2_TRY(plan_alloc(p, &pb.pass_word, p->n_active_len));
   return GPMP2MI_OK;
 }
 
diff --git a/gpmp2_amd/csrc/host/plan_run.hip b/gpmp2_amd/csrc/host/plan_run.hip
--- a/gpmp2_amd/csrc/host/plan_run.hip
+++ b/gpmp2_amd/csrc/host/plan_run.hip
@@ -225,8 +225,8 @@
   G2_CHECK(cap_l <= (1L << 26), GPMP2MI_ERR_UNSUPPORTED, "too many problems for one queue run");
   const int cap = (int)cap_l;
 
-  const size_t ints = 5 * (size_t)B + 1 + 3 * (size_t)cap;
-  const size_t bytes = sizeof(long long) + ints * sizeof(int);
+  const size_t slot_ints = (5 * (size_t)B + 1 + 1) & ~(size_t)1;
+  const size_t bytes = sizeof(long long) + slot_ints * sizeof(int) + (size_t)cap * (sizeof(unsigned long long) + 2 * sizeof(int));
   G2_TRY(p->ws[p->WS_QUEUE].reserve(bytes));
   if (p->qflags.cap < cap) {
     flags_release(p->qflags);
@@ -242,12 +242,12 @@
   q.qpass = w + 4 * B;
   q.head = w + 5 * B;
   PlanBuffers qb = p->pb;
-  qb.n_active = q.head + 1;
-  qb.done = qb.n_active + cap;
-  qb.host_flags = qb.done + cap;
+  qb.pass_word = (unsigned long long*)(w + slot_ints);
+  qb.n_active = (int*)(qb.pass_word + cap);
+  qb.host_flags = qb.n_active + cap;
   q.flags = p->qflags.dev;
   for (int k = 0; k < cap; k++) p->qflags.host[k] = -1;
-  G2_HIP(hipMemsetAsync(qb.n_active, 0, 3 * (size_t)cap * sizeof(int), st));
+  G2_HIP(hipMemsetAsync(qb.pass_word, 0, (size_t)cap * (sizeof(unsigned long long) + 2 * sizeof(int)), st));
 
   const PlanBuffers& pb = p->pb;
   p->timer.reset();
diff --git a/gpmp2_amd/csrc/linearize_kernels.hip b/gpmp2_amd/csrc/linearize_kernels.hip
--- a/gpmp2_amd/csrc/linearize_kernels.hip
+++ b/gpmp2_amd/csrc/linearize_kernels.hip
@@ -246,7 +246,7 @@
 }
 
 template <int AD, int SDIM, int NW>
-__global__ __launch_bounds__(64 * NW, 3) void k_linearize_arm(const RobotDev* __restrict__ Rg, SdfDev sdf,
+__global__ __launch_bounds__(64 * NW, 3) void k_linearize_arm(PassConsts pc, const RobotDev* __restrict__ Rg, SdfDev sdf,
                                                                const PlanParams* __restrict__ pp, PlanBuffers pb,
                                                                const double* __restrict__ traj, int bufsel,
                                                                const int* __restrict__ active, double* __restrict__ dst,
@@ -258,12 +258,16 @@
   constexpr int ROWS_P = (NW / 2) * rec_lds_stride(RV);
   constexpr int ROWS = (ROWS_F + ROWS_SC > ROWS_P) ? ROWS_F + ROWS_SC : ROWS_P;
   const PlanParams& P = *pp;
-  const int nchunk = P.Ppad / 64;
+  const int nchunk = pc.Ppad / 64;
   const int b = blockIdx.x / nchunk, chunk = blockIdx.x - b * nchunk;
-  if (active && !active[b]) return;
+  int act = (active ? active : pb.active)[b];
+  int wh = pb.which[b];
+  int stp = pb.stepped[b];
+  head_batch_end(act, wh, stp);
+  if (active && !act) return;
   const int wv = __builtin_amdgcn_readfirstlane(threadIdx.x >> 6), lane = threadIdx.x & 63;
-  double* __restrict__ rec = rec_of(pb, pb.which[b], bufsel);
-  double* __restrict__ gpu = gpu_of(pb, pb.which[b], bufsel);
+  double* __restrict__ rec = rec_of(pb, wh, bufsel);
+  double* __restrict__ gpu = gpu_of(pb, wh, bufsel);
   G2_LSTAMP(0);
   __shared__ RobotDev R;
   __shared__ double buf[ROWS][64];
@@ -275,8 +279,8 @@
     rtmp[u] = idx < RN ? reinterpret_cast<const int*>(Rg)[idx] : 0;
   }
   const int p_raw = chunk * 64 + lane;
-  const int p = min(p_raw, P.P - 1);
-  const int N = P.N, I = P.I;
+  const int p = min(p_raw, pc.P - 1);
+  const int N = pc.N, I = pc.I;
   int i = 0, j = I;
   if (p > 0) {
     const int t = p - 1;
@@ -284,14 +288,14 @@
     j = t - (i - 1) * (I + 1);
   }
   const bool unary = (j == I);
-  const bool store_ok = p_raw < P.P;
+  const bool store_ok = p_raw < pc.P;
   double (*fx)[16] = reinterpret_cast<double (*)[16]>(&buf[0][0]);
   static_assert(FXS * 16 <= ROWS * 64, "the step window lives in the frame buffer");
   __shared__ double zn[ZNS][n];
-  const int p_lo = chunk * 64, p_hi = min(p_lo + 63, P.P - 1);
+  const int p_lo = chunk * 64, p_hi = min(p_lo + 63, pc.P - 1);
   auto state_of = [&](int pt) { return pt == 0 ? 0 : 1 + (pt - 1) / (I + 1); };
   const int s1 = state_of(p_hi), s0 = max(0, state_of(p_lo) - 1), ns = s1 - s0 + 1;
-  const bool apply = dst != nullptr && pb.stepped[b] == pass;
+  const bool apply = dst != nullptr && stp == pass;
   const bool shares = bufsel == 0 && !trial;
   double* __restrict__ cshare = pb.cshare + ((size_t)b * nchunk + chunk) * 3;
   if (apply) {
@@ -575,9 +579,9 @@
   if (hp.lin_split == 4) {
     const dim3 block(256);
     if (sdf.dim == 3) {
-      G2_DISPATCH_ROBOT_ARM_ONLY(h.arm_dof, (k_linearize_arm<AD_, 3, 4><<<grid, block, 0, st>>>(robot, sdf, pb.params, pb, traj, bufsel, active, dst, pass, trial ? 1 : 0)));
+      G2_DISPATCH_ROBOT_ARM_ONLY(h.arm_dof, (k_linearize_arm<AD_, 3, 4><<<grid, block, 0, st>>>(pass_consts(hp), robot, sdf, pb.params, pb, traj, bufsel, active, dst, pass, trial ? 1 : 0)));
     } else {
-      G2_DISPATCH_ROBOT_ARM_ONLY(h.arm_dof, (k_linearize_arm<AD_, 2, 4><<<grid, block, 0, st>>>(robot, sdf, pb.params, pb, traj, bufsel, active, dst, pass, trial ? 1 : 0)));
+      G2_DISPATCH_ROBOT_ARM_ONLY(h.arm_dof, (k_linearize_arm<AD_, 2, 4><<<grid, block, 0, st>>>(pass_consts(hp), robot, sdf, pb.params, pb, traj, bufsel, active, dst, pass, trial ? 1 : 0)));
     }
   } else if (hp.lin_split == 2) {
     const dim3 block(128);
diff --git a/gpmp2_amd/csrc/pass_counter.h b/gpmp2_amd/csrc/pass_counter.h
--- /dev/null
+++ b/gpmp2_amd/csrc/pass_counter.h
@@ -0,0 +1,19 @@
+#pragma once
+#include <cstdint>
+
+#ifndef G2_PURE
+#ifdef __HIPCC__
+#define G2_PURE __host__ __device__ __forceinline__
+#else
+#define G2_PURE inline
+#endif
+#endif
+
+namespace g2 {
+
+G2_PURE uint64_t pass_arrival(int continues) { return (uint64_t(1) << 32) + (uint64_t)(uint32_t)continues; }
+G2_PURE int pass_arrivals_before(uint64_t before) { return (int)(uint32_t)(before >> 32); }
+G2_PURE bool pass_arrived_last(uint64_t before, int grid) { return pass_arrivals_before(before) == grid - 1; }
+G2_PURE int pass_count(uint64_t before, int continues) { return (int)(uint32_t)before + continues; }
+
+}
diff --git a/gpmp2_amd/csrc/plan.h b/gpmp2_amd/csrc/plan.h
--- a/gpmp2_amd/csrc/plan.h
+++ b/gpmp2_amd/csrc/plan.h
@@ -34,6 +34,15 @@
   double vel_lim[MAXD], vel_th[MAXD], vel_w[MAXD];
   double KA[4 * MAXD * MAXD], KB[4 * MAXD * MAXD], KO[4 * MAXD * MAXD];
 };
+
+struct PassConsts {
+  int N, Ppad, P, I, RECS, GPS, Npad;
+  int fuse_finish, split_back, lie;
+  StepRules rules;
+};
+inline PassConsts pass_consts(const PlanParams& hp) {
+  return PassConsts{hp.N, hp.Ppad, hp.P, hp.I, hp.RECS, hp.GPS, hp.Npad, hp.fuse_finish, hp.split_back, hp.lie, hp.rules};
+}
 
 struct SelfPairRec {
   double total_eps, w;
@@ -130,7 +139,7 @@
   double* epart;
   double* cshare;
   int* n_active;
-  int* done;
+  unsigned long long* pass_word;
   int* host_flags;
   unsigned long long* stamps;
 };
diff --git a/gpmp2_amd/csrc/plan_device.h b/gpmp2_amd/csrc/plan_device.h
--- a/gpmp2_amd/csrc/plan_device.h
+++ b/gpmp2_amd/csrc/plan_device.h
@@ -1,5 +1,6 @@
 #pragma once
 #include "device_math.h"
+#include "pass_counter.h"
 #include "plan.h"
 #include "tiles.h"
 
@@ -100,14 +101,37 @@
   return P.rules.opt_type == GPMP2MI_OPT_DOGLEG && pb.phase[b] != 0;
 }
 
-__device__ __forceinline__ double error_from_shares(const PlanParams& P, const PlanBuffers& pb, int b) {
-  const int nchunk = P.Ppad / 64;
+__device__ __forceinline__ void head_batch_end(int& a, int& b, int& c) {
+  asm volatile("" : "+s"(a), "+s"(b), "+s"(c)::"memory");
+}
+__device__ __forceinline__ void head_batch_end(int& a, int& b, int& c, int& d) {
+  asm volatile("" : "+s"(a), "+s"(b), "+s"(c), "+s"(d)::"memory");
+}
+
+struct ShareHead {
+  double a, g, m;
+};
+__device__ __forceinline__ ShareHead shares_request(const PlanBuffers& pb, int b, int nchunk, int lane) {
+  const double* __restrict__ cs = pb.cshare + ((size_t)b * nchunk + lane) * 3;
+  ShareHead h{0.0, 0.0, 0.0};
+  if (lane < nchunk) {
+    h.a = cs[0];
+    h.g = cs[1];
+    h.m = cs[2];
+  }
+  return h;
+}
+__device__ __forceinline__ double error_from_shares(const ShareHead& h, const PlanBuffers& pb, int b, int nchunk) {
+  const double t = (h.a + h.g) + h.m;
+  const int lo = __double2loint(t), hi = __double2hiint(t);
+  double acc = 0.0;
+  const int nq = min(nchunk, 64);
+  for (int q = 0; q < nq; q++)
+    acc += __hiloint2double(__builtin_amdgcn_readlane(hi, q), __builtin_amdgcn_readlane(lo, q));
   const double* __restrict__ cs = pb.cshare + (size_t)b * nchunk * 3;
-  double acc = 0.0;
-  for (int q = 0; q < nchunk; q++) acc += (cs[3 * q] + cs[3 * q + 1]) + cs[3 * q + 2];
+  for (int q = 64; q < nchunk; q++) acc += (cs[3 * q] + cs[3 * q + 1]) + cs[3 * q + 2];
   return 0.5 * acc;
 }
-
 
 template <int WAVES>
 __device__ __forceinline__ double block_sum(double v, double* red, int tid) {
@@ -189,12 +213,14 @@
   }
 }
 
-__device__ __forceinline__ void publish_pass_count(const PlanBuffers& pb, int pass) {
-  __threadfence();
-  if (atomicAdd(pb.done + pass, 1) == (int)gridDim.x - 1) {
-    const int v = atomicAdd(pb.n_active + pass, 0);
-    __hip_atomic_store(pb.host_flags + pass, v, __ATOMIC_RELEASE, __HIP_MEMORY_SCOPE_SYSTEM);
-  }
-}
-
-}
+__device__ __forceinline__ void publish_pass_count(const PlanBuffers& pb, int pass, int continues) {
+  const unsigned long long before = __hip_atomic_fetch_add(pb.pass_word + pass, (unsigned long long)pass_arrival(continues),
+                                                           __ATOMIC_RELAXED, __HIP_MEMORY_SCOPE_AGENT);
+  if (pass_arrived_last(before, (int)gridDim.x)) {
+    const int v = pass_count(before, continues);
+    pb.n_active[pass] = v;
+    __hip_atomic_store(pb.host_flags + pass, v, __ATOMIC_RELAXED, __HIP_MEMORY_SCOPE_SYSTEM);
+  }
+}
+
+}
diff --git a/gpmp2_amd/csrc/plan_kernels.hip b/gpmp2_amd/csrc/plan_kernels.hip
--- a/gpmp2_amd/csrc/plan_kernels.hip
+++ b/gpmp2_amd/csrc/plan_kernels.hip
@@ -122,7 +122,10 @@
     const size_t tot = B * (size_t)(P.N + 1) * P.n;
     for (size_t k = tid; k < tot; k += nth) pb.cur[k] = start[k];
   }
-  for (size_t k = tid; k < (size_t)P.max_pass; k += nth) pb.n_active[k] = pb.done[k] = 0;
+  for (size_t k = tid; k < (size_t)P.max_pass; k += nth) {
+    pb.n_active[k] = 0;
+    pb.pass_word[k] = 0;
+  }
   for (size_t k = tid; k < B * SC_COUNT; k += nth) pb.scal[k] = 0.0;
   for (size_t k = tid; k < B * (size_t)(P.rules.max_iter + 1); k += nth) pb.trace[k] = __longlong_as_double(0x7ff8000000000000LL);
   for (size_t b = tid; b < B; b += nth) reset_slot(P, pb, b);
@@ -136,12 +139,12 @@
   return GPMP2MI_OK;
 }
 
-__device__ __forceinline__ void decide_body(const PlanParams& P, const PlanBuffers& pb, int pass, int init) {
+__device__ __forceinline__ int decide_body(const PlanParams& P, const PlanBuffers& pb, int pass, int init) {
   const int b = blockIdx.x, tid = threadIdx.x, lane = tid & 63;
   const bool w0 = tid < 64;
   __shared__ int dec[2];
   __shared__ double red[4];
-  if (!pb.active[b]) return;
+  if (!pb.active[b]) return 0;
   const int N = P.N, n = P.n;
   const size_t tsz = (size_t)(N + 1) * n;
   double* cur = pb.cur + b * tsz;
@@ -290,14 +293,12 @@
   } else if (action == 2) {
     for (size_t k = tid; k < tsz; k += blockDim.x) result[k] = last[k];
   }
-  if (tid == 0) {
-    if (action != 0) pb.active[b] = 0;
-    else atomicAdd(pb.n_active + pass, 1);
-  }
+  if (tid == 0 && action != 0) pb.active[b] = 0;
+  return action == 0;
 }
 __global__ __launch_bounds__(256) void k_decide(const PlanParams* __restrict__ pp, PlanBuffers pb, int pass, int init) {
-  decide_body(*pp, pb, pass, init);
-  if (threadIdx.x == 0) publish_pass_count(pb, pass);
+  const int continues = decide_body(*pp, pb, pass, init);
+  if (threadIdx.x == 0) publish_pass_count(pb, pass, continues);
 }
 
 int launch_decide(const PlanParams& hp, const PlanBuffers& pb, int pass, bool init, hipStream_t st) {
```

Result: faster. 108,400 trajectories/sec (median of 6 runs) (+4.1%).
